# Woodenonez/TrajTrack-MPCnDQN-RLBoost

Hardware: NVIDIA B200
Metric: batched NMPC solves/sec (higher is better)
Workload: dtype f64

## Files before the change

### trajtrack_mpcndqn_rlboost_b200/csrc/ttmpc_api.cu

```cuda
#include <cuda_runtime.h>

#include <cstdio>
#include <cstdlib>
#include <cstring>
#include <algorithm>
#include <atomic>
#include <condition_variable>
#include <mutex>
#include <thread>
#include <string>
#include <vector>

#include "ttmpc_device.cuh"
#include "ttmpc_launch.cuh"

using namespace ttmpc;

static thread_local std::string g_err;
static int fail(int code, const std::string &msg) { g_err = msg; return code; }
namespace ttmpc { void set_last_error(const std::string &msg) { g_err = msg; } }
#define CUDA_TRY(x)                                                                     \
  do {                                                                                  \
    cudaError_t e__ = (x);                                                              \
    if (e__ != cudaSuccess)                                                             \
      return fail(TTMPC_ERR_CUDA, std::string(#x) + ": " + cudaGetErrorString(e__));    \
  } while (0)

extern "C" const char *ttmpc_last_error(void) { return g_err.c_str(); }
extern "C" int ttmpc_version(void) { return TTMPC_VERSION; }
extern "C" int ttmpc_set_device(int device) { CUDA_TRY(cudaSetDevice(device)); return TTMPC_OK; }
extern "C" int ttmpc_get_device(int *device) {
  if (!device) return fail(TTMPC_ERR_BAD_ARG, "null output");
  CUDA_TRY(cudaGetDevice(device));
  return TTMPC_OK;
}
extern "C" const char *ttmpc_exit_status_name(int code) {
  switch (code) {
    case TTMPC_CONVERGED: return "Converged";
    case TTMPC_NOT_CONVERGED_ITERATIONS: return "NotConvergedIterations";
    case TTMPC_NOT_CONVERGED_OUT_OF_TIME: return "NotConvergedOutOfTime";
    case TTMPC_NOT_FINITE: return "NotFiniteComputation";
    default: return "Unknown";
  }
}

extern "C" void ttmpc_default_config(ttmpc_config *c) {
  std::memset(c, 0, sizeof(*c));
  c->N_hor = 20; c->nu = 2; c->ns = 3; c->nq = 10;
  c->Nother = 10; c->Nstcobs = 10; c->nstcobs = 12; c->Ndynobs = 15; c->ndynobs = 6;
  c->ts = 0.2; c->vehicle_width = 0.5; c->social_margin = 0.2;
  c->lin_vel_min = -0.5; c->lin_vel_max = 1.5; c->ang_vel_max = 0.5;
  c->lin_acc_min = -1.0; c->lin_acc_max = 1.0; c->ang_acc_max = 3.0;
  c->tolerance = 1e-4; c->initial_tolerance = 1e-4; c->delta_tolerance = 1e-4;
  c->initial_penalty = 10.0; c->penalty_update_factor = 5.0;
  c->inner_tolerance_update_factor = 0.1; c->sufficient_decrease_coeff = 0.1;
  c->lbfgs_memory = 10; c->max_inner_iterations = 500; c->max_outer_iterations = 10;
  c->max_duration_ms = 5000;
}
extern "C" int ttmpc_num_params(const ttmpc_config *c) {
  const int N = c->N_hor;
  return 2 * c->ns + c->nu + c->nq + c->ns * N + N + c->ns * N * c->Nother +
         c->Nstcobs * c->nstcobs + c->Ndynobs * c->ndynobs * N + 2 * N;
}
extern "C" int ttmpc_num_decision(const ttmpc_config *c) { return c->nu * c->N_hor; }
extern "C" int ttmpc_num_alm(const ttmpc_config *c) { return 2 * c->N_hor; }
extern "C" int ttmpc_num_penalty(const ttmpc_config *c) { return c->Ndynobs; }

static int make_devcfg(const ttmpc_config *c, DevCfg *g) {
  if (!c) return fail(TTMPC_ERR_BAD_CONFIG, "null config");
  if (c->nu != 2 || c->ns != 3 || c->nq != 10 || c->ndynobs != 6)
    return fail(TTMPC_ERR_BAD_CONFIG, "nu/ns/nq/ndynobs must be 2/3/10/6 (unicycle, mpc_generator.py layout)");
  if (c->N_hor < 1 || c->N_hor > 32) return fail(TTMPC_ERR_BAD_CONFIG, "N_hor must be in 1..32");
  if (c->nstcobs % 3 != 0 || c->nstcobs / 3 > MAX_EDGE || (c->Nstcobs > 0 && c->nstcobs < 3))
    return fail(TTMPC_ERR_BAD_CONFIG, "nstcobs must be 3*edges with edges <= 8");
  if (c->Nother < 0 || c->Nstcobs < 0 || c->Ndynobs < 0 || c->Ndynobs > 64 || c->Nother > 32 ||
      c->Nstcobs > 32)
    return fail(TTMPC_ERR_BAD_CONFIG, "obstacle counts out of range (Nother, Nstcobs <= 32, Ndynobs <= 64)");
  if (c->lbfgs_memory < 1 || c->lbfgs_memory > MAX_MEM)
    return fail(TTMPC_ERR_BAD_CONFIG, "lbfgs_memory must be in 1..16");
  if (c->max_inner_iterations < 1 || c->max_outer_iterations < 1 || !(c->ts > 0.0))
    return fail(TTMPC_ERR_BAD_CONFIG, "iteration limits and ts must be positive");
  const int N = c->N_hor;
  g->N = N; g->Nother = c->Nother; g->Nstc = c->Nstcobs; g->nstcobs = c->nstcobs;
  g->ne = c->nstcobs / 3; g->Ndyn = c->Ndynobs; g->mem = c->lbfgs_memory;
  g->max_inner = c->max_inner_iterations; g->max_outer = c->max_outer_iterations;
  g->max_ns = c->max_duration_ms > 0 ? (unsigned long long)c->max_duration_ms * 1000000ull : 0ull;
  g->off_s = 0; g->off_q = 2 * c->ns + c->nu; g->off_r = g->off_q + c->nq;
  g->off_vref = g->off_r + c->ns * N; g->off_c = g->off_vref + N;
  g->off_os = g->off_c + c->ns * N * c->Nother;
  g->off_od = g->off_os + c->Nstcobs * c->nstcobs;
  g->off_qdyn = g->off_od + c->Ndynobs * c->ndynobs * N + N;
  g->np = g->off_qdyn + N;
  g->smem_per_warp = smem_bytes_per_warp(N, g->Nother, g->Nstc, g->nstcobs, g->Ndyn, g->mem);
  {
    const size_t cap = 232448 - 256;
    if ((size_t)g->smem_per_warp > cap)
      return fail(TTMPC_ERR_UNSUPPORTED, "configuration does not fit in shared memory: " +
                  std::to_string(g->smem_per_warp) + " bytes of tables per scene, 227 KB per SM");
    int wpb = 1, best = 0;
    for (int cand : {2, 3, 4, 1}) {
      const size_t per_cta = (size_t)g->smem_per_warp * cand + 96 + 1024;
      if ((size_t)g->smem_per_warp * cand > cap) continue;
      const int ctas = (int)std::min<size_t>(233472 / per_cta, (size_t)(8 / cand));
      if (ctas * cand > best) { best = ctas * cand; wpb = cand; }
    }
    g->warps_per_block = wpb;
  }
  g->ts = c->ts; g->inv_ts = 1.0 / c->ts; g->h6 = c->ts / 6.0; g->veh_d2 = c->vehicle_width * c->vehicle_width; g->margin = c->social_margin;
  g->vmin = c->lin_vel_min; g->vmax = c->lin_vel_max; g->wmax = c->ang_vel_max;
  g->amin = c->lin_acc_min; g->amax = c->lin_acc_max; g->awmax = c->ang_acc_max;
  g->tol = c->tolerance; g->init_tol = c->initial_tolerance; g->delta_tol = c->delta_tolerance;
  g->c0 = c->initial_penalty; g->pen_factor = c->penalty_update_factor;
  g->tol_factor = c->inner_tolerance_update_factor; g->suff_dec = c->sufficient_decrease_coeff;
  return TTMPC_OK;
}

struct Slot {
  bool keyed = false;
  cudaStream_t key = nullptr;
  bool host = false, host_busy = false;
  double *dyn_scratch = nullptr; size_t dyn_bytes = 0;
  int *work_counter = nullptr;
  unsigned long long *run_stats = nullptr;
  int *ready = nullptr;
  int *h_ready = nullptr;
  cudaStream_t copy_stream = nullptr, exec_stream = nullptr;
  cudaEvent_t ev_inputs = nullptr;
  cudaEvent_t ev_done = nullptr;
  int *order = nullptr; size_t order_ints = 0;
  void *dbuf = nullptr; size_t dbytes = 0;
  void *hbuf = nullptr; size_t hbytes = 0;
};
constexpr int MAX_STREAM_SLOTS = 16, MAX_HOST_SLOTS = 8;
struct Workspace {
  int device = -1;
  int sm_count = 0;
  unsigned long long *stats = nullptr;
  std::vector<Slot *> slots;
};
static std::mutex g_mu;
static std::condition_variable g_cv;
static std::vector<Workspace> g_ws;

static int get_ws(Workspace **out) {
  int dev = 0;
  CUDA_TRY(cudaGetDevice(&dev));
  for (auto &w : g_ws)
    if (w.device == dev) { *out = &w; return TTMPC_OK; }
  Workspace w;
  w.device = dev;
  CUDA_TRY(cudaDeviceGetAttribute(&w.sm_count, cudaDevAttrMultiProcessorCount, dev));
  CUDA_TRY(cudaMalloc(&w.stats, 192));
  CUDA_TRY(cudaMemset(w.stats, 0, 192));
  g_ws.reserve(16);
  g_ws.push_back(w);
  *out = &g_ws.back();
  return TTMPC_OK;
}
static int new_slot(Workspace *w, Slot **out) {
  Slot *s = new Slot();
  CUDA_TRY(cudaMalloc(&s->work_counter, 64));
  CUDA_TRY(cudaMalloc(&s->run_stats, 64));
  CUDA_TRY(cudaMemset(s->run_stats, 0, 64));
  CUDA_TRY(cudaMalloc(&s->ready, 64));
  w->slots.push_back(s);
  *out = s;
  return TTMPC_OK;
}
static int slot_for_stream(Workspace *w, cudaStream_t st, Slot **out) {
  for (int pass = 0; pass < 2; pass++) {
    int device_slots = 0;
    Slot *free_slot = nullptr;
    for (Slot *s : w->slots) {
      if (s->host) continue;
      device_slots++;
      if (s->keyed && s->key == st) { *out = s; return TTMPC_OK; }
      if (!s->keyed && !free_slot) free_slot = s;
    }
    if (!free_slot && device_slots < MAX_STREAM_SLOTS) {
      int rc = new_slot(w, &free_slot);
      if (rc) return rc;
    }
    if (free_slot) {
      free_slot->keyed = true; free_slot->key = st;
      *out = free_slot;
      return TTMPC_OK;
    }
    CUDA_TRY(cudaDeviceSynchronize());
    for (Slot *s : w->slots)
      if (!s->host) s->keyed = false;
  }
  return fail(TTMPC_ERR_CUDA, "no scene-queue slot for this stream");
}
static int acquire_host_slot(Workspace **wout, Slot **out, int *busy_calls) {
  std::unique_lock<std::mutex> lk(g_mu);
  Workspace *w;
  int rc = get_ws(&w);
  if (rc) return rc;
  *wout = w;
  while (true) {
    int hosts = 0, busy = 1;
    for (Slot *s : w->slots) busy += (s->host && s->host_busy) ? 1 : 0;
    *busy_calls = busy;
    for (Slot *s : w->slots) {
      if (!s->host) continue;
      hosts++;
      if (!s->host_busy) { s->host_busy = true; *out = s; return TTMPC_OK; }
    }
    if (hosts < MAX_HOST_SLOTS) break;
    g_cv.wait(lk);
  }
  Slot *s;
  rc = new_slot(w, &s);
  if (rc) return rc;
  cudaError_t e = cudaHostAlloc(&s->h_ready, sizeof(int) * 4096, cudaHostAllocDefault);
  if (e == cudaSuccess) e = cudaStreamCreateWithFlags(&s->copy_stream, cudaStreamNonBlocking);
  if (e == cudaSuccess) e = cudaStreamCreateWithFlags(&s->exec_stream, cudaStreamNonBlocking);
  if (e == cudaSuccess) e = cudaEventCreateWithFlags(&s->ev_inputs, cudaEventDisableTiming);
  if (e == cudaSuccess) e = cudaEventCreateWithFlags(&s->ev_done, cudaEventDisableTiming | cudaEventBlockingSync);
  if (e != cudaSuccess)
    return fail(TTMPC_ERR_CUDA, std::string("host path: streams / pinned memory of a new slot: ") + cudaGetErrorString(e));
  s->host = true; s->host_busy = true;
  *out = s;
  return TTMPC_OK;
}
namespace {
struct HostSlotLease {
  Slot *s = nullptr;
  bool clean = false;
  ~HostSlotLease() {
    if (!s) return;
    if (!clean) {
      if (s->copy_stream) cudaStreamSynchronize(s->copy_stream);
      if (s->exec_stream) cudaStreamSynchronize(s->exec_stream);
      cudaGetLastError();
    }
    { std::lock_guard<std::mutex> lk(g_mu); s->host_busy = false; }
    g_cv.notify_one();
  }
};
}
static int wait_stream(Slot *s, cudaStream_t st, int n_scenes) {
  if (n_scenes < 512) { CUDA_TRY(cudaStreamSynchronize(st)); return TTMPC_OK; }
  CUDA_TRY(cudaEventRecord(s->ev_done, st));
  CUDA_TRY(cudaEventSynchronize(s->ev_done));
  return TTMPC_OK;
}
static int ensure_dyn(Slot *w, size_t bytes) {
  if (bytes <= w->dyn_bytes) return TTMPC_OK;
  if (w->dyn_scratch) CUDA_TRY(cudaFree(w->dyn_scratch));
  w->dyn_scratch = nullptr; w->dyn_bytes = 0;
  CUDA_TRY(cudaMalloc(&w->dyn_scratch, bytes));
  w->dyn_bytes = bytes;
  return TTMPC_OK;
}
static int ensure_order(Slot *w, size_t ints) {
  if (ints <= w->order_ints) return TTMPC_OK;
  if (w->order) CUDA_TRY(cudaFree(w->order));
  w->order = nullptr; w->order_ints = 0;
  CUDA_TRY(cudaMalloc(&w->order, ints * sizeof(int)));
  w->order_ints = ints;
  return TTMPC_OK;
}
static int ensure_staging(Slot *w, size_t bytes) {
  if (bytes > w->dbytes) {
    if (w->dbuf) CUDA_TRY(cudaFree(w->dbuf));
    w->dbuf = nullptr; w->dbytes = 0;
    CUDA_TRY(cudaMalloc(&w->dbuf, bytes));
    if (w->copy_stream) CUDA_TRY(cudaMemsetAsync(w->dbuf, 0, bytes, w->copy_stream));
    else { CUDA_TRY(cudaMemset(w->dbuf, 0, bytes)); CUDA_TRY(cudaDeviceSynchronize()); }
    w->dbytes = bytes;
  }
  if (bytes > w->hbytes) {
    if (w->hbuf) CUDA_TRY(cudaFreeHost(w->hbuf));
    w->hbuf = nullptr; w->hbytes = 0;
    CUDA_TRY(cudaHostAlloc(&w->hbuf, bytes, cudaHostAllocDefault));
    w->hbytes = bytes;
  }
  return TTMPC_OK;
}

static int grid_for(Workspace *w, const DevCfg &g, int n_scenes, int *grid) {
  int bps = 0;
  CUDA_TRY(solve_occupancy(g, &bps));
  if (bps < 1) return fail(TTMPC_ERR_UNSUPPORTED, "configuration does not fit in shared memory");
  long long want = ((long long)n_scenes + g.warps_per_block - 1) / g.warps_per_block;
  long long cap = (long long)w->sm_count * bps;
  *grid = (int)(want < cap ? (want < 1 ? 1 : want) : cap);
  return TTMPC_OK;
}

static int solve_device_impl(const ttmpc_config *cfg, int n_scenes, const double *d_p, int use_u0,
                             int use_y0, const double *d_c0, const ttmpc_result *res,
                             cudaStream_t st, Slot *host_slot, bool gated);

extern "C" int ttmpc_solve_batch_device(const ttmpc_config *cfg, int n_scenes, const double *d_p,
                                        int use_u0, int use_y0, const double *d_c0,
                                        const ttmpc_result *res, void *stream) {
  return solve_device_impl(cfg, n_scenes, d_p, use_u0, use_y0, d_c0, res, (cudaStream_t)stream, nullptr, false);
}

static int solve_device_impl(const ttmpc_config *cfg, int n_scenes, const double *d_p, int use_u0,
                             int use_y0, const double *d_c0, const ttmpc_result *res,
                             cudaStream_t st, Slot *host_slot, bool gated) {
  DevCfg g;
  int rc = make_devcfg(cfg, &g);
  if (rc) return rc;
  if (n_scenes < 0 || !res || !res->u || (n_scenes > 0 && !d_p))
    return fail(TTMPC_ERR_BAD_ARG, "n_scenes >= 0, d_p and res->u are required");
  if (n_scenes == 0) return TTMPC_OK;
  Workspace *w;
  Slot *sl = host_slot;
  const int *d_ready = (host_slot && gated) ? host_slot->ready : nullptr;
  int grid;
  bool want_order = false;
  {
    std::lock_guard<std::mutex> lk(g_mu);
    rc = get_ws(&w);
    if (rc) return rc;
    if (!sl) { rc = slot_for_stream(w, st, &sl); if (rc) return rc; }
    rc = grid_for(w, g, n_scenes, &grid);
    if (rc) return rc;
    const size_t table = (size_t)DYN_FIELDS * g.Ndyn * g.N * sizeof(double);
    rc = ensure_dyn(sl, (table ? table : 8) * (size_t)grid * g.warps_per_block);
    if (rc) return rc;
    want_order = !d_ready && n_scenes > (long long)grid * g.warps_per_block;
    if (want_order) {
      rc = ensure_order(sl, 2 * (size_t)n_scenes + 64);
      if (rc) return rc;
    }
  }
  CUDA_TRY(cudaMemsetAsync(sl->work_counter, 0, sizeof(int), st));
  const char *nh = std::getenv("TTMPC_NO_HELPERS");
  SolveArgs A;
  A.eprof = w->stats + 8;
  A.helpers = (nh && nh[0] == '1') ? 0 : 1;
  A.ready = d_ready; A.timeout_flag = d_ready ? sl->ready + 1 : nullptr;
  A.p = d_p; A.c0 = d_c0; A.u = res->u; A.y = res->y; A.cost = res->cost;
  A.last_fpr = res->last_fpr; A.f1_infeas = res->f1_infeas; A.f2_norm = res->f2_norm;
  A.penalty = res->penalty; A.exit_status = res->exit_status; A.outer_iters = res->outer_iters;
  A.inner_iters = res->inner_iters; A.pred_states = res->pred_states; A.evals = res->evals;
  A.dyn_scratch = sl->dyn_scratch; A.work_counter = sl->work_counter; A.stats = w->stats;
  A.run_stats = sl->run_stats;
  CUDA_TRY(cudaMemsetAsync(A.run_stats, 0, 2 * sizeof(unsigned long long), st));
  A.n_scenes = n_scenes; A.use_u0 = use_u0; A.use_y0 = use_y0;
  A.order = nullptr;
  if (want_order) {
    CUDA_TRY(launch_rank_scenes(g, d_p, n_scenes, sl->order + n_scenes, sl->order, st));
    A.order = sl->order;
  }
  bool small_code = n_scenes > (long long)grid * g.warps_per_block;
  if (const char *e = std::getenv("TTMPC_CODE")) {
    if (e[0] == 's') small_code = true;
    else if (e[0] == 'u') small_code = false;
  }
  if (small_code) CUDA_TRY(launch_solve_small(g, A, grid, st));
  else CUDA_TRY(launch_solve(g, A, grid, st));
  return TTMPC_OK;
}

static int fleet_dims(const ttmpc_config *cfg, const ttmpc_fleet *f, FleetDims *d) {
  DevCfg g;
  int rc = make_devcfg(cfg, &g);
  if (rc) return rc;
  if (!f || f->n < 0) return fail(TTMPC_ERR_BAD_ARG, "fleet: null or n < 0");
  if (f->n > 0 && (!f->state || !f->goal || !f->last_u || !f->idx_ref || !f->status || !f->ref_traj ||
                   !f->ref_len || !f->stc))
    return fail(TTMPC_ERR_BAD_ARG, "fleet: state, goal, last_u, idx_ref, status, ref_traj, ref_len, stc are required");
  if (f->action_steps != 1) return fail(TTMPC_ERR_UNSUPPORTED, "fleet: only action_steps = 1 is supported");
  if (f->ref_stride < 1) return fail(TTMPC_ERR_BAD_ARG, "fleet: ref_stride must be >= 1");
  if (f->dyn_cur && (!f->dyn_last || !f->dyn_disp || f->n_dyn_live < 0 || f->n_dyn_live > cfg->Ndynobs))
    return fail(TTMPC_ERR_BAD_ARG, "fleet: dyn_cur needs dyn_last, dyn_disp and 0 <= n_dyn_live <= Ndynobs");
  d->N = cfg->N_hor; d->np = g.np; d->ts = cfg->ts;
  d->n_other = cfg->ns * cfg->N_hor * cfg->Nother;
  d->n_stc = cfg->Nstcobs * cfg->nstcobs;
  d->n_dyn = cfg->Ndynobs * cfg->ndynobs * cfg->N_hor;
  return TTMPC_OK;
}
extern "C" int ttmpc_fleet_pack_device(const ttmpc_config *cfg, const ttmpc_fleet *fleet, double *d_p,
                                       void *stream) {
  FleetDims d;
  int rc = fleet_dims(cfg, fleet, &d);
  if (rc) return rc;
  if (fleet->n == 0) return TTMPC_OK;
  if (!d_p) return fail(TTMPC_ERR_BAD_ARG, "fleet: d_p is required");
  CUDA_TRY(launch_fleet_pack(*fleet, d, d_p, (cudaStream_t)stream));
  return TTMPC_OK;
}
extern "C" int ttmpc_fleet_advance_device(const ttmpc_config *cfg, const ttmpc_fleet *fleet,
                                          const double *d_u, const int *d_exit_status, void *stream) {
  FleetDims d;
  int rc = fleet_dims(cfg, fleet, &d);
  if (rc) return rc;
  if (fleet->n == 0) return TTMPC_OK;
  if (!d_u) return fail(TTMPC_ERR_BAD_ARG, "fleet: d_u is required");
  CUDA_TRY(launch_fleet_advance(*fleet, d, d_u, d_exit_status, (cudaStream_t)stream));
  return TTMPC_OK;
}
extern "C" int ttmpc_fleet_step_device(const ttmpc_config *cfg, const ttmpc_fleet *fleet, double *d_p,
                                       int use_y0, const ttmpc_result *res, void *stream) {
  if (!res || !res->u || !res->exit_status)
    return fail(TTMPC_ERR_BAD_ARG, "fleet: res->u and res->exit_status are required");
  int rc = ttmpc_fleet_pack_device(cfg, fleet, d_p, stream);
  if (rc) return rc;
  rc = ttmpc_solve_batch_device(cfg, fleet->n, d_p, 0, use_y0, nullptr, res, stream);
  if (rc) return rc;
  return ttmpc_fleet_advance_device(cfg, fleet, res->u, res->exit_status, stream);
}

static int read_stats(unsigned long long *out, int count, int reset) {
  std::lock_guard<std::mutex> lk(g_mu);
  Workspace *w;
  int rc = get_ws(&w);
  if (rc) return rc;
  CUDA_TRY(cudaDeviceSynchronize());
  CUDA_TRY(cudaMemcpy(out, w->stats, count * sizeof(unsigned long long), cudaMemcpyDeviceToHost));
  if (reset) CUDA_TRY(cudaMemset(w->stats, 0, 192));
  return TTMPC_OK;
}
extern "C" int ttmpc_read_stats(unsigned long long out[4], int reset) { return read_stats(out, 4, reset); }
extern "C" int ttmpc_read_stats8(unsigned long long out[8], int reset) { return read_stats(out, 8, reset); }
extern "C" int ttmpc_read_stats24(unsigned long long out[24], int reset) { return read_stats(out, 24, reset); }

extern "C" int ttmpc_launch_info(const ttmpc_config *cfg, int n_scenes, int *grid, int *block,
                                 int *smem_bytes, int *blocks_per_sm, int *sm_count) {
  DevCfg g;
  int rc = make_devcfg(cfg, &g);
  if (rc) return rc;
  std::lock_guard<std::mutex> lk(g_mu);
  Workspace *w;
  rc = get_ws(&w);
  if (rc) return rc;
  int gr;
  rc = grid_for(w, g, n_scenes, &gr);
  if (rc) return rc;
  int bps = 0;
  CUDA_TRY(solve_occupancy(g, &bps));
  if (grid) *grid = gr;
  if (block) *block = g.warps_per_block * 32;
  if (smem_bytes) *smem_bytes = g.smem_per_warp * g.warps_per_block;
  if (blocks_per_sm) *blocks_per_sm = bps;
  if (sm_count) *sm_count = w->sm_count;
  return TTMPC_OK;
}

namespace {
struct Carver {
  char *d, *h; size_t off = 0;
  template <class T> void take(size_t n, T **dp, T **hp) {
    off = (off + 255) / 256 * 256;
    *dp = reinterpret_cast<T *>(d + off);
    *hp = reinterpret_cast<T *>(h + off);
    off += n * sizeof(T);
  }
};
}

extern "C" int ttmpc_solve_batch_host(const ttmpc_config *cfg, int n, const double *h_p,
                                      int use_u0, int use_y0, const double *h_c0,
                                      const ttmpc_result *res) {
  DevCfg g;
  int rc = make_devcfg(cfg, &g);
  if (rc) return rc;
  if (n < 0 || !res || !res->u || (n > 0 && !h_p))
    return fail(TTMPC_ERR_BAD_ARG, "n >= 0, h_p and res->u are required");
  if (n == 0) return TTMPC_OK;
  const size_t nn = (size_t)n, nu = 2 * (size_t)g.N;
  size_t total = 4096 + 256 * 16 + sizeof(double) * (nn * g.np + nn + 2 * nn * nu + 5 * nn + nn * g.N * 3) +
                 sizeof(int) * 3 * nn + sizeof(long long) * 4 * nn;
  Workspace *ws;
  Slot *w = nullptr;
  int busy_calls = 1;
  rc = acquire_host_slot(&ws, &w, &busy_calls);
  HostSlotLease lease{w};
  if (rc) return rc;
  rc = ensure_staging(w, total);
  if (rc) return rc;
  Carver cv{(char *)w->dbuf, (char *)w->hbuf};
  double *dp, *hp, *dc0, *hc0, *du, *hu, *dy, *hy, *dcost, *hcost, *dfpr, *hfpr, *df1, *hf1, *df2,
      *hf2, *dpen, *hpen, *dps, *hps;
  int *dex, *hex, *dout, *hout, *din, *hin;
  long long *dev, *hev;
  cv.take(nn * g.np, &dp, &hp);
  cv.take(nn, &dc0, &hc0);
  cv.take(nn * nu, &du, &hu);
  cv.take(nn * nu, &dy, &hy);
  cv.take(nn, &dcost, &hcost);
  cv.take(nn, &dfpr, &hfpr);
  cv.take(nn, &df1, &hf1);
  cv.take(nn, &df2, &hf2);
  cv.take(nn, &dpen, &hpen);
  cv.take(nn * g.N * 3, &dps, &hps);
  cv.take(nn, &dex, &hex);
  cv.take(nn, &dout, &hout);
  cv.take(nn, &din, &hin);
  cv.take(4 * nn, &dev, &hev);
  cudaStream_t cs = w->copy_stream, st = w->exec_stream;
  CUDA_TRY(cudaMemsetAsync(w->ready, 0, 2 * sizeof(int), cs));
  if (h_c0) {
    std::memcpy(hc0, h_c0, sizeof(double) * nn);
    CUDA_TRY(cudaMemcpyAsync(dc0, hc0, sizeof(double) * nn, cudaMemcpyHostToDevice, cs));
  }
  if (use_u0) {
    std::memcpy(hu, res->u, sizeof(double) * nn * nu);
    CUDA_TRY(cudaMemcpyAsync(du, hu, sizeof(double) * nn * nu, cudaMemcpyHostToDevice, cs));
  }
  if (use_y0 && res->y) {
    std::memcpy(hy, res->y, sizeof(double) * nn * nu);
    CUDA_TRY(cudaMemcpyAsync(dy, hy, sizeof(double) * nn * nu, cudaMemcpyHostToDevice, cs));
  }
  CUDA_TRY(cudaEventRecord(w->ev_inputs, cs));
  CUDA_TRY(cudaStreamWaitEvent(st, w->ev_inputs, 0));
  ttmpc_result dres;
  std::memset(&dres, 0, sizeof(dres));
  dres.u = du; dres.y = res->y ? dy : nullptr; dres.cost = dcost; dres.exit_status = dex;
  dres.outer_iters = dout; dres.inner_iters = din; dres.last_fpr = dfpr; dres.f1_infeas = df1;
  dres.f2_norm = df2; dres.penalty = dpen; dres.pred_states = res->pred_states ? dps : nullptr;
  dres.evals = dev;
  const char *lb = std::getenv("CUDA_LAUNCH_BLOCKING");
  const bool stream_in = busy_calls <= 1 && !(lb && lb[0] == '1');
  if (stream_in) {
    rc = solve_device_impl(cfg, n, dp, use_u0, use_y0 && res->y, h_c0 ? dc0 : nullptr, &dres, st, w, true);
    if (rc) return rc;
  }
  cudaPointerAttributes at;
  const bool pinned_in = cudaPointerGetAttributes(&at, h_p) == cudaSuccess ? at.type == cudaMemoryTypeHost
                                                                           : (cudaGetLastError(), false);
  {
    int chunk = 256;
    while ((n + chunk - 1) / chunk > 4096) chunk *= 2;
    const int n_chunks = (n + chunk - 1) / chunk;
    struct Chunk { int s1; size_t off, cnt; };
    auto chunk_at = [&](int ci) {
      const int s0 = ci * chunk, s1 = std::min(s0 + chunk, n);
      return Chunk{s1, (size_t)s0 * g.np, (size_t)(s1 - s0) * g.np};
    };
    const unsigned hw = std::thread::hardware_concurrency();
    int budget = (int)(hw ? hw / 2 : 1);
    if (const char *e = std::getenv("TTMPC_HOST_THREADS")) { const int v = std::atoi(e); if (v >= 1) budget = v; }
    const int T = pinned_in ? 1 : std::max(1, std::min({8, budget / std::max(1, busy_calls), n_chunks}));
    const double *src = pinned_in ? h_p : hp;
    std::vector<std::atomic<int>> staged(n_chunks);
    for (auto &f : staged) f.store(pinned_in ? 1 : 0, std::memory_order_relaxed);
    auto stage = [&](int ci) {
      const Chunk c = chunk_at(ci);
      std::memcpy(hp + c.off, h_p + c.off, sizeof(double) * c.cnt);
      staged[ci].store(1, std::memory_order_release);
    };
    std::vector<std::thread> workers;
    for (int t = 1; t < T; t++)
      workers.emplace_back([&, t] { for (int ci = t; ci < n_chunks; ci += T) stage(ci); });
    int rc_copy = TTMPC_OK;
    int mine = 0;
    for (int ci = 0; ci < n_chunks; ci++) {
      while (!staged[ci].load(std::memory_order_acquire)) {
        if (mine < n_chunks) { stage(mine); mine += T; }
        else std::this_thread::yield();
      }
      if (rc_copy != TTMPC_OK) continue;
      const Chunk c = chunk_at(ci);
      w->h_ready[ci] = c.s1;
      if (cudaMemcpyAsync(dp + c.off, src + c.off, sizeof(double) * c.cnt, cudaMemcpyHostToDevice, cs) != cudaSuccess ||
          cudaMemcpyAsync(w->ready, w->h_ready + ci, sizeof(int), cudaMemcpyHostToDevice, cs) != cudaSuccess)
        rc_copy = TTMPC_ERR_CUDA;
    }
    for (auto &th : workers) th.join();
    if (rc_copy != TTMPC_OK) return fail(TTMPC_ERR_CUDA, "host path: asynchronous copy of the parameter block failed");
  }
  int timed_out = 0;
  if (stream_in) {
    rc = wait_stream(w, st, n);
    if (rc) return rc;
    CUDA_TRY(cudaMemcpy(&timed_out, w->ready + 1, sizeof(int), cudaMemcpyDeviceToHost));
  }
  if (!stream_in || timed_out) {
    rc = wait_stream(w, cs, n);
    if (rc) return rc;
    if (use_u0) CUDA_TRY(cudaMemcpyAsync(du, hu, sizeof(double) * nn * nu, cudaMemcpyHostToDevice, st));
    if (use_y0 && res->y) CUDA_TRY(cudaMemcpyAsync(dy, hy, sizeof(double) * nn * nu, cudaMemcpyHostToDevice, st));
    rc = solve_device_impl(cfg, n, dp, use_u0, use_y0 && res->y, h_c0 ? dc0 : nullptr, &dres, st, w, false);
    if (rc) return rc;
  }
  const size_t out_begin = (size_t)((char *)du - (char *)w->dbuf);
  CUDA_TRY(cudaMemcpyAsync((char *)w->hbuf + out_begin, (char *)w->dbuf + out_begin, cv.off - out_begin,
                           cudaMemcpyDeviceToHost, st));
  rc = wait_stream(w, st, n);
  if (rc) return rc;
  std::memcpy(res->u, hu, sizeof(double) * nn * nu);
  if (res->y) std::memcpy(res->y, hy, sizeof(double) * nn * nu);
  if (res->cost) std::memcpy(res->cost, hcost, sizeof(double) * nn);
  if (res->last_fpr) std::memcpy(res->last_fpr, hfpr, sizeof(double) * nn);
  if (res->f1_infeas) std::memcpy(res->f1_infeas, hf1, sizeof(double) * nn);
  if (res->f2_norm) std::memcpy(res->f2_norm, hf2, sizeof(double) * nn);
  if (res->penalty) std::memcpy(res->penalty, hpen, sizeof(double) * nn);
  if (res->pred_states) std::memcpy(res->pred_states, hps, sizeof(double) * nn * g.N * 3);
  if (res->exit_status) std::memcpy(res->exit_status, hex, sizeof(int) * nn);
  if (res->outer_iters) std::memcpy(res->outer_iters, hout, sizeof(int) * nn);
  if (res->inner_iters) std::memcpy(res->inner_iters, hin, sizeof(int) * nn);
  if (res->evals) std::memcpy(res->evals, hev, sizeof(long long) * 4 * nn);
  lease.clean = true;
  return TTMPC_OK;
}

extern "C" int ttmpc_eval_batch_device(const ttmpc_config *cfg, int n, const double *d_p,
                                       const double *d_u, const double *d_c, const double *d_y,
                                       double *d_f, double *d_F1, double *d_F2, double *d_psi,
                                       double *d_grad, void *stream) {
  DevCfg g;
  int rc = make_devcfg(cfg, &g);
  if (rc) return rc;
  if (n < 0 || (n > 0 && (!d_p || !d_u))) return fail(TTMPC_ERR_BAD_ARG, "d_p and d_u are required");
  if (n == 0) return TTMPC_OK;
  std::lock_guard<std::mutex> lk(g_mu);
  Workspace *w;
  rc = get_ws(&w);
  if (rc) return rc;
  int grid;
  rc = grid_for(w, g, n, &grid);
  if (rc) return rc;
  const size_t table = (size_t)DYN_FIELDS * g.Ndyn * g.N * sizeof(double);
  Slot *sl;
  rc = slot_for_stream(w, (cudaStream_t)stream, &sl);
  if (rc) return rc;
  rc = ensure_dyn(sl, (table ? table : 8) * (size_t)grid * g.warps_per_block);
  if (rc) return rc;
  EvalArgs A;
  A.p = d_p; A.u = d_u; A.c = d_c; A.y = d_y; A.f = d_f; A.F1 = d_F1; A.F2 = d_F2; A.psi = d_psi;
  A.grad = d_grad; A.dyn_scratch = sl->dyn_scratch; A.n_scenes = n;
  CUDA_TRY(launch_eval(g, A, grid, (cudaStream_t)stream));
  return TTMPC_OK;
}

extern "C" int ttmpc_eval_batch_host(const ttmpc_config *cfg, int n, const double *h_p,
                                     const double *h_u, const double *h_c, const double *h_y,
                                     double *h_f, double *h_F1, double *h_F2, double *h_psi,
                                     double *h_grad) {
  DevCfg g;
  int rc = make_devcfg(cfg, &g);
  if (rc) return rc;
  if (n < 0 || (n > 0 && (!h_p || !h_u))) return fail(TTMPC_ERR_BAD_ARG, "h_p and h_u are required");
  if (n == 0) return TTMPC_OK;
  const size_t nn = (size_t)n, nu = 2 * (size_t)g.N;
  double *dp = nullptr, *du = nullptr, *dc = nullptr, *dy = nullptr, *df = nullptr, *dF1 = nullptr,
         *dF2 = nullptr, *dpsi = nullptr, *dgrad = nullptr;
  auto cleanup = [&]() {
    cudaFree(dp); cudaFree(du); cudaFree(dc); cudaFree(dy); cudaFree(df); cudaFree(dF1);
    cudaFree(dF2); cudaFree(dpsi); cudaFree(dgrad);
  };
#define TRY_OR_CLEAN(x) do { cudaError_t e__ = (x); if (e__ != cudaSuccess) { cleanup(); return fail(TTMPC_ERR_CUDA, std::string(#x) + ": " + cudaGetErrorString(e__)); } } while (0)
  TRY_OR_CLEAN(cudaMalloc(&dp, sizeof(double) * nn * g.np));
  TRY_OR_CLEAN(cudaMalloc(&du, sizeof(double) * nn * nu));
  TRY_OR_CLEAN(cudaMalloc(&dc, sizeof(double) * nn));
  TRY_OR_CLEAN(cudaMalloc(&dy, sizeof(double) * nn * nu));
  TRY_OR_CLEAN(cudaMalloc(&df, sizeof(double) * nn));
  TRY_OR_CLEAN(cudaMalloc(&dF1, sizeof(double) * nn * nu));
  TRY_OR_CLEAN(cudaMalloc(&dF2, sizeof(double) * nn * (g.Ndyn > 0 ? g.Ndyn : 1)));
  TRY_OR_CLEAN(cudaMalloc(&dpsi, sizeof(double) * nn));
  TRY_OR_CLEAN(cudaMalloc(&dgrad, sizeof(double) * nn * nu));
  TRY_OR_CLEAN(cudaMemcpy(dp, h_p, sizeof(double) * nn * g.np, cudaMemcpyHostToDevice));
  TRY_OR_CLEAN(cudaMemcpy(du, h_u, sizeof(double) * nn * nu, cudaMemcpyHostToDevice));
  if (h_c) TRY_OR_CLEAN(cudaMemcpy(dc, h_c, sizeof(double) * nn, cudaMemcpyHostToDevice));
  if (h_y) TRY_OR_CLEAN(cudaMemcpy(dy, h_y, sizeof(double) * nn * nu, cudaMemcpyHostToDevice));
  rc = ttmpc_eval_batch_device(cfg, n, dp, du, h_c ? dc : nullptr, h_y ? dy : nullptr, df, dF1, dF2,
                               dpsi, dgrad, 0);
  if (rc) { cleanup(); return rc; }
  TRY_OR_CLEAN(cudaDeviceSynchronize());
  if (h_f) TRY_OR_CLEAN(cudaMemcpy(h_f, df, sizeof(double) * nn, cudaMemcpyDeviceToHost));
  if (h_F1) TRY_OR_CLEAN(cudaMemcpy(h_F1, dF1, sizeof(double) * nn * nu, cudaMemcpyDeviceToHost));
  if (h_F2 && g.Ndyn) TRY_OR_CLEAN(cudaMemcpy(h_F2, dF2, sizeof(double) * nn * g.Ndyn, cudaMemcpyDeviceToHost));
  if (h_psi) TRY_OR_CLEAN(cudaMemcpy(h_psi, dpsi, sizeof(double) * nn, cudaMemcpyDeviceToHost));
  if (h_grad) TRY_OR_CLEAN(cudaMemcpy(h_grad, dgrad, sizeof(double) * nn * nu, cudaMemcpyDeviceToHost));
  cleanup();
  return TTMPC_OK;
}

extern "C" int ttmpc_probe_latency(const ttmpc_config *cfg, const double *h_p, long long out[8], int reps) {
  DevCfg g;
  int rc = make_devcfg(cfg, &g);
  if (rc) return rc;
  double *dp = nullptr, *dyn = nullptr; long long *dout = nullptr;
  CUDA_TRY(cudaMalloc(&dp, sizeof(double) * g.np));
  CUDA_TRY(cudaMalloc(&dyn, sizeof(double) * DYN_FIELDS * (g.Ndyn > 0 ? g.Ndyn : 1) * g.N));
  CUDA_TRY(cudaMalloc(&dout, 64));
  CUDA_TRY(cudaMemcpy(dp, h_p, sizeof(double) * g.np, cudaMemcpyHostToDevice));
  CUDA_TRY(launch_probe(g, dp, dyn, dout, reps, 0));
  CUDA_TRY(cudaDeviceSynchronize());
  CUDA_TRY(cudaMemcpy(out, dout, 64, cudaMemcpyDeviceToHost));
  cudaFree(dp); cudaFree(dyn); cudaFree(dout);
  return TTMPC_OK;
}

extern "C" int ttmpc_measure_fp64_peak(double *tflops, void *stream) {
  if (!tflops) return fail(TTMPC_ERR_BAD_ARG, "null output");
  int dev = 0, sms = 0;
  CUDA_TRY(cudaGetDevice(&dev));
  CUDA_TRY(cudaDeviceGetAttribute(&sms, cudaDevAttrMultiProcessorCount, dev));
  const int threads = 256, blocks = sms * 8, iters = 1 << 15;
  double *out = nullptr;
  CUDA_TRY(cudaMalloc(&out, sizeof(double) * threads * blocks));
  cudaStream_t st = (cudaStream_t)stream;
  cudaEvent_t e0, e1;
  CUDA_TRY(cudaEventCreate(&e0));
  CUDA_TRY(cudaEventCreate(&e1));
  double best = 0.0;
  for (int rep = 0; rep < 4; rep++) {
    CUDA_TRY(cudaEventRecord(e0, st));
    CUDA_TRY(launch_fp64_peak(out, blocks, threads, iters, st));
    CUDA_TRY(cudaEventRecord(e1, st));
    CUDA_TRY(cudaEventSynchronize(e1));
    float ms = 0;
    CUDA_TRY(cudaEventElapsedTime(&ms, e0, e1));
    double fl = 2.0 * 8.0 * (double)iters * threads * blocks;
    double tf = fl / (ms * 1e-3) / 1e12;
    if (rep > 0 && tf > best) best = tf;
  }
  cudaEventDestroy(e0); cudaEventDestroy(e1); cudaFree(out);
  *tflops = best;
  return TTMPC_OK;
}
```

### trajtrack_mpcndqn_rlboost_b200/csrc/ttmpc_device.cuh

```cuda
#pragma once
#include <cuda_runtime.h>
#include <math.h>
#include <stdint.h>

#include "../../include/ttmpc.h"

#ifdef TTMPC_SMALL_CODE
#define TT_UNROLL_4 _Pragma("unroll 1")
#else
#define TT_UNROLL_4 _Pragma("unroll 4")
#endif
namespace ttmpc {

constexpr unsigned FULL = 0xffffffffu;
constexpr int MAX_MEM = 16;
constexpr int MAX_EDGE = 8;
constexpr int DYN_FIELDS = 10;
#ifndef TT_DYN_SLOTS
#define TT_DYN_SLOTS 4
#endif
constexpr int DYN_SLOTS = TT_DYN_SLOTS;

struct DevCfg {
  int N, Nother, Nstc, ne, nstcobs, Ndyn, mem, max_inner, max_outer;
  int off_s, off_q, off_r, off_vref, off_c, off_os, off_od, off_qdyn, np;
  int smem_per_warp;
  int warps_per_block;
  double ts, inv_ts, h6, veh_d2, margin;
  double vmin, vmax, wmax, amin, amax, awmax;
  double tol, init_tol, delta_tol, c0, pen_factor, tol_factor, suff_dec;
  unsigned long long max_ns;
};

__host__ __device__ __forceinline__ void tt_sincos(double x, double *s, double *c) {
  const double kd = rint(x * 6.36619772367581382433e-01);
  double r = fma(-kd, 1.5707963267948966e+00, x);
  r = fma(-kd, 6.123233995736766e-17, r);
  r = fma(-kd, -1.4973849048591698e-33, r);
  const int q = (int)((long long)kd & 3);
  const double z = r * r;
  double ps = fma(z, 1.58969099521155010221e-10, -2.50507602534068634195e-08);
  ps = fma(z, ps, 2.75573137070700676789e-06);
  ps = fma(z, ps, -1.98412698298579493134e-04);
  ps = fma(z, ps, 8.33333333332248946124e-03);
  ps = fma(z, ps, -1.66666666666666324348e-01);
  const double sr = fma(r * z, ps, r);
  double pc = fma(z, -1.13596475577881948265e-11, 2.08757232129817482790e-09);
  pc = fma(z, pc, -2.75573143513906633035e-07);
  pc = fma(z, pc, 2.48015872894767294178e-05);
  pc = fma(z, pc, -1.38888888888741095749e-03);
  pc = fma(z, pc, 4.16666666666666019037e-02);
  const double cr = fma(z * z, pc, fma(-0.5, z, 1.0));
  const bool swap = (q & 1) != 0;
  const double sb = swap ? cr : sr, cb = swap ? sr : cr;
  double so = (q & 2) ? -sb : sb, co = ((q + 1) & 2) ? -cb : cb;
  if (!(fabs(x) < 1.0e9)) { so = x * 0.0 + NAN; co = so; }
  *s = so; *c = co;
}

static __constant__ double TT_SC[16] = {
    6.36619772367581382433e-01, 1.5707963267948966e+00, 6.123233995736766e-17, -1.4973849048591698e-33,
    1.58969099521155010221e-10, -2.50507602534068634195e-08, 2.75573137070700676789e-06,
    -1.98412698298579493134e-04, 8.33333333332248946124e-03, -1.66666666666666324348e-01,
    -1.13596475577881948265e-11, 2.08757232129817482790e-09, -2.75573143513906633035e-07,
    2.48015872894767294178e-05, -1.38888888888741095749e-03, 4.16666666666666019037e-02};
__device__ __forceinline__ void tt_sincos_c(double x, double *s, double *c) {
  const double kd = rint(x * TT_SC[0]);
  double r = fma(-kd, TT_SC[1], x);
  r = fma(-kd, TT_SC[2], r);
  r = fma(-kd, TT_SC[3], r);
  const int q = (int)((long long)kd & 3);
  const double z = r * r;
  double ps = fma(z, TT_SC[4], TT_SC[5]);
  ps = fma(z, ps, TT_SC[6]);
  ps = fma(z, ps, TT_SC[7]);
  ps = fma(z, ps, TT_SC[8]);
  ps = fma(z, ps, TT_SC[9]);
  const double sr = fma(r * z, ps, r);
  double pc = fma(z, TT_SC[10], TT_SC[11]);
  pc = fma(z, pc, TT_SC[12]);
  pc = fma(z, pc, TT_SC[13]);
  pc = fma(z, pc, TT_SC[14]);
  pc = fma(z, pc, TT_SC[15]);
  const double cr = fma(z * z, pc, fma(-0.5, z, 1.0));
  const bool swap = (q & 1) != 0;
  const double sb = swap ? cr : sr, cb = swap ? sr : cr;
  double so = (q & 2) ? -sb : sb, co = ((q + 1) & 2) ? -cb : cb;
  if (!(fabs(x) < 1.0e9)) { so = x * 0.0 + NAN; co = so; }
  *s = so; *c = co;
}

static __device__ __noinline__ double tt_div(double a, double b) { return a / b; }
static __device__ __noinline__ double tt_sqrt(double a) { return sqrt(a); }

template <int O>
__device__ __forceinline__ void up_add(double &v) {
  asm volatile("{\n\t.reg .pred p;\n\t.reg .b32 lo, hi, tl, th;\n\t.reg .f64 t;\n\t"
               "mov.b64 {lo, hi}, %0;\n\t"
               "shfl.sync.up.b32 tl|p, lo, %1, 0, 0xffffffff;\n\t"
               "shfl.sync.up.b32 th, hi, %1, 0, 0xffffffff;\n\t"
               "mov.b64 t, {tl, th};\n\t"
               "@p add.rn.f64 %0, %0, t;\n\t}"
               : "+d"(v) : "n"(O));
}
template <int O>
__device__ __forceinline__ void down_add(double &v) {
  asm volatile("{\n\t.reg .pred p;\n\t.reg .b32 lo, hi, tl, th;\n\t.reg .f64 t;\n\t"
               "mov.b64 {lo, hi}, %0;\n\t"
               "shfl.sync.down.b32 tl|p, lo, %1, 31, 0xffffffff;\n\t"
               "shfl.sync.down.b32 th, hi, %1, 31, 0xffffffff;\n\t"
               "mov.b64 t, {tl, th};\n\t"
               "@p add.rn.f64 %0, %0, t;\n\t}"
               : "+d"(v) : "n"(O));
}
__device__ __forceinline__ double wscan(double v, int) {
  up_add<1>(v); up_add<2>(v); up_add<4>(v); up_add<8>(v); up_add<16>(v);
  return v;
}
__device__ __forceinline__ void wscan2(double &a, double &b) {
  up_add<1>(a); up_add<1>(b); up_add<2>(a); up_add<2>(b); up_add<4>(a); up_add<4>(b);
  up_add<8>(a); up_add<8>(b); up_add<16>(a); up_add<16>(b);
}
__device__ __forceinline__ double wsuffix(double v, int) {
  down_add<1>(v); down_add<2>(v); down_add<4>(v); down_add<8>(v); down_add<16>(v);
  return v;
}
__device__ __forceinline__ void wsuffix2(double &a, double &b) {
  down_add<1>(a); down_add<1>(b); down_add<2>(a); down_add<2>(b); down_add<4>(a); down_add<4>(b);
  down_add<8>(a); down_add<8>(b); down_add<16>(a); down_add<16>(b);
}
template <int O>
__device__ __forceinline__ double xor_get(double v) {
  double t;
  asm volatile("{\n\t.reg .b32 lo, hi, tl, th;\n\t"
               "mov.b64 {lo, hi}, %1;\n\t"
               "shfl.sync.bfly.b32 tl, lo, %2, 31, 0xffffffff;\n\t"
               "shfl.sync.bfly.b32 th, hi, %2, 31, 0xffffffff;\n\t"
               "mov.b64 %0, {tl, th};\n\t}"
               : "=d"(t) : "d"(v), "n"(O));
  return t;
}
__device__ __forceinline__ double wsum_inl(double v) {
  v += xor_get<16>(v); v += xor_get<8>(v); v += xor_get<4>(v); v += xor_get<2>(v); v += xor_get<1>(v);
  return v;
}
static __device__ __noinline__ double wsum(double v) { return wsum_inl(v); }
__device__ __forceinline__ void wsum4_inl(double &a, double &b, double &c, double &d, int lane) {
  const bool b4 = (lane & 16) != 0, b3 = (lane & 8) != 0;
  double x = b4 ? c : a, y = b4 ? d : b;
  const double sx = b4 ? a : c, sy = b4 ? b : d;
  x += xor_get<16>(sx); y += xor_get<16>(sy);
  double z = b3 ? y : x;
  const double sz = b3 ? x : y;
  z += xor_get<8>(sz);
  z += xor_get<4>(z); z += xor_get<2>(z); z += xor_get<1>(z);
  a = __shfl_sync(FULL, z, 0); b = __shfl_sync(FULL, z, 8);
  c = __shfl_sync(FULL, z, 16); d = __shfl_sync(FULL, z, 24);
}
struct D4 { double a, b, c, d; };
static __device__ __noinline__ D4 wsum4v(double a, double b, double c, double d) {
  wsum4_inl(a, b, c, d, threadIdx.x & 31);
  D4 r; r.a = a; r.b = b; r.c = c; r.d = d;
  return r;
}
__device__ __forceinline__ void wsum4(double &a, double &b, double &c, double &d, int) {
  const D4 r = wsum4v(a, b, c, d);
  a = r.a; b = r.b; c = r.c; d = r.d;
}
__device__ __forceinline__ void wsum2(double &a, double &b) {
  const D4 r = wsum4v(a, b, 0.0, 0.0);
  a = r.a; b = r.b;
}
__device__ __forceinline__ void wsum3(double &a, double &b, double &c) {
  const D4 r = wsum4v(a, b, c, 0.0);
  a = r.a; b = r.b; c = r.c;
}
__device__ __forceinline__ double clipd_ref(double z, double lo, double hi) {
  return fmin(fmax(z, lo), hi);
}
__device__ __forceinline__ double sel_gt(double a, double b, double x, double y) {
  double r;
  asm("{\n\t.reg .pred p;\n\tsetp.gt.f64 p, %1, %2;\n\tselp.f64 %0, %3, %4, p;\n\t}"
      : "=d"(r) : "d"(a), "d"(b), "d"(x), "d"(y));
  return r;
}
__device__ __forceinline__ double sel_lt(double a, double b, double x, double y) {
  double r;
  asm("{\n\t.reg .pred p;\n\tsetp.lt.f64 p, %1, %2;\n\tselp.f64 %0, %3, %4, p;\n\t}"
      : "=d"(r) : "d"(a), "d"(b), "d"(x), "d"(y));
  return r;
}
__device__ __forceinline__ double clipd(double z, double lo, double hi) {
  const double t = sel_gt(z, lo, z, lo);
  return sel_lt(t, hi, t, hi);
}
__device__ __forceinline__ double relu(double x) { return sel_gt(x, 0.0, x, 0.0); }
__device__ __forceinline__ double clamp01(double x) {
  const double t = sel_gt(x, 0.0, x, 0.0);
  return sel_lt(t, 1.0, t, 1.0);
}
__device__ __forceinline__ double pdot(double a0, double a1, double b0, double b1) {
  return fma(a1, b1, a0 * b0);
}

struct WarpCtx {
  const double *p;
  double *dyn;
  double x0, y0, th0, xg, yg, thg, v_init, w_init;
  double qvel, rv, rw, qN, qthetaN, qrpd, acc_pen, wacc_pen;
  long long n_cost, n_grad, n_body;
  int nstc_active;
  float fleet_thr;
  double box_half;
  unsigned long long dyn_live;
  unsigned fleet_live;
  double lipc;
  double icm_c, icm;
#ifdef TTMPC_PROFILE
  long long prof[8];
  long long eprof[10];
#endif
};

struct HelpHdr;
struct WarpSmem {
  WarpCtx *ctx;
  double *seg;
  double *os;
  double *D;
  double *vref;
  float2 *fleet;
  float *dynb;
  double *dynt;
  double2 *lbs;
  double2 *lby;
  double *rho;
  double *alpha;
  double2 *hreq;
  double2 *hres;
  double2 *yrow;
  struct HelpHdr *hhdr;
};
struct HelpHdr {
  int state;
  int grad;
  double c, gamma_ls;
  double psi, f, f2sq, S, dd, g2;
};

__device__ __forceinline__ int first_bit(unsigned m) { return __ffs((int)m) - 1; }
__device__ __forceinline__ int first_bit(unsigned long long m) { return __ffsll((long long)m) - 1; }
__device__ __forceinline__ int pop_bits(unsigned m) { return __popc(m); }
__device__ __forceinline__ int pop_bits(unsigned long long m) { return __popcll(m); }
template <bool WIDE> struct DynMask { using type = unsigned long long; };
template <> struct DynMask<false> { using type = unsigned; };

template <int N_, int NO_, int NS_, int NE_, int ND_, int MEM_ = 0>
struct Dims {
  using dmask = typename DynMask<(N_ == 0 || ND_ > 32)>::type;
  static constexpr int kN = N_, kNstc = NS_;
  __device__ __forceinline__ static int mem(const DevCfg &g) { return N_ ? MEM_ : g.mem; }
  __device__ __forceinline__ static int N(const DevCfg &g) { return N_ ? N_ : g.N; }
  __device__ __forceinline__ static int Nother(const DevCfg &g) { return N_ ? NO_ : g.Nother; }
  __device__ __forceinline__ static int Nstc(const DevCfg &g) { return N_ ? NS_ : g.Nstc; }
  __device__ __forceinline__ static int ne(const DevCfg &g) { return N_ ? NE_ : g.ne; }
  __device__ __forceinline__ static int Ndyn(const DevCfg &g) { return N_ ? ND_ : g.Ndyn; }
};
using DimsRuntime = Dims<0, 0, 0, 0, 0>;
using DimsDefault = Dims<20, 10, 10, 4, 15, 10>;

__host__ __device__ inline int smem_bytes_per_warp(int N, int Nother, int Nstc, int nstcobs, int Ndyn,
                                                   int mem) {
  size_t b = 0;
  b += (sizeof(WarpCtx) + 15) / 16 * 16;
  b += sizeof(double) * 6 * N;
  b += sizeof(double) * ((Nstc * nstcobs + 1) / 2 * 2);
  b += sizeof(double) * ((Ndyn + 1) / 2 * 2);
  b += sizeof(double) * ((N + 1) / 2 * 2);
  b += (sizeof(float2) * (size_t)Nother * N + 15) / 16 * 16;
  b += (sizeof(float) * 3 * (size_t)Ndyn * N + 15) / 16 * 16;
  b += sizeof(double) * (size_t)(Ndyn ? DYN_SLOTS * DYN_FIELDS * N : 0);
  const int NP = N | 1;
  b += sizeof(double2) * (size_t)(mem + 1) * NP * 2;
  b += sizeof(double) * ((mem + 2) / 2 * 2);
  b += sizeof(double) * (2 * (mem + 1));
  b += sizeof(double2) * 3 * (size_t)N + (sizeof(HelpHdr) + 15) / 16 * 16;
  return (int)((b + 15) / 16 * 16);
}

template <class DM>
__device__ __forceinline__ WarpSmem carve(unsigned char *base, const DevCfg &g) {
  WarpSmem w;
  unsigned char *q = base;
  const int N = DM::N(g), MEM = DM::mem(g), Nother = DM::Nother(g), Nstc = DM::Nstc(g),
            nstcobs = 3 * DM::ne(g), Ndyn = DM::Ndyn(g);
  w.ctx = reinterpret_cast<WarpCtx *>(q); q += (sizeof(WarpCtx) + 15) / 16 * 16;
  const int NP = N | 1;
  w.lbs = reinterpret_cast<double2 *>(q); q += sizeof(double2) * (size_t)(MEM + 1) * NP;
  w.lby = reinterpret_cast<double2 *>(q); q += sizeof(double2) * (size_t)(MEM + 1) * NP;
  w.fleet = reinterpret_cast<float2 *>(q); q += (sizeof(float2) * (size_t)Nother * N + 15) / 16 * 16;
  w.dynb = reinterpret_cast<float *>(q); q += (sizeof(float) * 3 * (size_t)Ndyn * N + 15) / 16 * 16;
  w.dynt = reinterpret_cast<double *>(q); q += sizeof(double) * (size_t)(Ndyn ? DYN_SLOTS * DYN_FIELDS * N : 0);
  w.seg = reinterpret_cast<double *>(q); q += sizeof(double) * 6 * N;
  w.os = reinterpret_cast<double *>(q); q += sizeof(double) * ((Nstc * nstcobs + 1) / 2 * 2);
  w.D = reinterpret_cast<double *>(q); q += sizeof(double) * ((Ndyn + 1) / 2 * 2);
  w.vref = reinterpret_cast<double *>(q); q += sizeof(double) * ((N + 1) / 2 * 2);
  w.rho = reinterpret_cast<double *>(q); q += sizeof(double) * ((MEM + 2) / 2 * 2);
  w.alpha = reinterpret_cast<double *>(q); q += sizeof(double) * (2 * (MEM + 1));
  w.hreq = reinterpret_cast<double2 *>(q); q += sizeof(double2) * (size_t)N;
  w.hres = reinterpret_cast<double2 *>(q); q += sizeof(double2) * (size_t)N;
  w.yrow = reinterpret_cast<double2 *>(q); q += sizeof(double2) * (size_t)N;
  w.hhdr = reinterpret_cast<HelpHdr *>(q);
  return w;
}

__device__ __forceinline__ double &dynf(double *t, const DevCfg &g, int f, int j, int k) {
  return t[((size_t)f * g.Ndyn + j) * g.N + k];
}

struct DynRow { const double *p; int sf; };
template <class M>
__device__ __forceinline__ DynRow dyn_row(const WarpSmem &sm, const WarpCtx *cx, int j, int N, int Ndyn, int lk) {
  const M live = (M)cx->dyn_live;
  const int slot = pop_bits((M)(live & (((M)1 << j) - (M)1)));
  const bool in_s = (live >> j & (M)1) != (M)0 && slot < DYN_SLOTS;
  DynRow r;
  r.p = in_s ? sm.dynt + (size_t)slot * DYN_FIELDS * N + lk : cx->dyn + (size_t)j * N + lk;
  r.sf = in_s ? N : Ndyn * N;
  return r;
}

__device__ inline void stage_part1(const DevCfg &g, const WarpSmem &sm, const double *p, const double *p_global,
                                   double *dyn_scratch, int lane) {
  WarpCtx *c = sm.ctx;
  if (lane == 0) {
    const double *s = p + g.off_s, *q = p + g.off_q;
    c->p = p_global; c->dyn = dyn_scratch;
    c->x0 = s[0]; c->y0 = s[1]; c->th0 = s[2];
    c->xg = s[3]; c->yg = s[4]; c->thg = s[5];
    c->v_init = s[6]; c->w_init = s[7];
    c->qvel = q[1]; c->rv = q[3]; c->rw = q[4]; c->qN = q[5]; c->qthetaN = q[6];
    c->qrpd = q[7]; c->acc_pen = q[8]; c->wacc_pen = q[9];
    c->n_cost = 0; c->n_grad = 0; c->n_body = 0;
    c->lipc = 0.0; c->icm_c = NAN; c->icm = 0.0;
#ifdef TTMPC_PROFILE
    for (int i = 0; i < 8; i++) c->prof[i] = 0;
    for (int i = 0; i < 10; i++) c->eprof[i] = 0;
#endif
  }
  const double *r = p + g.off_r;
  for (int j = lane; j < g.N; j += 32) {
    int j2 = (j + 1 < g.N) ? j + 1 : g.N - 1;
    double s1x = r[3 * j], s1y = r[3 * j + 1];
    double sx = r[3 * j2] - s1x, sy = r[3 * j2 + 1] - s1y;
    double den = fma(sy, sy, sx * sx) + 1e-16;
    sm.seg[6 * j + 0] = s1x; sm.seg[6 * j + 1] = s1y;
    sm.seg[6 * j + 2] = sx;  sm.seg[6 * j + 3] = sy;
    sm.seg[6 * j + 4] = 1.0 / den; sm.seg[6 * j + 5] = 0.0;
  }
  const double *os = p + g.off_os;
  {
    int n_act = 0;
    for (int i0 = 0; i0 < g.Nstc; i0 += 32) {
      const int i = i0 + lane;
      bool live = false;
      if (i < g.Nstc) {
        live = true;
        const double *b = os + i * g.nstcobs, *a0 = b + g.ne, *a1 = b + 2 * g.ne;
        for (int e = 0; e < g.ne; e++)
          if (a0[e] == 0.0 && a1[e] == 0.0 && !(b[e] > 0.0)) live = false;
      }
      const unsigned m = __ballot_sync(FULL, live);
      if (live) {
        const int slot = n_act + __popc(m & ((1u << lane) - 1u));
        const double *src = os + i * g.nstcobs;
        double *dst = sm.os + slot * g.nstcobs;
        for (int e = 0; e < g.nstcobs; e++) dst[e] = (e < g.ne) ? src[e] : -src[e];
      }
      n_act += __popc(m);
    }
    if (lane == 0) c->nstc_active = n_act;
  }
  for (int k = lane; k < g.N; k += 32) sm.vref[k] = p[g.off_vref + k];
  const double *cpar = p + g.off_c;
  for (int t = lane; t < g.Nother * g.N; t += 32)
    sm.fleet[t] = make_float2((float)cpar[(size_t)t * 3], (float)cpar[(size_t)t * 3 + 1]);
  double cmax = 0.0;
  bool cnan = false;
  for (int t = lane; t < g.Nother * g.N; t += 32) {
    const double ax = fabs(cpar[(size_t)t * 3]), ay = fabs(cpar[(size_t)t * 3 + 1]);
    cnan = cnan || !(ax == ax) || !(ay == ay);
    cmax = fmax(cmax, fmax(ax, ay));
  }
  for (int o = 16; o > 0; o >>= 1) cmax = fmax(cmax, __shfl_xor_sync(FULL, cmax, o));
  cnan = __any_sync(FULL, cnan);
  if (lane == 0) {
    if (cnan) cmax = NAN;
    const double d = sqrt(g.veh_d2), pad = 4.8e-7 * (2.0 * cmax + 2.0 * d + 1.0) + 1e-6;
    float thr = __double2float_ru((d + pad) * (d + pad) * (1.0 + 1e-6));
    if (!(cmax == cmax)) thr = INFINITY;
    c->fleet_thr = thr;
  }
  {
    const double x0 = p[g.off_s], y0 = p[g.off_s + 1];
    const double vm = fmax(fabs(g.vmax), fabs(g.vmin));
    const double bh = 2.0 * g.N * g.ts * vm + 1.0;
    unsigned fl = 0;
    const double dveh = sqrt(g.veh_d2) * 1.001 + 1e-3;
    for (int t = lane; t < g.Nother * g.N; t += 32) {
      const int j = t / g.N;
      const bool outside = fabs(cpar[(size_t)t * 3] - x0) > bh + dveh || fabs(cpar[(size_t)t * 3 + 1] - y0) > bh + dveh;
      if (!outside) fl |= 1u << j;
    }
    fl = __reduce_or_sync(FULL, fl);
    if (lane == 0) { c->box_half = bh; c->fleet_live = fl; }
  }
  __syncwarp();
}

__device__ inline void stage_part2(const DevCfg &g, const WarpSmem &sm, const double *od, const double *qdyn,
                                   double *dyn_scratch, int lane) {
  WarpCtx *c = sm.ctx;
  const int npair = g.Ndyn * g.N;
  unsigned long long live;
  {
    const double x0 = c->x0, y0 = c->y0;
    const double bh = c->box_half;
    unsigned long long dl = 0;
    for (int t = lane; t < npair; t += 32) {
      const int j = t / g.N;
      const double *e = od + (size_t)t * 6;
      const double rmax = fmax(fmax(fabs(e[2] + 1e-6), fabs(e[3] + 1e-6)),
                               fmax(fabs(e[2] + g.margin + 1e-6), fabs(e[3] + g.margin + 1e-6))) * 1.001 + 1e-3;
      const bool outside = fabs(e[0] - x0) > bh + rmax || fabs(e[1] - y0) > bh + rmax;
      if (!outside) dl |= 1ull << j;
    }
    const unsigned dlo = __reduce_or_sync(FULL, (unsigned)dl), dhi = __reduce_or_sync(FULL, (unsigned)(dl >> 32));
    live = ((unsigned long long)dhi << 32) | dlo;
    if (lane == 0) c->dyn_live = live;
  }
  for (int t = lane; t < npair; t += 32) {
    int j = t / g.N, k = t - j * g.N;
    const double *e = od + (size_t)t * 6;
    double cx = e[0], cy = e[1], rx = e[2], ry = e[3], ang = e[4], alpha = e[5];
    double sa, ca;
    tt_sincos(ang, &sa, &ca);
    double Rx = rx + 1e-6, Ry = ry + 1e-6;
    double Rxm = rx + g.margin + 1e-6, Rym = ry + g.margin + 1e-6;
    double rmax = fmax(fmax(fabs(Rx), fabs(Ry)), fmax(fabs(Rxm), fabs(Rym)));
    double f[DYN_FIELDS];
    f[0] = cx; f[1] = cy; f[2] = rmax * rmax * (1.0 + 1e-9); f[3] = ca; f[4] = sa;
    f[5] = 1.0 / (Rx * Rx); f[6] = 1.0 / (Ry * Ry); f[7] = 1.0 / (Rxm * Rxm); f[8] = 1.0 / (Rym * Rym);
    f[9] = alpha * qdyn[k];
#pragma unroll
    for (int q = 0; q < DYN_FIELDS; q++) dynf(dyn_scratch, g, q, j, k) = f[q];
    {
      const int slot = __popcll(live & ((1ull << j) - 1ull));
      if ((live >> j & 1ull) && slot < DYN_SLOTS) {
#pragma unroll
        for (int q = 0; q < DYN_FIELDS; q++) sm.dynt[((size_t)slot * DYN_FIELDS + q) * g.N + k] = f[q];
      }
    }
    {
      const double pad = 4.8e-7 * (fabs(cx) + fabs(cy) + 2.0 * rmax + 1.0) + 1e-6;
      const double rp = rmax + pad;
      float r2f = __double2float_ru(rp * rp * (1.0 + 1e-6));
      if (!(rmax == rmax) || !(cx == cx) || !(cy == cy)) r2f = 0.0f;
      sm.dynb[3 * t] = (float)cx; sm.dynb[3 * t + 1] = (float)cy; sm.dynb[3 * t + 2] = r2f;
    }
  }
  __syncwarp();
}

__device__ inline void stage_scene(const DevCfg &g, const WarpSmem &sm, const double *p,
                                   double *dyn_scratch, int lane) {
#ifdef TTMPC_PROFILE_STAGE
  const long long td0 = clock64();
#endif
  stage_part1(g, sm, p, p, dyn_scratch, lane);
#ifdef TTMPC_PROFILE_STAGE
  const long long td1 = clock64();
#endif
  stage_part2(g, sm, p + g.off_od, p + g.off_qdyn, dyn_scratch, lane);
#ifdef TTMPC_PROFILE_STAGE
  if (lane == 0) { sm.ctx->prof[4] += td1 - td0; sm.ctx->prof[5] += clock64() - td1; }
#endif
}

#ifdef TTMPC_PROFILE
#define EPROF(slot) { const long long tt_ = clock64(); if (lane == 0 && !Dalt) sm.ctx->eprof[slot] += tt_ - ep_t; ep_t = tt_; }
#else
#define EPROF(slot)
#endif

struct EvalOut {
  double psi;
  double f;
  double f2sq;
  double S;
  double gv, gw;
  double h0, h1, dd, g2;
  bool any_hard;
};

static __device__ __noinline__ double icm_miss(double c, WarpCtx *ctx, bool store) {
  const double icm = 1.0 / fmax(c, 1.0);
  if (store) {
    __syncwarp();
    if ((threadIdx.x & 31) == 0) { ctx->icm = icm; ctx->icm_c = c; }
    __syncwarp();
  }
  return icm;
}

template <class DM>
__device__ __noinline__ EvalOut eval_psi(const DevCfg *gp, unsigned char *smem_base, double v_in,
                                         double w_in, double c, double ya, double yw,
                                         double *st_out, const bool GRAD, const double gamma_ls,
                                         double *Dalt = nullptr) {
  const DevCfg &g = *gp;
  const WarpSmem sm = carve<DM>(smem_base, g);
  double *const Dv = Dalt ? Dalt : sm.D;
  const int lane = threadIdx.x & 31;
  const double v = lane < DM::N(g) ? v_in : 0.0, w = lane < DM::N(g) ? w_in : 0.0;
  const WarpCtx *cx = sm.ctx;
  const int N = DM::N(g), Nother = DM::Nother(g), Nstc = cx->nstc_active, ne = DM::ne(g),
            Ndyn = DM::Ndyn(g);
  const int nstcobs = 3 * ne;
  const bool act = lane < N;
  const int lk = act ? lane : N - 1;
  const double ts = g.ts;

#ifdef TTMPC_PROFILE
  long long ep_t = clock64();
#endif
  const double icm = __builtin_expect(!Dalt && c == cx->icm_c, 1) ? cx->icm : icm_miss(c, sm.ctx, Dalt == nullptr);
  const double vr = sm.vref[lk];
  double t_vel, t_ctl, t_acc;
  double aa, aw, ea, ew, alm;
  {
    const double dv_ = v - vr;
    t_vel = cx->qvel * (dv_ * dv_);
    t_ctl = fma(cx->rw, w * w, cx->rv * (v * v));
    double vp = __shfl_up_sync(FULL, v, 1), wp = __shfl_up_sync(FULL, w, 1);
    if (lane == 0) { vp = cx->v_init; wp = cx->w_init; }
    aa = (v - vp) * g.inv_ts; aw = (w - wp) * g.inv_ts;
    t_acc = fma(aw * aw, cx->wacc_pen, (aa * aa) * cx->acc_pen);
    double z = fma(ya, icm, aa);
    ea = z - clipd(z, g.amin, g.amax);
    z = fma(yw, icm, aw);
    ew = z - clipd(z, -g.awmax, g.awmax);
    alm = fma(ew, ew, ea * ea);
  }
  const double tw = ts * w;
  const double th_in = wscan(tw, lane);
  double th_ex = __shfl_up_sync(FULL, th_in, 1);
  if (lane == 0) th_ex = 0.0;
  const double tha = cx->th0 + th_ex;
  const double thb = fma(0.5, tw, tha), thc = tha + tw;
  double sa, ca, sb, cb, sc, cc;
  tt_sincos_c(tha, &sa, &ca);
  tt_sincos_c(thb, &sb, &cb);
  if (N < 32) {
    sc = __shfl_down_sync(FULL, sa, 1); cc = __shfl_down_sync(FULL, ca, 1);
  } else {
    tt_sincos_c(thc, &sc, &cc);
  }
  const double Cs = fma(4.0, cb, ca) + cc, Ss = fma(4.0, sb, sa) + sc;
  const double hv = g.h6 * v;
  const double dx = hv * Cs, dy = hv * Ss;
  double X, Y;
  {
    double a = dx, b = dy;
    wscan2(a, b);
    X = cx->x0 + a; Y = cx->y0 + b;
  }
  const double TH = cx->th0 + th_in;
  if (st_out && act) { st_out[3 * lane] = X; st_out[3 * lane + 1] = Y; st_out[3 * lane + 2] = TH; }

  const bool in_box = __all_sync(FULL, fabs(X - cx->x0) < cx->box_half && fabs(Y - cx->y0) < cx->box_half);
  EPROF(0)
  double cost;
  double gx = 0.0, gy = 0.0;
  double S_loc = 0.0, gSx = 0.0, gSy = 0.0;

  auto static_obstacle = [&](int i) {
    const double *b = sm.os + i * nstcobs, *na0 = b + ne, *na1 = b + 2 * ne;
    double m[MAX_EDGE], sq[MAX_EDGE];
    double inside = 1.0;
#pragma unroll
    for (int e = 0; e < MAX_EDGE; e++) {
      if (e < ne) {
        m[e] = relu(fma(na1[e], Y, fma(na0[e], X, b[e])));
        sq[e] = m[e] * m[e];
        inside *= sq[e];
      }
    }
    if (__builtin_expect(__any_sync(FULL, inside > 0.0), 0)) {
      if (inside > 0.0) {
        S_loc += inside;
        if (GRAD) {
#pragma unroll
          for (int e = 0; e < MAX_EDGE; e++) {
            if (e < ne) {
              double rest = 1.0;
#pragma unroll
              for (int e2 = 0; e2 < MAX_EDGE; e2++)
                if (e2 < ne && e2 != e) rest *= sq[e2];
              const double coef = rest * (2.0 * m[e]);
              gSx = fma(coef, na0[e], gSx);
              gSy = fma(coef, na1[e], gSy);
            }
          }
        }
      }
    }
  };
  {
    const int nh = 32 - N;
    const bool is_helper = !act && (lane - N) < N;
    const int kq = is_helper ? lane - N : lk;
    const double Xq = __shfl_sync(FULL, X, kq), Yq = __shfl_sync(FULL, Y, kq);
    const bool split = kq < nh;
    const int mid = kq + (N - kq + 1) / 2;
    const int lo = is_helper ? mid : kq;
    const int hi = (act && split) ? mid : N;
    const int cnt = (act || is_helper) ? hi - lo : 0;
    const int trips = (nh >= N) ? (N + 1) / 2 : max((N + 1) / 2, N - nh);
    double dmin = INFINITY; int jmin = lo;
    const double2 *segv = reinterpret_cast<const double2 *>(sm.seg);
#pragma unroll 2
    for (int t = 0; t < trips; t++) {
      const int j = min(lo + t, N - 1);
      const double2 s1 = segv[3 * j], sd = segv[3 * j + 1];
      const double inv = sm.seg[6 * j + 4];
      const double px = Xq - s1.x, py = Yq - s1.y;
      const double t_hat = fma(py, sd.y, px * sd.x) * inv;
      const double tt = clamp01(t_hat);
      const double qx = fma(tt, sd.x, -px), qy = fma(tt, sd.y, -py);
      const double d2 = fma(qy, qy, qx * qx);
      const bool take = (t < cnt) && !(dmin <= d2);
      dmin = take ? d2 : dmin;
      jmin = take ? j : jmin;
    }
    {
      const int src = (act && split) ? N + lane : lane;
      const double dh = __shfl_sync(FULL, dmin, src);
      const int jh = __shfl_sync(FULL, jmin, src);
      if (act && split && !(dmin <= dh)) { dmin = dh; jmin = jh; }
    }
    cost = dmin * cx->qrpd;
    if (GRAD) {
      const int j = act ? jmin : N - 1;
      const double2 s1 = segv[3 * j], sd = segv[3 * j + 1];
      const double inv = sm.seg[6 * j + 4];
      const double px = X - s1.x, py = Y - s1.y;
      const double t_hat = fma(py, sd.y, px * sd.x) * inv;
      const double t = clamp01(t_hat);
      const double qx = fma(t, sd.x, -px), qy = fma(t, sd.y, -py);
      const double pass = (t_hat >= 0.0 && t_hat <= 1.0) ? 1.0 : 0.0;
      const double cs = fma(qy, sd.y, qx * sd.x) * pass * inv;
      gx = cx->qrpd * (2.0 * fma(cs, sd.x, -qx));
      gy = cx->qrpd * (2.0 * fma(cs, sd.y, -qy));
    }
  }
  EPROF(1)
  cost += t_vel;
  cost += t_ctl;
  const unsigned fleet_todo = in_box ? cx->fleet_live : (Nother >= 32 ? 0xffffffffu : ((1u << Nother) - 1u));
  using dmask = typename DM::dmask;
  const dmask dyn_todo = in_box ? (dmask)cx->dyn_live
                                : (Ndyn >= (int)(8 * sizeof(dmask)) ? ~(dmask)0 : (((dmask)1 << Ndyn) - (dmask)1));
  dmask hard_mask = 0;
  bool any_hard = false;
  if (fleet_todo != 0u || dyn_todo != 0ull) {
  const float Xf = (float)X, Yf = (float)Y;
  {
    unsigned hit = 0;
    const float thr = cx->fleet_thr;
    unsigned todo = fleet_todo;
    while (todo) {
      const int j = __ffs(todo) - 1;
      todo &= todo - 1;
      const float2 o = sm.fleet[j * N + lk];
      const float exf = Xf - o.x, eyf = Yf - o.y;
      hit |= (!((exf * exf + eyf * eyf) >= thr) ? 1u : 0u) << j;
    }
    if (__builtin_expect(__any_sync(FULL, hit != 0), 0)) {
      const double *cp = cx->p + g.off_c + 3 * lk;
      double acc = 0.0, fx = 0.0, fy = 0.0;
      while (hit) {
        const int j = __ffs(hit) - 1;
        hit &= hit - 1;
        const double ex = X - cp[(size_t)j * 3 * N], ey = Y - cp[(size_t)j * 3 * N + 1];
        const double e = g.veh_d2 - fma(ey, ey, ex * ex);
        if (e > 0.0) {
          acc += e;
          if (GRAD) { fx = fma(-2.0, ex, fx); fy = fma(-2.0, ey, fy); }
        }
      }
      cost += 1000.0 * acc;
      if (GRAD) { gx = fma(1000.0, fx, gx); gy = fma(1000.0, fy, gy); }
    }
  }
  EPROF(2)
  {
    dmask near_mask = 0;
    dmask todo = dyn_todo;
    while (todo) {
      const int j = first_bit(todo);
      todo &= todo - 1;
      const float *b = sm.dynb + 3 * (j * N + lk);
      const float exf = Xf - b[0], eyf = Yf - b[1];
      near_mask |= (dmask)((exf * exf + eyf * eyf) < b[2] ? 1u : 0u) << j;
    }
    if (__builtin_expect(__any_sync(FULL, near_mask != 0), 0)) {
      double soft = 0.0;
      int bodies = 0;
      while (near_mask) {
        const int j = first_bit(near_mask);
        near_mask &= near_mask - 1;
        const DynRow T = dyn_row<dmask>(sm, cx, j, N, Ndyn, lk);
        const double ex = X - T.p[0];
        const double ey = Y - T.p[T.sf];
        if (fma(ey, ey, ex * ex) < T.p[2 * T.sf]) {
          bodies++;
          const double ca_ = T.p[3 * T.sf];
          const double sa_ = T.p[4 * T.sf];
          const double A = fma(ey, sa_, ex * ca_), B = fma(-ey, ca_, ex * sa_);
          const double A2 = A * A, B2 = B * B;
          const double in1 = fma(-B2, T.p[6 * T.sf], fma(-A2, T.p[5 * T.sf], 1.0));
          if (in1 > 0.0) hard_mask |= (dmask)1 << j;
          const double iRxm = T.p[7 * T.sf];
          const double iRym = T.p[8 * T.sf];
          const double in2 = fma(-B2, iRym, fma(-A2, iRxm, 1.0));
          if (in2 > 0.0) {
            const double ws = T.p[9 * T.sf];
            soft = fma(in2 * in2, ws, soft);
            if (GRAD) {
              const double wg = ws * (2.0 * in2);
              const double tA = A * iRxm, tB = B * iRym;
              gx = fma(wg, -2.0 * fma(tB, sa_, tA * ca_), gx);
              gy = fma(wg, -2.0 * fma(-tB, ca_, tA * sa_), gy);
            }
          }
        }
      }
      cost += soft;
      if (!act) { bodies = 0; hard_mask = 0; }
      bodies = __reduce_add_sync(FULL, bodies);
      if (lane == 0 && !Dalt) sm.ctx->n_body += bodies;
    }
  }
  any_hard = __any_sync(FULL, hard_mask != 0);
  if (__builtin_expect(any_hard, 0)) {
    dmask warp_hard;
    if constexpr (sizeof(dmask) == 4) {
      warp_hard = __reduce_or_sync(FULL, (unsigned)hard_mask);
    } else {
      const unsigned lo = __reduce_or_sync(FULL, (unsigned)hard_mask);
      const unsigned hi = __reduce_or_sync(FULL, (unsigned)((unsigned long long)hard_mask >> 32));
      warp_hard = (dmask)(((unsigned long long)hi << 32) | lo);
    }
    for (int j = lane; j < Ndyn; j += 32) Dv[j] = 0.0;
    __syncwarp();
    while (warp_hard) {
      const int j = first_bit(warp_hard);
      warp_hard &= warp_hard - 1;
      double in1 = 0.0;
      if (hard_mask >> j & (dmask)1) {
        const DynRow T = dyn_row<dmask>(sm, cx, j, N, Ndyn, lk);
        const double ex = X - T.p[0];
        const double ey = Y - T.p[T.sf];
        const double ca_ = T.p[3 * T.sf];
        const double sa_ = T.p[4 * T.sf];
        const double A = fma(ey, sa_, ex * ca_), B = fma(-ey, ca_, ex * sa_);
        in1 = fma(-(B * B), T.p[6 * T.sf], fma(-(A * A), T.p[5 * T.sf], 1.0));
      }
      const double Dj = wsum(in1);
      if (lane == 0) Dv[j] = Dj;
    }
    __syncwarp();
  }
  }
  EPROF(3)
  double gt = 0.0;
  if (lane == N - 1 && (cx->qN != 0.0 || cx->qthetaN != 0.0)) {
    const double dxg = X - cx->xg, dyg = Y - cx->yg, dtg = TH - cx->thg;
    cost += fma(cx->qthetaN, dtg * dtg, cx->qN * fma(dyg, dyg, dxg * dxg));
    if (GRAD) {
      gx = fma(2.0 * cx->qN, dxg, gx);
      gy = fma(2.0 * cx->qN, dyg, gy);
      gt = 2.0 * cx->qthetaN * dtg;
    }
  }
  {
TT_UNROLL_4
    for (int i = 0; i < Nstc; i++) static_obstacle(i);
  }
  EPROF(4)
  cost += t_acc;
  if (!act) {
    cost = 0.0; gx = 0.0; gy = 0.0; S_loc = 0.0; gSx = 0.0; gSy = 0.0;
    aa = 0.0; aw = 0.0; ea = 0.0; ew = 0.0; alm = 0.0;
  }
  EPROF(5)
  double S = 0.0;
  if (__builtin_expect(__any_sync(FULL, S_loc != 0.0), 0)) S = wsum(S_loc);
  double f2sq = 0.0, sumF2 = 0.0;
  if (__builtin_expect(any_hard, 0)) {
#pragma unroll 1
    for (int j = 0; j < Ndyn; j++) {
      const double F2j = S + Dv[j];
      f2sq = fma(F2j, F2j, f2sq);
      sumF2 += F2j;
    }
  } else if (__builtin_expect(S != 0.0, 0)) {
#pragma unroll 5
    for (int j = 0; j < Ndyn; j++) {
      f2sq = fma(S, S, f2sq);
      sumF2 += S;
    }
  }
  EvalOut out;
  out.f2sq = f2sq; out.S = S; out.any_hard = any_hard;
  out.gv = 0.0; out.gw = 0.0;
  out.h0 = out.h1 = out.dd = out.g2 = 0.0;
  double ddp = 0.0, g2p = 0.0;

  EPROF(6)
  if (GRAD) {
    double gv = 0.0, gw = 0.0;
    if (c != 0.0) {
      const double cs_ = c * sumF2;
      gx = fma(cs_, gSx, gx);
      gy = fma(cs_, gSy, gy);
      if (__builtin_expect(any_hard, 0)) {
        dmask mk = hard_mask;
        while (mk) {
          const int j = first_bit(mk);
          mk &= mk - 1;
          const DynRow T = dyn_row<dmask>(sm, cx, j, N, Ndyn, lk);
          const double ex = X - T.p[0];
          const double ey = Y - T.p[T.sf];
          const double ca_ = T.p[3 * T.sf];
          const double sa_ = T.p[4 * T.sf];
          const double iRx = T.p[5 * T.sf];
          const double iRy = T.p[6 * T.sf];
          const double A = fma(ey, sa_, ex * ca_), B = fma(-ey, ca_, ex * sa_);
          const double wg = c * (S + Dv[j]);
          const double tA = A * iRx, tB = B * iRy;
          gx = fma(wg, -2.0 * fma(tB, sa_, tA * ca_), gx);
          gy = fma(wg, -2.0 * fma(-tB, ca_, tA * sa_), gy);
        }
      }
    }
    const double dxdv = g.h6 * Cs, dydv = g.h6 * Ss;
    const double hvt = hv * ts;
    const double dxdw = -(hvt * fma(2.0, sb, sc)), dydw = hvt * fma(2.0, cb, cc);
    double lx = gx, ly = gy;
    wsuffix2(lx, ly);
    const double m = fma(ly, dx, -(lx * dy));
    const double lt = wsuffix(gt + m, lane) - m;
    const double aa_n = __shfl_down_sync(FULL, aa, 1), aw_n = __shfl_down_sync(FULL, aw, 1);
    const double ea_n = __shfl_down_sync(FULL, ea, 1), ew_n = __shfl_down_sync(FULL, ew, 1);
    if (act) {
      const bool last = lane == N - 1;
      double dv = 2 * cx->qvel * (v - vr) + 2 * cx->rv * v;
      double dw = 2 * cx->rw * w;
      dv += (2 * cx->acc_pen * (aa - (last ? 0.0 : aa_n)) + c * (ea - (last ? 0.0 : ea_n))) * g.inv_ts;
      dw += (2 * cx->wacc_pen * (aw - (last ? 0.0 : aw_n)) + c * (ew - (last ? 0.0 : ew_n))) * g.inv_ts;
      gv = dv + lx * dxdv + ly * dydv;
      gw = dw + lx * dxdw + ly * dydw + lt * ts;
    }
    out.gv = gv; out.gw = gw;
    if (gamma_ls > 0.0 && act) {
      const double s0 = fma(-gamma_ls, gv, v), s1 = fma(-gamma_ls, gw, w);
      out.h0 = clipd(s0, g.vmin, g.vmax); out.h1 = clipd(s1, -g.wmax, g.wmax);
      const double q0 = out.h0 - s0, q1 = out.h1 - s1;
      ddp = pdot(q0, q1, q0, q1);
      g2p = pdot(gv, gw, gv, gw);
    }
  }
  EPROF(7)
  wsum4(cost, alm, ddp, g2p, lane);
  out.f = cost; out.dd = ddp; out.g2 = g2p;
  out.psi = cost + c * alm / 2 + c * f2sq / 2;
  EPROF(8)
  return out;
}

}
```

### trajtrack_mpcndqn_rlboost_b200/csrc/ttmpc_launch.cuh

```cuda
#pragma once
#include "ttmpc_device.cuh"

namespace ttmpc {

struct SolveArgs {
  const double *p;
  const double *c0;
  double *u;
  double *y;
  double *cost, *last_fpr, *f1_infeas, *f2_norm, *penalty;
  int *exit_status, *outer_iters, *inner_iters;
  double *pred_states;
  long long *evals;
  double *dyn_scratch;
  int *work_counter;
  const int *order;
  unsigned long long *eprof;
  int helpers;
  int *timeout_flag;
  const int *ready;
  unsigned long long *stats;
  unsigned long long *run_stats;
  int n_scenes;
  int use_u0, use_y0;
};

struct EvalArgs {
  const double *p, *u, *c, *y;
  double *f, *F1, *F2, *psi, *grad;
  double *dyn_scratch;
  int n_scenes;
};

cudaError_t launch_solve(const DevCfg &g, const SolveArgs &A, int grid, cudaStream_t st);
cudaError_t launch_solve_small(const DevCfg &g, const SolveArgs &A, int grid, cudaStream_t st);
cudaError_t launch_rank_scenes(const DevCfg &g, const double *p, int n, int *scratch, int *order,
                               cudaStream_t st);
cudaError_t launch_eval(const DevCfg &g, const EvalArgs &A, int grid, cudaStream_t st);
cudaError_t solve_occupancy(const DevCfg &g, int *blocks_per_sm);
cudaError_t launch_probe(const DevCfg &g, const double *p, double *dyn, long long *out, int reps,
                         cudaStream_t st);
struct FleetDims { int N, np, n_other, n_stc, n_dyn; double ts; };
cudaError_t launch_fleet_pack(const ttmpc_fleet &f, const FleetDims &d, double *p, cudaStream_t st);
cudaError_t launch_fleet_advance(const ttmpc_fleet &f, const FleetDims &d, const double *u,
                                 const int *exit_status, cudaStream_t st);
cudaError_t launch_fp64_peak(double *out, int blocks, int threads, int iters, cudaStream_t st);

}
```

### trajtrack_mpcndqn_rlboost_b200/csrc/ttmpc_solve.cu

```cuda
#include "ttmpc_device.cuh"
#include "ttmpc_launch.cuh"
#include <algorithm>
#include <cstdlib>
#include <map>
#include <mutex>
#include <tuple>

#ifndef TTMPC_MIN_BLOCKS
#define TTMPC_MIN_BLOCKS 2
#endif
#ifndef TTMPC_MAX_THREADS
#define TTMPC_MAX_THREADS 128
#endif
#ifdef TTMPC_SMALL_CODE
#define solve_kernel solve_kernel_small
#define launch_solve launch_solve_small
#define solve_occupancy_impl solve_occupancy_small_impl
#endif

namespace ttmpc {

constexpr double GAMMA_L_COEFF = 0.95;
constexpr double DELTA_LIPSCHITZ = 1e-12;
constexpr double EPSILON_LIPSCHITZ = 1e-6;
constexpr double LIPSCHITZ_UPDATE_EPSILON = 1e-6;
constexpr int MAX_LIPSCHITZ_UPDATE_ITERATIONS = 10;
constexpr double MAX_LIPSCHITZ_CONSTANT = 1e9;
constexpr int MAX_LINESEARCH_ITERATIONS = 10;
constexpr double MIN_L_ESTIMATE = 1e-10;
constexpr double CBFGS_EPSILON = 1e-8;
constexpr double SY_EPSILON = 1e-10;

struct Lane {
  double u0, u1;
  double g0, g1;
  double gp0, gp1;
  double h0, h1;
  double d0, d1;
  double f0, f1;
  double os0, os1, og0, og1;
};

struct Uni {
  double gamma, L, sigma, cost, norm_fpr, tau, akkt_tol, lb_gamma;
  double ip;
  double env_dd, env_g2;
  int iteration, lb_active, lb_head, lb_first;
};

__device__ __forceinline__ void project(const DevCfg &g, double a0, double a1, double &o0, double &o1) {
  o0 = clipd(a0, g.vmin, g.vmax);
  o1 = clipd(a1, -g.wmax, g.wmax);
}

__device__ __forceinline__ void set_lip_coeff(const Uni &U, const WarpSmem &sm) {
  const double lc = tt_div(GAMMA_L_COEFF, 2.0 * U.gamma);
  __syncwarp();
  if ((threadIdx.x & 31) == 0) sm.ctx->lipc = lc;
  __syncwarp();
}
__device__ __forceinline__ void set_gamma_terms(Uni &U, const WarpSmem &sm) {
  U.sigma = tt_div(1.0 - GAMMA_L_COEFF, 4.0 * U.gamma);
  set_lip_coeff(U, sm);
}
__device__ __forceinline__ double div_env(double x, double y) {
  if (x == 0.0 && y > 0.0) return x;
  return tt_div(x, y);
}

template <class DM>
__device__ __forceinline__ void lbfgs_update(const DevCfg &g, const WarpSmem &sm, Lane &z, Uni &U,
                                             int lane) {
  const int N = DM::N(g), NP = N | 1, MEM = DM::mem(g), M1 = MEM + 1;
  const double sv0 = z.u0 - z.os0, sv1 = z.u1 - z.os1;
  const double yv0 = z.f0 - z.og0, yv1 = z.f1 - z.og1;
  bool accept = true;
  double ys = 0.0, yy = 0.0;
  if (!U.lb_first) {
    double ss = pdot(sv0, sv1, sv0, sv1);
    ys = pdot(sv0, sv1, yv0, yv1); yy = pdot(yv0, yv1, yv0, yv1);
    wsum3(ys, ss, yy);
    const double lhs = tt_div(ys, ss);
    const double rhs = CBFGS_EPSILON * U.norm_fpr;
    accept = !(ss <= 2.2250738585072014e-308 || ys <= SY_EPSILON) &&
             (lhs > rhs && isfinite(lhs) && isfinite(rhs));
  }
  if (!accept) return;
  z.os0 = z.u0; z.os1 = z.u1; z.og0 = z.f0; z.og1 = z.f1;
  if (U.lb_first) { U.lb_first = 0; return; }
  U.lb_head = U.lb_head + MEM; if (U.lb_head >= M1) U.lb_head -= M1;
  const int k0 = U.lb_head;
  const double rho = tt_div(1.0, ys);
  if (lane < N) {
    sm.lbs[k0 * NP + lane] = make_double2(sv0, sv1);
    sm.lby[k0 * NP + lane] = make_double2(yv0, yv1);
  }
  if (lane == 0) sm.rho[k0] = rho;
  U.lb_gamma = tt_div(tt_div(1.0, rho), yy);
  U.lb_active = min(MEM, U.lb_active + 1);
  __syncwarp();
}

template <class DM>
__device__ __forceinline__ void lbfgs_apply(const DevCfg &g, const WarpSmem &sm, Lane &z,
                                            const Uni &U, int lane) {
  const int m = U.lb_active;
  if (m == 0) return;
  const int N = DM::N(g), NP = N | 1, M1 = DM::mem(g) + 1;
  const bool act = lane < N;
  const int lk = act ? lane : N - 1;
  double q0 = z.d0, q1 = z.d1, a_me = 0.0;
  int k = U.lb_head;
#pragma unroll 1
  for (int i = 0; i < m; i++) {
    const double2 s = sm.lbs[k * NP + lk], y = sm.lby[k * NP + lk];
    const double a = sm.rho[k] * wsum_inl(act ? pdot(s.x, s.y, q0, q1) : 0.0);
    if (lane == i) a_me = a;
    q0 = fma(-a, y.x, q0); q1 = fma(-a, y.y, q1);
    k = (k + 1 == M1) ? 0 : k + 1;
  }
  q0 = U.lb_gamma * q0; q1 = U.lb_gamma * q1;
#pragma unroll 1
  for (int i = m - 1; i >= 0; i--) {
    k = (k == 0) ? M1 - 1 : k - 1;
    const double2 s = sm.lbs[k * NP + lk], y = sm.lby[k * NP + lk];
    const double beta = sm.rho[k] * wsum_inl(act ? pdot(y.x, y.y, q0, q1) : 0.0);
    const double cf = __shfl_sync(FULL, a_me, i) - beta;
    q0 = fma(cf, s.x, q0); q1 = fma(cf, s.y, q1);
  }
  z.d0 = act ? q0 : 0.0; z.d1 = act ? q1 : 0.0;
}

__device__ __forceinline__ unsigned long long globaltimer_ns() {
  unsigned long long t;
  asm volatile("mov.u64 %0, %%globaltimer;" : "=l"(t));
  return t;
}

#ifdef TTMPC_PROFILE
#define PROF_BEGIN(v) const long long v = clock64();
#define PROF_END(v, slot) if (lane == 0) sm.ctx->prof[slot] += clock64() - v;
#else
#define PROF_BEGIN(v)
#define PROF_END(v, slot)
#endif

struct CtaHelp {
  int busy[8];
  int helper[8];
  int epoch[8];
};
struct HelpCtl {
  bool enabled;
  bool timed_out;
  volatile int *slot;
  bool pending;
};
template <bool HELP>
__device__ __forceinline__ bool help_available(const HelpCtl &hc) {
  if constexpr (!HELP) return false;
  else return hc.enabled && *hc.slot >= 0;
}
__device__ __forceinline__ bool help_wait(HelpCtl &hc, const WarpSmem &sm, int lane, int N, EvalOut &e) {
  int ok = 1;
  if (lane == 0) {
    const volatile int *st = reinterpret_cast<volatile int *>(&sm.hhdr->state);
    const unsigned long long t0 = globaltimer_ns();
    int spins = 0;
    while (*st != 2) {
      if (((++spins) & 1023) == 0 && globaltimer_ns() - t0 > 50000000ull) { ok = 0; break; }
    }
  }
  ok = __shfl_sync(FULL, ok, 0);
  hc.pending = false;
  if (!ok) {
    hc.enabled = false;
    hc.timed_out = true;
    return false;
  }
  __threadfence_block();
  const volatile HelpHdr *h = sm.hhdr;
  e.psi = h->psi; e.f = h->f; e.f2sq = h->f2sq; e.S = h->S; e.dd = h->dd; e.g2 = h->g2;
  {
    const volatile double *hr = reinterpret_cast<const volatile double *>(sm.hres);
    e.gv = lane < N ? hr[2 * lane] : 0.0;
    e.gw = lane < N ? hr[2 * lane + 1] : 0.0;
  }
  e.any_hard = false;
  e.h0 = e.h1 = 0.0;
  __syncwarp();
  if (lane == 0) *reinterpret_cast<volatile int *>(&sm.hhdr->state) = 0;
  return true;
}
__device__ __forceinline__ void help_post(HelpCtl &hc, const WarpSmem &sm, int lane, int N, double v,
                                          double w, double c, int grad, double gamma_ls) {
  if (hc.pending) {
    EvalOut tmp;
    if (!help_wait(hc, sm, lane, N, tmp)) return;
  }
  if (lane < N) sm.hreq[lane] = make_double2(v, w);
  if (lane == 0) { sm.hhdr->c = c; sm.hhdr->gamma_ls = gamma_ls; sm.hhdr->grad = grad; }
  __threadfence_block();
  __syncwarp();
  if (lane == 0) *reinterpret_cast<volatile int *>(&sm.hhdr->state) = 1;
  hc.pending = true;
}
__device__ __forceinline__ void help_drain(HelpCtl &hc, const WarpSmem &sm, int lane, int N) {
  if (hc.pending) { EvalOut tmp; help_wait(hc, sm, lane, N, tmp); }
}

struct Problem {
  double c, ya, yw;
};

template <class DM>
__device__ __forceinline__ double eval_cost(const DevCfg &g, const WarpSmem &sm, int lane,
                                            const Problem &pb, double a0, double a1, HelpCtl &hc) {
  PROF_BEGIN(t0)
  EvalOut e = eval_psi<DM>(&g, reinterpret_cast<unsigned char *>(sm.ctx), a0, a1, pb.c, pb.ya,
                           pb.yw, nullptr, false, 0.0);
  PROF_END(t0, 0)
  if (lane == 0) sm.ctx->n_cost++;
  return e.psi;
}
template <class DM>
__device__ __forceinline__ double eval_grad(const DevCfg &g, const WarpSmem &sm, int lane,
                                            const Problem &pb, double a0, double a1, double &o0,
                                            double &o1, HelpCtl &hc) {
  PROF_BEGIN(t0)
  EvalOut e = eval_psi<DM>(&g, reinterpret_cast<unsigned char *>(sm.ctx), a0, a1, pb.c, pb.ya, pb.yw,
                           nullptr, true, 0.0);
  PROF_END(t0, 1)
  if (lane == 0) sm.ctx->n_grad++;
  o0 = e.gv; o1 = e.gw;
  return e.psi;
}

__device__ __forceinline__ void compute_fpr(Lane &z, Uni &U) {
  z.f0 = z.u0 - z.h0; z.f1 = z.u1 - z.h1;
  double nf = pdot(z.f0, z.f1, z.f0, z.f1), ip = pdot(z.g0, z.g1, z.f0, z.f1);
  wsum2(nf, ip);
  U.norm_fpr = tt_sqrt(nf);
  U.ip = ip;
}
template <bool ENV>
__device__ __forceinline__ void gradient_and_half_step(const DevCfg &g, Lane &z, Uni &U,
                                                       double a0, double a1) {
  const double s0 = fma(-U.gamma, z.g0, a0), s1 = fma(-U.gamma, z.g1, a1);
  project(g, s0, s1, z.h0, z.h1);
  if constexpr (ENV) {
    const double e0 = s0 - z.h0, e1 = s1 - z.h1;
    double dist2 = pdot(e0, e1, e0, e1), gg = pdot(z.g0, z.g1, z.g0, z.g1);
    wsum2(dist2, gg);
    U.env_dd = dist2; U.env_g2 = gg;
  }
}

template <class DM>
__device__ bool serve_owner(const DevCfg &g, CtaHelp *cta, unsigned char *smem_raw, int m, int epoch_m,
                            const WarpSmem &mine, int lane) {
  unsigned char *base_m = smem_raw + (size_t)m * g.smem_per_warp;
  const WarpSmem own = carve<DM>(base_m, g);
  const int N = g.N;
  unsigned long long t_idle = globaltimer_ns();
  int idle_polls = 0;
  while (true) {
    int st = 0, alive = 1;
    if (lane == 0) {
      st = *reinterpret_cast<volatile int *>(&own.hhdr->state);
      alive = *reinterpret_cast<volatile int *>(&cta->busy[m]) &&
              *reinterpret_cast<volatile int *>(&cta->epoch[m]) == epoch_m;
    }
    st = __shfl_sync(FULL, st, 0);
    alive = __shfl_sync(FULL, alive, 0);
    if (st == 1 && alive) {
      __threadfence_block();
      const volatile HelpHdr *h = own.hhdr;
      double2 pt = make_double2(0.0, 0.0), yv = make_double2(0.0, 0.0);
      if (lane < N) {
        const volatile double *rq = reinterpret_cast<const volatile double *>(own.hreq);
        const volatile double *yr = reinterpret_cast<const volatile double *>(own.yrow);
        pt.x = rq[2 * lane]; pt.y = rq[2 * lane + 1];
        yv.x = yr[2 * lane]; yv.y = yr[2 * lane + 1];
      }
      const double c = h->c, gamma_ls = h->gamma_ls;
      const int grad = h->grad;
      const EvalOut e = eval_psi<DM>(&g, base_m, pt.x, pt.y, c, yv.x, yv.y, nullptr, grad != 0, gamma_ls, mine.D);
      if (lane < N) own.hres[lane] = make_double2(e.gv, e.gw);
      if (lane == 0) {
        own.hhdr->psi = e.psi; own.hhdr->f = e.f; own.hhdr->f2sq = e.f2sq; own.hhdr->S = e.S;
        own.hhdr->dd = e.dd; own.hhdr->g2 = e.g2;
      }
      __threadfence_block();
      __syncwarp();
      if (lane == 0) *reinterpret_cast<volatile int *>(&own.hhdr->state) = 2;
      t_idle = globaltimer_ns();
      idle_polls = 0;
    } else if (!alive) {
      if (lane == 0) atomicExch(&cta->helper[m], -1);
      return true;
    } else {
      if (++idle_polls > 96) {
        __nanosleep(32);
        if ((idle_polls & 255) == 0 && globaltimer_ns() - t_idle > 3000000000ull) {
          if (lane == 0) atomicExch(&cta->helper[m], -1);
          return false;
        }
      }
    }
  }
}

template <class DM>
__device__ void helper_loop(const DevCfg &g, const SolveArgs &A, CtaHelp *cta, unsigned char *smem_raw,
                            int warp, int lane) {
  const int W = g.warps_per_block;
  const WarpSmem mine = carve<DM>(smem_raw + (size_t)warp * g.smem_per_warp, g);
  const unsigned long long t_start = globaltimer_ns();
  while (true) {
    int m = -1, any_busy = 0, ep = 0;
    if (lane == 0) {
      for (int k = 1; k < W; k++) {
        const int cand = (warp + k) % W;
        if (*reinterpret_cast<volatile int *>(&cta->busy[cand])) {
          any_busy = 1;
          ep = *reinterpret_cast<volatile int *>(&cta->epoch[cand]);
          if (atomicCAS(&cta->helper[cand], -1, warp) == -1) { m = cand; break; }
        }
      }
    }
    m = __shfl_sync(FULL, m, 0);
    any_busy = __shfl_sync(FULL, any_busy, 0);
    ep = __shfl_sync(FULL, ep, 0);
    if (m < 0) {
      if (!any_busy || globaltimer_ns() - t_start > 20000000000ull) return;
      __nanosleep(2000);
      continue;
    }
    if (!serve_owner<DM>(g, cta, smem_raw, m, ep, mine, lane)) return;
  }
}

template <class DM>
__device__ bool help_long_running_mate(const DevCfg &g, const SolveArgs &A, CtaHelp *cta,
                                       unsigned char *smem_raw, int warp, int lane) {
  int m = -1, ep = 0;
  if (lane == 0) {
    const unsigned long long nd = *reinterpret_cast<volatile unsigned long long *>(A.run_stats + 1);
    if (nd >= 64) {
      const unsigned long long sum = *reinterpret_cast<volatile unsigned long long *>(A.run_stats);
      const long long thr = 4 * (long long)(sum / nd);
      const int W = g.warps_per_block;
      for (int k = 1; k < W; k++) {
        const int cand = (warp + k) % W;
        if (!*reinterpret_cast<volatile int *>(&cta->busy[cand]) ||
            *reinterpret_cast<volatile int *>(&cta->helper[cand]) != -1)
          continue;
        const volatile WarpCtx *cx = reinterpret_cast<const volatile WarpCtx *>(smem_raw + (size_t)cand * g.smem_per_warp);
        ep = *reinterpret_cast<volatile int *>(&cta->epoch[cand]);
        if (cx->n_cost + cx->n_grad > thr && atomicCAS(&cta->helper[cand], -1, warp) == -1) { m = cand; break; }
      }
    }
  }
  m = __shfl_sync(FULL, m, 0);
  ep = __shfl_sync(FULL, ep, 0);
  if (m < 0) return false;
  const WarpSmem mine = carve<DM>(smem_raw + (size_t)warp * g.smem_per_warp, g);
  serve_owner<DM>(g, cta, smem_raw, m, ep, mine, lane);
  return true;
}

template <class DM, bool HELP>
__device__ __forceinline__ bool panoc_step(const DevCfg &g, const WarpSmem &sm, int lane, const Problem &pb,
                           Lane &z, Uni &U, double tolerance, HelpCtl &hc) {
  PROF_BEGIN(t_step)
  if (U.iteration >= 1) { z.gp0 = z.g0; z.gp1 = z.g1; }
  compute_fpr(z, U);
  if (__builtin_expect(U.norm_fpr < tolerance, 0)) {
    const double r0 = fma(U.gamma, z.g0 - z.gp0, z.f0), r1 = fma(U.gamma, z.g1 - z.gp1, z.f1);
    if (sqrt(wsum(pdot(r0, r1, r0, r1))) < U.akkt_tol) return false;
  }
  bool lbfgs_done = false;
  {
    double cost_half = 0.0;
    const bool spec = __builtin_expect(help_available<HELP>(hc), 0);
    int s_first = 0, s_head = 0, s_active = 0;
    double s_gamma = 0.0, s_os0 = 0.0, s_os1 = 0.0, s_og0 = 0.0, s_og1 = 0.0;
    if (spec) {
      PROF_BEGIN(tp)
      help_post(hc, sm, lane, DM::N(g), z.h0, z.h1, pb.c, 0, 0.0);
      PROF_END(tp, 4)
      s_first = U.lb_first; s_head = U.lb_head; s_active = U.lb_active;
      s_gamma = U.lb_gamma; s_os0 = z.os0; s_os1 = z.os1; s_og0 = z.og0; s_og1 = z.og1;
    }
#pragma unroll 1
    for (int pass = 0; pass < 2; pass++) {
      if (pass == 0 ? spec : !lbfgs_done) {
        PROF_BEGIN(tl)
        {
          PROF_BEGIN(t0)
          lbfgs_update<DM>(g, sm, z, U, lane);
          PROF_END(t0, 2)
        }
        if (U.iteration > 0) {
          PROF_BEGIN(t0)
          z.d0 = z.f0; z.d1 = z.f1;
          lbfgs_apply<DM>(g, sm, z, U, lane);
          PROF_END(t0, 3)
        }
        if (pass == 0) { PROF_END(tl, 5) }
      }
      if (pass == 1) break;
      bool got = false;
      if (spec) {
        EvalOut r;
        PROF_BEGIN(tw)
        got = hc.pending && help_wait(hc, sm, lane, DM::N(g), r);
        PROF_END(tw, 6)
        if (got) {
          cost_half = r.psi;
          if (lane == 0) sm.ctx->n_cost++;
        }
      }
      if (!got) cost_half = eval_cost<DM>(g, sm, lane, pb, z.h0, z.h1, hc);
      if (spec) {
        const double rhs0 = U.cost + LIPSCHITZ_UPDATE_EPSILON * fabs(U.cost) - U.ip +
                            sm.ctx->lipc * (U.norm_fpr * U.norm_fpr);
        if (cost_half > rhs0 && U.L < MAX_LIPSCHITZ_CONSTANT) {
          U.lb_first = s_first; U.lb_head = s_head; U.lb_active = s_active; U.lb_gamma = s_gamma;
          z.os0 = s_os0; z.os1 = s_os1; z.og0 = s_og0; z.og1 = s_og1;
        } else {
          lbfgs_done = true;
        }
      }
      int it = 0;
      while (true) {
        const double rhs = U.cost + LIPSCHITZ_UPDATE_EPSILON * fabs(U.cost) - U.ip +
                           sm.ctx->lipc * (U.norm_fpr * U.norm_fpr);
        if (!(cost_half > rhs && it < MAX_LIPSCHITZ_UPDATE_ITERATIONS &&
              U.L < MAX_LIPSCHITZ_CONSTANT))
          break;
        U.lb_active = 0; U.lb_first = 1;
        U.L *= 2.0;
        U.gamma /= 2.0;
        set_lip_coeff(U, sm);
        gradient_and_half_step<false>(g, z, U, z.u0, z.u1);
        cost_half = eval_cost<DM>(g, sm, lane, pb, z.h0, z.h1, hc);
        compute_fpr(z, U);
        it++;
      }
      if (it > 0 && U.iteration > 0) gradient_and_half_step<true>(g, z, U, z.u0, z.u1);
      if (it > 0) U.sigma = tt_div(1.0 - GAMMA_L_COEFF, 4.0 * U.gamma);
    }
  }
  if (U.iteration == 0) {
    z.u0 = z.h0; z.u1 = z.h1;
    U.cost = eval_grad<DM>(g, sm, lane, pb, z.u0, z.u1, z.g0, z.g1, hc);
    gradient_and_half_step<true>(g, z, U, z.u0, z.u1);
  } else {
    const double dist2 = U.env_dd, gg = U.env_g2;
    const double fbe = U.cost - 0.5 * U.gamma * gg + div_env(0.5 * dist2, U.gamma);
    const double rhs_ls = fbe - U.sigma * (U.norm_fpr * U.norm_fpr);
    U.tau = 1.0;
    int nls = 0;
    double p0, p1;
    while (true) {
      const double one_m = 1.0 - U.tau;
      p0 = fma(-U.tau, z.d0, fma(-one_m, z.f0, z.u0));
      p1 = fma(-U.tau, z.d1, fma(-one_m, z.f1, z.u1));
      bool posted = false;
      double n0 = 0.0, n1 = 0.0;
      if (__builtin_expect(nls < MAX_LINESEARCH_ITERATIONS && help_available<HELP>(hc), 0)) {
        const double tau2 = U.tau / 2.0, one_m2 = 1.0 - tau2;
        n0 = fma(-tau2, z.d0, fma(-one_m2, z.f0, z.u0));
        n1 = fma(-tau2, z.d1, fma(-one_m2, z.f1, z.u1));
        help_post(hc, sm, lane, DM::N(g), n0, n1, pb.c, 1, U.gamma);
        posted = hc.pending;
      }
      PROF_BEGIN(t0)
      EvalOut e = eval_psi<DM>(&g, reinterpret_cast<unsigned char *>(sm.ctx), p0, p1, pb.c,
                               pb.ya, pb.yw, nullptr, true, U.gamma);
      PROF_END(t0, 1)
      if (lane == 0) sm.ctx->n_grad++;
      U.cost = e.psi;
      z.g0 = e.gv; z.g1 = e.gw; z.h0 = e.h0; z.h1 = e.h1;
      double lhs_ls = U.cost - 0.5 * U.gamma * e.g2 + div_env(0.5 * e.dd, U.gamma);
      U.env_dd = e.dd; U.env_g2 = e.g2;
      if (!(lhs_ls > rhs_ls && nls < MAX_LINESEARCH_ITERATIONS)) break;
      U.tau /= 2.0;
      nls++;
      if (posted && help_wait(hc, sm, lane, DM::N(g), e)) {
        if (lane == 0) sm.ctx->n_grad++;
        p0 = n0; p1 = n1;
        U.cost = e.psi;
        z.g0 = e.gv; z.g1 = e.gw;
        gradient_and_half_step<false>(g, z, U, p0, p1);
        lhs_ls = U.cost - 0.5 * U.gamma * e.g2 + div_env(0.5 * e.dd, U.gamma);
        U.env_dd = e.dd; U.env_g2 = e.g2;
        if (!(lhs_ls > rhs_ls && nls < MAX_LINESEARCH_ITERATIONS)) break;
        U.tau /= 2.0;
        nls++;
      }
    }
    z.u0 = p0; z.u1 = p1;
  }
  U.iteration++;
  PROF_END(t_step, 7)
  return true;
}

__device__ __forceinline__ void panoc_reset(Uni &U) {
  U.lb_active = 0; U.lb_first = 1; U.env_dd = 0.0; U.env_g2 = 0.0;
  U.tau = 1.0; U.L = 0.0; U.sigma = 0.0; U.cost = 0.0; U.iteration = 0; U.gamma = 0.0;
}

template <class DM>
__device__ void solve_scene(const DevCfg &g, const WarpSmem &sm, const SolveArgs &A, int scene,
                            int lane, unsigned long long *wstats, HelpCtl &hc) {
  const int N = g.N;
  const bool act = lane < N;
  const unsigned long long t_start = globaltimer_ns();
#ifdef TTMPC_PROFILE
  const long long t_clk0 = clock64();
#endif
  Lane z;
  Uni U;
  Problem pb;
  z.u0 = z.u1 = 0.0;
  pb.ya = pb.yw = 0.0;
  if (act) {
    if (A.use_u0) {
      z.u0 = A.u[(size_t)scene * 2 * N + 2 * lane];
      z.u1 = A.u[(size_t)scene * 2 * N + 2 * lane + 1];
    }
    if (A.use_y0 && A.y) {
      pb.ya = A.y[(size_t)scene * 2 * N + lane];
      pb.yw = A.y[(size_t)scene * 2 * N + N + lane];
    }
  }
  pb.c = A.c0 ? A.c0[scene] : g.c0;
  z.g0 = z.g1 = z.gp0 = z.gp1 = z.h0 = z.h1 = 0.0;
  z.d0 = z.d1 = z.f0 = z.f1 = z.os0 = z.os1 = z.og0 = z.og1 = 0.0;
  U.lb_head = 0; U.lb_gamma = 1.0; U.norm_fpr = 0.0;
  panoc_reset(U);
  U.akkt_tol = g.init_tol;

  double yp_a = 0.0, yp_w = 0.0;
  double delta_y_norm = 0.0, delta_y_norm_plus = 0.0, f2_norm = 0.0, f2_norm_plus = 0.0;
  double last_fpr = 0.0, f_final = 0.0;
  int alm_iter = 0, inner_count = 0, num_outer = 0, exit_status = TTMPC_CONVERGED;
  unsigned long long panoc_iters = 0;
  const double SMALL_EPSILON = 2.220446049250313e-16;

  bool in_time = true;
  for (int outer = 1; outer <= g.max_outer; outer++) {
    if (g.max_ns) {
      unsigned long long el = globaltimer_ns() - t_start;
      el = __shfl_sync(FULL, el, 0);
      if (el > g.max_ns) { exit_status = TTMPC_NOT_CONVERGED_OUT_OF_TIME; in_time = false; break; }
    }
    num_outer++;
    pb.ya = clipd(pb.ya, -1e12, 1e12);
    pb.yw = clipd(pb.yw, -1e12, 1e12);
    help_drain(hc, sm, lane, N);
    if (act) sm.yrow[lane] = make_double2(pb.ya, pb.yw);
    __syncwarp();
    int inner_status;
    {
      panoc_reset(U);
      U.cost = eval_grad<DM>(g, sm, lane, pb, z.u0, z.u1, z.g0, z.g1, hc);
      if (lane == 0) sm.ctx->n_cost++;
      {
        double h0 = 0.0, h1 = 0.0;
        if (act) {
          h0 = (EPSILON_LIPSCHITZ * z.u0 > DELTA_LIPSCHITZ) ? EPSILON_LIPSCHITZ * z.u0 : DELTA_LIPSCHITZ;
          h1 = (EPSILON_LIPSCHITZ * z.u1 > DELTA_LIPSCHITZ) ? EPSILON_LIPSCHITZ * z.u1 : DELTA_LIPSCHITZ;
        }
        double t0, t1;
        eval_grad<DM>(g, sm, lane, pb, z.u0 + h0, z.u1 + h1, t0, t1, hc);
        const double e0 = t0 - z.g0, e1 = t1 - z.g1;
        double nh = pdot(h0, h1, h0, h1);
        double nd = pdot(e0, e1, e0, e1);
        wsum2(nh, nd);
        U.L = sqrt(nd) / sqrt(nh);
      }
      U.gamma = GAMMA_L_COEFF / fmax(U.L, MIN_L_ESTIMATE);
      set_gamma_terms(U, sm);
      gradient_and_half_step<false>(g, z, U, z.u0, z.u1);

      int num_iter = 0;
      bool cont = true;
      while (true) {
        bool flag;
        if (__builtin_expect(hc.enabled && *hc.slot >= 0, 0))
          flag = panoc_step<DM, true>(g, sm, lane, pb, z, U, g.tol, hc);
        else
          flag = panoc_step<DM, false>(g, sm, lane, pb, z, U, g.tol, hc);
        if (!(flag && cont && in_time)) break;
        num_iter++;
        cont = num_iter < g.max_inner;
        if (g.max_ns) {
          unsigned long long el = globaltimer_ns() - t_start;
          el = __shfl_sync(FULL, el, 0);
          in_time = el <= g.max_ns;
        }
      }
      const bool finite = isfinite(z.u0) && isfinite(z.u1);
      if (!__all_sync(FULL, finite)) { exit_status = TTMPC_NOT_FINITE; inner_count += num_iter; break; }
      z.u0 = z.h0; z.u1 = z.h1;
      inner_status = !cont ? TTMPC_NOT_CONVERGED_ITERATIONS
                           : (!in_time ? TTMPC_NOT_CONVERGED_OUT_OF_TIME : TTMPC_CONVERGED);
      inner_count += num_iter;
      panoc_iters += num_iter;
      last_fpr = U.norm_fpr;
    }
    double F1a = 0.0, F1w = 0.0;
    {
      double vp = __shfl_up_sync(FULL, z.u0, 1), wp = __shfl_up_sync(FULL, z.u1, 1);
      if (lane == 0) { vp = sm.ctx->v_init; wp = sm.ctx->w_init; }
      if (act) { F1a = (z.u0 - vp) * g.inv_ts; F1w = (z.u1 - wp) * g.inv_ts; }
    }
    {
      const double icm = 1.0 / fmax(pb.c, 1.0);
      double t = clipd(fma(pb.ya, icm, F1a), g.amin, g.amax);
      yp_a = pb.ya + pb.c * (F1a - t);
      t = clipd(fma(pb.yw, icm, F1w), -g.awmax, g.awmax);
      yp_w = pb.yw + pb.c * (F1w - t);
      if (!act) { yp_a = 0.0; yp_w = 0.0; }
    }
    {
      const EvalOut e = eval_psi<DM>(&g, reinterpret_cast<unsigned char *>(sm.ctx), z.u0, z.u1, 0.0, 0.0,
                                     0.0, nullptr, false, 0.0);
      if (lane == 0) sm.ctx->n_cost++;
      f2_norm_plus = sqrt(e.f2sq);
      f_final = e.f;
    }
    {
      const double da = yp_a - pb.ya, dw = yp_w - pb.yw;
      delta_y_norm_plus = sqrt(wsum(pdot(da, dw, da, dw)));
    }
    const bool crit1 = alm_iter > 0 && delta_y_norm_plus <= pb.c * g.delta_tol + SMALL_EPSILON;
    const bool crit2 = f2_norm_plus <= g.delta_tol + SMALL_EPSILON;
    const bool crit3 = U.akkt_tol <= g.tol + SMALL_EPSILON;
    if (crit1 && crit2 && crit3) { exit_status = inner_status; break; }
    const bool crit_alm = delta_y_norm_plus <= g.suff_dec * delta_y_norm + SMALL_EPSILON;
    const bool crit_pm = g.Ndyn == 0 || f2_norm_plus <= g.suff_dec * f2_norm + SMALL_EPSILON;
    const bool stall = alm_iter == 0 || (crit_alm && crit_pm);
    if (!stall) pb.c *= g.pen_factor;
    U.akkt_tol = fmax(U.akkt_tol * g.tol_factor, g.tol);
    z.gp0 = 0.0; z.gp1 = 0.0;
    alm_iter++;
    delta_y_norm = delta_y_norm_plus;
    f2_norm = f2_norm_plus;
    pb.ya = yp_a; pb.yw = yp_w;
  }
  if (exit_status != TTMPC_NOT_FINITE && in_time && num_outer == g.max_outer)
    exit_status = TTMPC_NOT_CONVERGED_ITERATIONS;

  help_drain(hc, sm, lane, N);
  if (act) {
    A.u[(size_t)scene * 2 * N + 2 * lane] = z.u0;
    A.u[(size_t)scene * 2 * N + 2 * lane + 1] = z.u1;
    if (A.y) {
      A.y[(size_t)scene * 2 * N + lane] = pb.ya;
      A.y[(size_t)scene * 2 * N + N + lane] = pb.yw;
    }
  }
  if (A.pred_states)
    eval_psi<DM>(&g, reinterpret_cast<unsigned char *>(sm.ctx), z.u0, z.u1, 0.0, 0.0, 0.0,
                 A.pred_states + (size_t)scene * N * 3, false, 0.0);
  if (lane == 0) {
    if (A.cost) A.cost[scene] = f_final;
    if (A.exit_status) A.exit_status[scene] = exit_status;
    if (A.outer_iters) A.outer_iters[scene] = num_outer;
    if (A.inner_iters) A.inner_iters[scene] = inner_count;
    if (A.last_fpr) A.last_fpr[scene] = last_fpr;
    if (A.f1_infeas) A.f1_infeas[scene] = delta_y_norm_plus / pb.c;
    if (A.f2_norm) A.f2_norm[scene] = f2_norm_plus;
    if (A.penalty) A.penalty[scene] = pb.c;
    if (A.evals) {
      A.evals[4 * scene] = sm.ctx->n_cost; A.evals[4 * scene + 1] = sm.ctx->n_grad;
      A.evals[4 * scene + 2] = (long long)(globaltimer_ns() - t_start);
      A.evals[4 * scene + 3] = (long long)t_start;
    }
    wstats[0] += sm.ctx->n_cost;
    wstats[1] += sm.ctx->n_grad;
    wstats[2] += sm.ctx->n_body;
    wstats[3] += panoc_iters;
#ifdef TTMPC_PROFILE
    wstats[4] += sm.ctx->prof[0]; wstats[5] += sm.ctx->prof[1];
    wstats[6] += sm.ctx->prof[2] + sm.ctx->prof[3];
    wstats[7] += clock64() - t_clk0;
#ifndef TTMPC_PROFILE_STAGE
    sm.ctx->eprof[9] = sm.ctx->prof[3];
#else
    sm.ctx->eprof[9] = 0;
    sm.ctx->eprof[8] = sm.ctx->prof[4]; sm.ctx->eprof[7] = sm.ctx->prof[5];
#endif
#ifdef TTMPC_PROFILE_HELP
    for (int i = 0; i < 4; i++) sm.ctx->eprof[i] = sm.ctx->prof[4 + i];
#endif
    if (A.eprof) for (int i = 0; i < 10; i++) atomicAdd(A.eprof + i, (unsigned long long)sm.ctx->eprof[i]);
#endif
  }
}

template <class DM>
__global__ void __launch_bounds__(TTMPC_MAX_THREADS, TTMPC_MIN_BLOCKS) solve_kernel(const __grid_constant__ DevCfg g,
                                                    const __grid_constant__ SolveArgs A) {
  extern __shared__ __align__(16) unsigned char smem_raw[];
  const int warp = threadIdx.x >> 5, lane = threadIdx.x & 31;
  const WarpSmem sm = carve<DM>(smem_raw + (size_t)warp * g.smem_per_warp, g);
  const int gwarp = blockIdx.x * g.warps_per_block + warp;
  double *dyn = A.dyn_scratch + (size_t)gwarp * DYN_FIELDS * g.Ndyn * g.N;
  CtaHelp *cta = reinterpret_cast<CtaHelp *>(smem_raw + (size_t)g.warps_per_block * g.smem_per_warp);
  if (threadIdx.x < 8) { cta->busy[threadIdx.x] = 0; cta->helper[threadIdx.x] = -1; cta->epoch[threadIdx.x] = 0; }
  __syncthreads();
  HelpCtl hc;
  hc.enabled = A.helpers != 0;
  hc.timed_out = false;
  hc.slot = &cta->helper[warp];
  hc.pending = false;
  if (lane == 0) sm.hhdr->state = 0;
  unsigned long long wstats[8] = {0, 0, 0, 0, 0, 0, 0, 0};
  bool had_scene = false;
  while (true) {
    if (had_scene && A.helpers && A.run_stats && help_long_running_mate<DM>(g, A, cta, smem_raw, warp, lane))
      continue;
    int scene = 0;
    if (lane == 0) scene = atomicAdd(A.work_counter, 1);
    scene = __shfl_sync(FULL, scene, 0);
    if (scene >= A.n_scenes) break;
    had_scene = true;
    if (A.order) scene = A.order[scene];
    if (lane == 0) {
      *reinterpret_cast<volatile int *>(&cta->epoch[warp]) = cta->epoch[warp] + 1;
      *reinterpret_cast<volatile int *>(&cta->busy[warp]) = 1;
    }
    if (__builtin_expect(hc.timed_out, 0)) {
      if (lane == 0) {
        const unsigned long long t0 = globaltimer_ns();
        const volatile int *stp = reinterpret_cast<volatile int *>(&sm.hhdr->state);
        while (*reinterpret_cast<volatile int *>(&cta->helper[warp]) >= 0 && *stp == 1) {
          __nanosleep(1000);
          if (globaltimer_ns() - t0 > 5000000000ull) break;
        }
      }
      __syncwarp();
    }
    if (lane == 0) *reinterpret_cast<volatile int *>(&sm.hhdr->state) = 0;
    __syncwarp();
    if (A.ready) {
      int ok = 1;
      if (lane == 0) {
        const volatile int *rdy = A.ready;
        const unsigned long long t0 = globaltimer_ns();
        while (*rdy <= scene) {
          __nanosleep(200);
          if (globaltimer_ns() - t0 > 2000000000ull) {
            ok = 0; if (A.timeout_flag) atomicExch(A.timeout_flag, 1); break;
          }
        }
      }
      ok = __shfl_sync(FULL, ok, 0);
      if (!ok) {
        if (lane == 0) *reinterpret_cast<volatile int *>(&cta->busy[warp]) = 0;
        break;
      }
      __threadfence();
    }
#ifdef TTMPC_PROFILE_STAGE
    const long long t_stage0 = clock64();
#endif
    stage_scene(g, sm, A.p + (size_t)scene * g.np, dyn, lane);
#ifdef TTMPC_PROFILE_STAGE
    if (lane == 0 && A.eprof) atomicAdd(A.eprof + 9, (unsigned long long)(clock64() - t_stage0));
#endif
    hc.enabled = A.helpers != 0 && !hc.timed_out;
    solve_scene<DM>(g, sm, A, scene, lane, wstats, hc);
    if (lane == 0) {
      *reinterpret_cast<volatile int *>(&cta->busy[warp]) = 0;
      if (A.run_stats) {
        atomicAdd(A.run_stats, (unsigned long long)(sm.ctx->n_cost + sm.ctx->n_grad));
        atomicAdd(A.run_stats + 1, 1ull);
      }
    }
    __syncwarp();
  }
  if (A.helpers) helper_loop<DM>(g, A, cta, smem_raw, warp, lane);
  if (lane == 0 && A.stats) {
    for (int i = 0; i < 8; i++)
      if (wstats[i]) atomicAdd(A.stats + i, wstats[i]);
  }
}



#ifndef TTMPC_SMALL_CODE
constexpr int RANK_CLASSES = 16;
__global__ void __launch_bounds__(128) rank_scenes_kernel(const DevCfg g, const double *__restrict__ p_all,
                                                          int n, int *__restrict__ cls, int *__restrict__ hist) {
  const int scene = blockIdx.x * (blockDim.x >> 5) + (threadIdx.x >> 5), lane = threadIdx.x & 31;
  if (scene >= n) return;
  const double *p = p_all + (size_t)scene * g.np;
  int cnt = 0;
  if (lane < g.N) {
    const double x = p[g.off_r + 3 * lane], y = p[g.off_r + 3 * lane + 1];
    const double *os = p + g.off_os;
    for (int i = 0; i < g.Nstc; i++) {
      const double *b = os + i * g.nstcobs, *a0 = b + g.ne, *a1 = b + 2 * g.ne;
      bool inside = true, live = false;
      for (int e = 0; e < g.ne; e++) {
        inside = inside && (b[e] - a0[e] * x - a1[e] * y > 0.0);
        live = live || a0[e] != 0.0 || a1[e] != 0.0;
      }
      cnt += (inside && live) ? 1 : 0;
    }
    const double *od = p + g.off_od;
    for (int j = 0; j < g.Ndyn; j++) {
      const double *e = od + ((size_t)j * g.N + lane) * 6;
      const double dx = x - e[0], dy = y - e[1], r = fmax(e[2], e[3]) + g.margin;
      cnt += (e[5] > 0.0 && r > g.margin && dx * dx + dy * dy < r * r) ? 1 : 0;
    }
  }
  cnt = __reduce_add_sync(FULL, cnt);
  if (lane == 0) {
    const int c = cnt < RANK_CLASSES - 1 ? cnt : RANK_CLASSES - 1;
    cls[scene] = c;
    atomicAdd(hist + c, 1);
  }
}
__global__ void __launch_bounds__(256) order_scenes_kernel(int n, const int *__restrict__ cls,
                                                           const int *__restrict__ hist, int *__restrict__ cursor,
                                                           int *__restrict__ order) {
  const int scene = blockIdx.x * blockDim.x + threadIdx.x;
  if (scene >= n) return;
  const int c = cls[scene];
  int base = 0;
  for (int k = RANK_CLASSES - 1; k > c; k--) base += hist[k];
  order[base + atomicAdd(cursor + c, 1)] = scene;
}

template <class DM>
__global__ void __launch_bounds__(128) eval_kernel(const __grid_constant__ DevCfg g,
                                                   const __grid_constant__ EvalArgs A) {
  extern __shared__ __align__(16) unsigned char smem_raw[];
  const int warp = threadIdx.x >> 5, lane = threadIdx.x & 31;
  const WarpSmem sm = carve<DM>(smem_raw + (size_t)warp * g.smem_per_warp, g);
  const int gwarp = blockIdx.x * g.warps_per_block + warp;
  const int nwarps = gridDim.x * g.warps_per_block;
  double *dyn = A.dyn_scratch + (size_t)gwarp * DYN_FIELDS * g.Ndyn * g.N;
  const int N = g.N;
  for (int scene = gwarp; scene < A.n_scenes; scene += nwarps) {
    stage_scene(g, sm, A.p + (size_t)scene * g.np, dyn, lane);
    const bool act = lane < N;
    double v = 0.0, w = 0.0, ya = 0.0, yw = 0.0;
    if (act) {
      v = A.u[(size_t)scene * 2 * N + 2 * lane];
      w = A.u[(size_t)scene * 2 * N + 2 * lane + 1];
      if (A.y) { ya = A.y[(size_t)scene * 2 * N + lane]; yw = A.y[(size_t)scene * 2 * N + N + lane]; }
    }
    const double c = A.c ? A.c[scene] : 0.0;
    EvalOut e = eval_psi<DM>(&g, reinterpret_cast<unsigned char *>(sm.ctx), v, w, c, ya, yw, nullptr, true, 0.0);
    const double gv = e.gv, gw = e.gw;
    double vp = __shfl_up_sync(FULL, v, 1), wp = __shfl_up_sync(FULL, w, 1);
    if (lane == 0) { vp = sm.ctx->v_init; wp = sm.ctx->w_init; }
    if (act) {
      if (A.grad) { A.grad[(size_t)scene * 2 * N + 2 * lane] = gv; A.grad[(size_t)scene * 2 * N + 2 * lane + 1] = gw; }
      if (A.F1) {
        A.F1[(size_t)scene * 2 * N + lane] = (v - vp) * g.inv_ts;
        A.F1[(size_t)scene * 2 * N + N + lane] = (w - wp) * g.inv_ts;
      }
    }
    if (A.F2)
      for (int j = lane; j < g.Ndyn; j += 32)
        A.F2[(size_t)scene * g.Ndyn + j] = e.S + (e.any_hard ? sm.D[j] : 0.0);
    if (lane == 0) {
      if (A.f) A.f[scene] = e.f;
      if (A.psi) A.psi[scene] = e.psi;
    }
    __syncwarp();
  }
}

template <class DM>
__global__ void __launch_bounds__(128, 3) probe_kernel(const __grid_constant__ DevCfg g, const double *p,
                                                       double *dyn, long long *out, int reps,
                                                       int warps) {
  extern __shared__ __align__(16) unsigned char smem_all[];
  const int lane = threadIdx.x & 31, warp_id = threadIdx.x >> 5;
  if (warp_id >= warps) return;
  unsigned char *smem_raw = smem_all + (size_t)warp_id * g.smem_per_warp;
  const WarpSmem sm = carve<DM>(smem_raw, g);
  stage_scene(g, sm, p, dyn, lane);
  {
    const long long until = clock64() + ((blockIdx.x * 4 + warp_id) * 7919) % 9000;
    while (clock64() < until) {}
  }
  double v = lane < g.N ? 0.8 : 0.0, w = lane < g.N ? 0.05 : 0.0, acc = 0.0;
  long long t0 = clock64();
  for (int i = 0; i < reps; i++) {
    EvalOut e = eval_psi<DM>(&g, smem_raw, v, w, 10.0, 0.0, 0.0, nullptr, false, 0.0);
    v += 1e-9 * e.psi * 0.0 + 1e-12;
    acc += e.psi;
  }
  long long t1 = clock64();
  for (int i = 0; i < reps; i++) {
    EvalOut e = eval_psi<DM>(&g, smem_raw, v, w, 10.0, 0.0, 0.0, nullptr, true, 1e-3);
    v += e.gv * 1e-300; w += e.gw * 1e-300;
    acc += e.psi;
  }
  long long t2 = clock64();
  for (int i = 0; i < reps; i++) acc = wsum(acc * 1e-3 + v);
  long long t3 = clock64();
  Lane z; Uni U;
  z.d0 = v; z.d1 = w; U.lb_active = g.mem; U.lb_head = 0; U.lb_gamma = 0.7;
  if (lane < g.N)
    for (int k = 0; k <= g.mem; k++) {
      sm.lbs[k * (g.N | 1) + lane] = make_double2(0.01 * (k + 1), 0.02);
      sm.lby[k * (g.N | 1) + lane] = make_double2(0.03, 0.01 * (k + 2));
    }
  if (lane <= g.mem) sm.rho[lane] = 0.5;
  __syncwarp();
  for (int i = 0; i < reps; i++) { lbfgs_apply<DM>(g, sm, z, U, lane); z.d0 *= 1e-3; z.d1 *= 1e-3; }
  long long t4 = clock64();
  double d = 1.0 + acc * 1e-30;
  for (int i = 0; i < reps; i++) d = 1.0 / (d + 0.5);
  long long t5 = clock64();
  for (int i = 0; i < reps; i++) d = sqrt(d + 0.5);
  long long t6 = clock64();
  double f = d;
  for (int i = 0; i < reps; i++) f = fma(f, 0.999, 1e-3);
  long long t7 = clock64();
  if (lane == 0 && blockIdx.x == 0 && warp_id == 0) {
    out[0] = (t1 - t0) / reps; out[1] = (t2 - t1) / reps; out[2] = (t3 - t2) / reps;
    out[3] = (t4 - t3) / reps; out[4] = (t5 - t4) / reps; out[5] = (t6 - t5) / reps;
    out[6] = (t7 - t6) / reps; out[7] = (long long)(acc + z.d0 + d + f);
  }
}

__global__ void fp64_peak_kernel(double *out, int iters) {
  double a0 = threadIdx.x * 1e-3, a1 = a0 + 1, a2 = a0 + 2, a3 = a0 + 3, a4 = a0 + 4, a5 = a0 + 5,
         a6 = a0 + 6, a7 = a0 + 7;
  const double b = 1.0000001, c = 1e-9;
  for (int i = 0; i < iters; i++) {
    a0 = fma(a0, b, c); a1 = fma(a1, b, c); a2 = fma(a2, b, c); a3 = fma(a3, b, c);
    a4 = fma(a4, b, c); a5 = fma(a5, b, c); a6 = fma(a6, b, c); a7 = fma(a7, b, c);
  }
  out[blockIdx.x * blockDim.x + threadIdx.x] = a0 + a1 + a2 + a3 + a4 + a5 + a6 + a7;
}

#endif
}

namespace ttmpc {

static bool is_default_dims(const DevCfg &g) {
  return g.N == 20 && g.Nother == 10 && g.Nstc == 10 && g.ne == 4 && g.Ndyn == 15 && g.mem == 10;
}

static std::mutex g_attr_mu;
static std::map<std::pair<const void *, int>, size_t> g_attr_smem;
static std::map<std::tuple<const void *, int, int, size_t>, int> g_attr_occ;
template <class K>
static cudaError_t set_smem(K kernel, size_t smem) {
  int dev = 0;
  cudaError_t e = cudaGetDevice(&dev);
  if (e != cudaSuccess) return e;
  const auto key = std::make_pair(reinterpret_cast<const void *>(kernel), dev);
  {
    std::lock_guard<std::mutex> lk(g_attr_mu);
    auto it = g_attr_smem.find(key);
    if (it != g_attr_smem.end() && it->second >= smem) return cudaSuccess;
  }
  e = cudaFuncSetAttribute(kernel, cudaFuncAttributeMaxDynamicSharedMemorySize, (int)smem);
  if (e == cudaSuccess) {
    std::lock_guard<std::mutex> lk(g_attr_mu);
    size_t &v = g_attr_smem[key];
    if (v < smem) v = smem;
  }
  return e;
}
template <class K>
static cudaError_t cached_occupancy(K kernel, int block, size_t smem, int *blocks_per_sm) {
  int dev = 0;
  cudaError_t e = cudaGetDevice(&dev);
  if (e != cudaSuccess) return e;
  const auto key = std::make_tuple(reinterpret_cast<const void *>(kernel), dev, block, smem);
  {
    std::lock_guard<std::mutex> lk(g_attr_mu);
    auto it = g_attr_occ.find(key);
    if (it != g_attr_occ.end()) { *blocks_per_sm = it->second; return cudaSuccess; }
  }
  if ((e = set_smem(kernel, smem)) != cudaSuccess) return e;
  e = cudaOccupancyMaxActiveBlocksPerMultiprocessor(blocks_per_sm, kernel, block, smem);
  if (e == cudaSuccess) {
    std::lock_guard<std::mutex> lk(g_attr_mu);
    g_attr_occ[key] = *blocks_per_sm;
  }
  return e;
}

#define TTMPC_SOLVE_SHAPES(X) \
  X(20, 10, 10, 4, 15, 10)    \
  X(10, 10, 10, 4, 15, 10)    \
  X(32, 10, 10, 4, 15, 10)    \
  X(20, 10, 4, 4, 4, 10)      \
  X(20, 10, 20, 4, 30, 10)
template <class F>
static cudaError_t with_solve_dims(const DevCfg &g, F &&f) {
#define X(n, no, ns, e, nd, m) \
  if (g.N == n && g.Nother == no && g.Nstc == ns && g.ne == e && g.Ndyn == nd && g.mem == m) return f(Dims<n, no, ns, e, nd, m>{});
  TTMPC_SOLVE_SHAPES(X)
#undef X
  return f(DimsRuntime{});
}

cudaError_t launch_solve(const DevCfg &g, const SolveArgs &A, int grid, cudaStream_t st) {
  const size_t smem = (size_t)g.smem_per_warp * g.warps_per_block + sizeof(CtaHelp);
  return with_solve_dims(g, [&](auto dm) -> cudaError_t {
    using DM = decltype(dm);
    cudaError_t e;
    if ((e = set_smem(solve_kernel<DM>, smem)) != cudaSuccess) return e;
    solve_kernel<DM><<<grid, g.warps_per_block * 32, smem, st>>>(g, A);
    return cudaGetLastError();
  });
}
cudaError_t solve_occupancy_impl(const DevCfg &g, int *blocks_per_sm) {
  const size_t smem = (size_t)g.smem_per_warp * g.warps_per_block + sizeof(CtaHelp);
  return with_solve_dims(g, [&](auto dm) -> cudaError_t {
    using DM = decltype(dm);
    return cached_occupancy(solve_kernel<DM>, g.warps_per_block * 32, smem, blocks_per_sm);
  });
}
#ifndef TTMPC_SMALL_CODE
cudaError_t launch_rank_scenes(const DevCfg &g, const double *p, int n, int *scratch, int *order,
                               cudaStream_t st) {
  int *cls = scratch, *hist = scratch + n, *cursor = hist + RANK_CLASSES;
  cudaError_t e = cudaMemsetAsync(hist, 0, 2 * RANK_CLASSES * sizeof(int), st);
  if (e != cudaSuccess) return e;
  rank_scenes_kernel<<<(n + 3) / 4, 128, 0, st>>>(g, p, n, cls, hist);
  order_scenes_kernel<<<(n + 255) / 256, 256, 0, st>>>(n, cls, hist, cursor, order);
  return cudaGetLastError();
}
cudaError_t launch_eval(const DevCfg &g, const EvalArgs &A, int grid, cudaStream_t st) {
  const size_t smem = (size_t)g.smem_per_warp * g.warps_per_block;
  cudaError_t e;
  if (is_default_dims(g)) {
    if ((e = set_smem(eval_kernel<DimsDefault>, smem)) != cudaSuccess) return e;
    eval_kernel<DimsDefault><<<grid, g.warps_per_block * 32, smem, st>>>(g, A);
  } else {
    if ((e = set_smem(eval_kernel<DimsRuntime>, smem)) != cudaSuccess) return e;
    eval_kernel<DimsRuntime><<<grid, g.warps_per_block * 32, smem, st>>>(g, A);
  }
  return cudaGetLastError();
}
cudaError_t solve_occupancy(const DevCfg &g, int *blocks_per_sm) { return solve_occupancy_impl(g, blocks_per_sm); }
cudaError_t launch_probe(const DevCfg &g, const double *p, double *dyn, long long *out, int reps,
                         cudaStream_t st) {
  const size_t smem = (size_t)g.smem_per_warp * g.warps_per_block;
  cudaError_t e;
  int grid = 1, warps = 1;
  if (const char *s = std::getenv("TTMPC_PROBE_GRID")) grid = std::max(1, std::atoi(s));
  if (const char *s = std::getenv("TTMPC_PROBE_WARPS")) warps = std::min(std::max(1, std::atoi(s)), g.warps_per_block);
  if (is_default_dims(g)) {
    if ((e = set_smem(probe_kernel<DimsDefault>, smem)) != cudaSuccess) return e;
    probe_kernel<DimsDefault><<<grid, 128, smem, st>>>(g, p, dyn, out, reps, warps);
  } else {
    if ((e = set_smem(probe_kernel<DimsRuntime>, smem)) != cudaSuccess) return e;
    probe_kernel<DimsRuntime><<<grid, 128, smem, st>>>(g, p, dyn, out, reps, warps);
  }
  return cudaGetLastError();
}
cudaError_t launch_fp64_peak(double *out, int blocks, int threads, int iters, cudaStream_t st) {
  fp64_peak_kernel<<<blocks, threads, 0, st>>>(out, iters);
  return cudaGetLastError();
}

#endif
}
```

Before: 665,600.

## Move per-warp solver state from registers into shared memory to cut register pressure

Moves PANOC/L-BFGS scalar state and the old iterate/gradient vectors out of per-lane registers into a shared-memory context struct and per-warp buffers. It also shrinks the dyn table slots from 4 to 1, drops the odd-stride padding of the L-BFGS history, aliases hres onto hreq, and replaces per-warp stat accumulators with direct atomics. The grid is now sized from the occupancy of the small-code kernel when that kernel is chosen. The aim is lower register use and smaller shared memory per warp so more warps are resident. The cost is extra shared-memory traffic, more syncwarps, and possible bank conflicts from removing the padding.

```diff
diff --git a/trajtrack_mpcndqn_rlboost_b200/csrc/ttmpc_api.cu b/trajtrack_mpcndqn_rlboost_b200/csrc/ttmpc_api.cu
--- a/trajtrack_mpcndqn_rlboost_b200/csrc/ttmpc_api.cu
+++ b/trajtrack_mpcndqn_rlboost_b200/csrc/ttmpc_api.cu
@@ -280,13 +280,35 @@
   return TTMPC_OK;
 }
 
-static int grid_for(Workspace *w, const DevCfg &g, int n_scenes, int *grid) {
-  int bps = 0;
-  CUDA_TRY(solve_occupancy(g, &bps));
+static int grid_for_occupancy(Workspace *w, const DevCfg &g, int n_scenes, int bps, int *grid) {
   if (bps < 1) return fail(TTMPC_ERR_UNSUPPORTED, "configuration does not fit in shared memory");
   long long want = ((long long)n_scenes + g.warps_per_block - 1) / g.warps_per_block;
   long long cap = (long long)w->sm_count * bps;
   *grid = (int)(want < cap ? (want < 1 ? 1 : want) : cap);
+  return TTMPC_OK;
+}
+static int grid_for(Workspace *w, const DevCfg &g, int n_scenes, int *grid) {
+  int bps = 0;
+  CUDA_TRY(solve_occupancy(g, &bps));
+  return grid_for_occupancy(w, g, n_scenes, bps, grid);
+}
+struct SolvePlan { int grid, blocks_per_sm; bool small_code; };
+static int plan_solve(Workspace *w, const DevCfg &g, int n_scenes, SolvePlan *pl) {
+  int bps = 0, grid = 0;
+  CUDA_TRY(solve_occupancy(g, &bps));
+  int rc = grid_for_occupancy(w, g, n_scenes, bps, &grid);
+  if (rc) return rc;
+  bool small_code = n_scenes > (long long)grid * g.warps_per_block;
+  if (const char *e = std::getenv("TTMPC_CODE")) {
+    if (e[0] == 's') small_code = true;
+    else if (e[0] == 'u') small_code = false;
+  }
+  if (small_code) {
+    CUDA_TRY(solve_occupancy_small(g, &bps));
+    rc = grid_for_occupancy(w, g, n_scenes, bps, &grid);
+    if (rc) return rc;
+  }
+  pl->grid = grid; pl->blocks_per_sm = bps; pl->small_code = small_code;
   return TTMPC_OK;
 }
 
@@ -312,19 +334,19 @@
   Workspace *w;
   Slot *sl = host_slot;
   const int *d_ready = (host_slot && gated) ? host_slot->ready : nullptr;
-  int grid;
+  SolvePlan plan;
   bool want_order = false;
   {
     std::lock_guard<std::mutex> lk(g_mu);
     rc = get_ws(&w);
     if (rc) return rc;
     if (!sl) { rc = slot_for_stream(w, st, &sl); if (rc) return rc; }
-    rc = grid_for(w, g, n_scenes, &grid);
+    rc = plan_solve(w, g, n_scenes, &plan);
     if (rc) return rc;
     const size_t table = (size_t)DYN_FIELDS * g.Ndyn * g.N * sizeof(double);
-    rc = ensure_dyn(sl, (table ? table : 8) * (size_t)grid * g.warps_per_block);
+    rc = ensure_dyn(sl, (table ? table : 8) * (size_t)plan.grid * g.warps_per_block);
     if (rc) return rc;
-    want_order = !d_ready && n_scenes > (long long)grid * g.warps_per_block;
+    want_order = !d_ready && n_scenes > (long long)plan.grid * g.warps_per_block;
     if (want_order) {
       rc = ensure_order(sl, 2 * (size_t)n_scenes + 64);
       if (rc) return rc;
@@ -349,13 +371,8 @@
     CUDA_TRY(launch_rank_scenes(g, d_p, n_scenes, sl->order + n_scenes, sl->order, st));
     A.order = sl->order;
   }
-  bool small_code = n_scenes > (long long)grid * g.warps_per_block;
-  if (const char *e = std::getenv("TTMPC_CODE")) {
-    if (e[0] == 's') small_code = true;
-    else if (e[0] == 'u') small_code = false;
-  }
-  if (small_code) CUDA_TRY(launch_solve_small(g, A, grid, st));
-  else CUDA_TRY(launch_solve(g, A, grid, st));
+  if (plan.small_code) CUDA_TRY(launch_solve_small(g, A, plan.grid, st));
+  else CUDA_TRY(launch_solve(g, A, plan.grid, st));
   return TTMPC_OK;
 }
 
@@ -431,15 +448,13 @@
   Workspace *w;
   rc = get_ws(&w);
   if (rc) return rc;
-  int gr;
-  rc = grid_for(w, g, n_scenes, &gr);
-  if (rc) return rc;
-  int bps = 0;
-  CUDA_TRY(solve_occupancy(g, &bps));
-  if (grid) *grid = gr;
+  SolvePlan plan;
+  rc = plan_solve(w, g, n_scenes, &plan);
+  if (rc) return rc;
+  if (grid) *grid = plan.grid;
   if (block) *block = g.warps_per_block * 32;
   if (smem_bytes) *smem_bytes = g.smem_per_warp * g.warps_per_block;
-  if (blocks_per_sm) *blocks_per_sm = bps;
+  if (blocks_per_sm) *blocks_per_sm = plan.blocks_per_sm;
   if (sm_count) *sm_count = w->sm_count;
   return TTMPC_OK;
 }
diff --git a/trajtrack_mpcndqn_rlboost_b200/csrc/ttmpc_device.cuh b/trajtrack_mpcndqn_rlboost_b200/csrc/ttmpc_device.cuh
--- a/trajtrack_mpcndqn_rlboost_b200/csrc/ttmpc_device.cuh
+++ b/trajtrack_mpcndqn_rlboost_b200/csrc/ttmpc_device.cuh
@@ -17,7 +17,7 @@
 constexpr int MAX_EDGE = 8;
 constexpr int DYN_FIELDS = 10;
 #ifndef TT_DYN_SLOTS
-#define TT_DYN_SLOTS 4
+#define TT_DYN_SLOTS 1
 #endif
 constexpr int DYN_SLOTS = TT_DYN_SLOTS;
 
@@ -203,6 +203,19 @@
   return fma(a1, b1, a0 * b0);
 }
 
+struct PanocCold {
+  double L, sigma, lb_gamma;
+  double ip;
+  double env_dd, env_g2;
+  double tau;
+  double rhs_ls;
+  int iteration;
+  int lb_active, lb_head, lb_first;
+};
+struct SpecSave {
+  double lb_gamma;
+  int lb_first, lb_head, lb_active;
+};
 struct WarpCtx {
   const double *p;
   double *dyn;
@@ -216,6 +229,11 @@
   unsigned fleet_live;
   double lipc;
   double icm_c, icm;
+  PanocCold pc;
+  SpecSave spec;
+  double akkt_tol, f_final, last_fpr, dy_norm, dy_norm_plus, f2_norm, f2_norm_plus;
+  unsigned long long t_start, panoc_iters;
+  int inner_count, exit_status, num_outer, scene, in_time;
 #ifdef TTMPC_PROFILE
   long long prof[8];
   long long eprof[10];
@@ -235,7 +253,9 @@
   double2 *lbs;
   double2 *lby;
   double *rho;
-  double *alpha;
+  double2 *gprev;
+  double2 *olds;
+  double2 *oldg;
   double2 *hreq;
   double2 *hres;
   double2 *yrow;
@@ -280,11 +300,10 @@
   b += (sizeof(float2) * (size_t)Nother * N + 15) / 16 * 16;
   b += (sizeof(float) * 3 * (size_t)Ndyn * N + 15) / 16 * 16;
   b += sizeof(double) * (size_t)(Ndyn ? DYN_SLOTS * DYN_FIELDS * N : 0);
-  const int NP = N | 1;
-  b += sizeof(double2) * (size_t)(mem + 1) * NP * 2;
+  b += sizeof(double2) * (size_t)(mem + 1) * N * 2;
   b += sizeof(double) * ((mem + 2) / 2 * 2);
-  b += sizeof(double) * (2 * (mem + 1));
-  b += sizeof(double2) * 3 * (size_t)N + (sizeof(HelpHdr) + 15) / 16 * 16;
+  b += sizeof(double2) * ((size_t)N + 64);
+  b += sizeof(double2) * 2 * (size_t)N + (sizeof(HelpHdr) + 15) / 16 * 16;
   return (int)((b + 15) / 16 * 16);
 }
 
@@ -295,9 +314,8 @@
   const int N = DM::N(g), MEM = DM::mem(g), Nother = DM::Nother(g), Nstc = DM::Nstc(g),
             nstcobs = 3 * DM::ne(g), Ndyn = DM::Ndyn(g);
   w.ctx = reinterpret_cast<WarpCtx *>(q); q += (sizeof(WarpCtx) + 15) / 16 * 16;
-  const int NP = N | 1;
-  w.lbs = reinterpret_cast<double2 *>(q); q += sizeof(double2) * (size_t)(MEM + 1) * NP;
-  w.lby = reinterpret_cast<double2 *>(q); q += sizeof(double2) * (size_t)(MEM + 1) * NP;
+  w.lbs = reinterpret_cast<double2 *>(q); q += sizeof(double2) * (size_t)(MEM + 1) * N;
+  w.lby = reinterpret_cast<double2 *>(q); q += sizeof(double2) * (size_t)(MEM + 1) * N;
   w.fleet = reinterpret_cast<float2 *>(q); q += (sizeof(float2) * (size_t)Nother * N + 15) / 16 * 16;
   w.dynb = reinterpret_cast<float *>(q); q += (sizeof(float) * 3 * (size_t)Ndyn * N + 15) / 16 * 16;
   w.dynt = reinterpret_cast<double *>(q); q += sizeof(double) * (size_t)(Ndyn ? DYN_SLOTS * DYN_FIELDS * N : 0);
@@ -306,9 +324,11 @@
   w.D = reinterpret_cast<double *>(q); q += sizeof(double) * ((Ndyn + 1) / 2 * 2);
   w.vref = reinterpret_cast<double *>(q); q += sizeof(double) * ((N + 1) / 2 * 2);
   w.rho = reinterpret_cast<double *>(q); q += sizeof(double) * ((MEM + 2) / 2 * 2);
-  w.alpha = reinterpret_cast<double *>(q); q += sizeof(double) * (2 * (MEM + 1));
+  w.gprev = reinterpret_cast<double2 *>(q); q += sizeof(double2) * (size_t)N;
+  w.olds = reinterpret_cast<double2 *>(q); q += sizeof(double2) * 32;
+  w.oldg = reinterpret_cast<double2 *>(q); q += sizeof(double2) * 32;
   w.hreq = reinterpret_cast<double2 *>(q); q += sizeof(double2) * (size_t)N;
-  w.hres = reinterpret_cast<double2 *>(q); q += sizeof(double2) * (size_t)N;
+  w.hres = w.hreq;
   w.yrow = reinterpret_cast<double2 *>(q); q += sizeof(double2) * (size_t)N;
   w.hhdr = reinterpret_cast<HelpHdr *>(q);
   return w;
diff --git a/trajtrack_mpcndqn_rlboost_b200/csrc/ttmpc_launch.cuh b/trajtrack_mpcndqn_rlboost_b200/csrc/ttmpc_launch.cuh
--- a/trajtrack_mpcndqn_rlboost_b200/csrc/ttmpc_launch.cuh
+++ b/trajtrack_mpcndqn_rlboost_b200/csrc/ttmpc_launch.cuh
@@ -38,6 +38,7 @@
                                cudaStream_t st);
 cudaError_t launch_eval(const DevCfg &g, const EvalArgs &A, int grid, cudaStream_t st);
 cudaError_t solve_occupancy(const DevCfg &g, int *blocks_per_sm);
+cudaError_t solve_occupancy_small(const DevCfg &g, int *blocks_per_sm);
 cudaError_t launch_probe(const DevCfg &g, const double *p, double *dyn, long long *out, int reps,
                          cudaStream_t st);
 struct FleetDims { int N, np, n_other, n_stc, n_dyn; double ts; };
diff --git a/trajtrack_mpcndqn_rlboost_b200/csrc/ttmpc_solve.cu b/trajtrack_mpcndqn_rlboost_b200/csrc/ttmpc_solve.cu
--- a/trajtrack_mpcndqn_rlboost_b200/csrc/ttmpc_solve.cu
+++ b/trajtrack_mpcndqn_rlboost_b200/csrc/ttmpc_solve.cu
@@ -9,13 +9,16 @@
 #ifndef TTMPC_MIN_BLOCKS
 #define TTMPC_MIN_BLOCKS 2
 #endif
+#ifndef TTMPC_MIN_BLOCKS_RUNTIME
+#define TTMPC_MIN_BLOCKS_RUNTIME TTMPC_MIN_BLOCKS
+#endif
 #ifndef TTMPC_MAX_THREADS
 #define TTMPC_MAX_THREADS 128
 #endif
 #ifdef TTMPC_SMALL_CODE
 #define solve_kernel solve_kernel_small
 #define launch_solve launch_solve_small
-#define solve_occupancy_impl solve_occupancy_small_impl
+#define solve_occupancy solve_occupancy_small
 #endif
 
 namespace ttmpc {
@@ -27,6 +30,7 @@
 constexpr int MAX_LIPSCHITZ_UPDATE_ITERATIONS = 10;
 constexpr double MAX_LIPSCHITZ_CONSTANT = 1e9;
 constexpr int MAX_LINESEARCH_ITERATIONS = 10;
+constexpr double MIN_LINESEARCH_TAU = 1.0 / (1 << MAX_LINESEARCH_ITERATIONS);
 constexpr double MIN_L_ESTIMATE = 1e-10;
 constexpr double CBFGS_EPSILON = 1e-8;
 constexpr double SY_EPSILON = 1e-10;
@@ -34,18 +38,14 @@
 struct Lane {
   double u0, u1;
   double g0, g1;
-  double gp0, gp1;
   double h0, h1;
   double d0, d1;
   double f0, f1;
-  double os0, os1, og0, og1;
 };
 
 struct Uni {
-  double gamma, L, sigma, cost, norm_fpr, tau, akkt_tol, lb_gamma;
-  double ip;
-  double env_dd, env_g2;
-  int iteration, lb_active, lb_head, lb_first;
+  double gamma, cost, norm_fpr;
+  PanocCold *pc;
 };
 
 __device__ __forceinline__ void project(const DevCfg &g, double a0, double a1, double &o0, double &o1) {
@@ -60,7 +60,7 @@
   __syncwarp();
 }
 __device__ __forceinline__ void set_gamma_terms(Uni &U, const WarpSmem &sm) {
-  U.sigma = tt_div(1.0 - GAMMA_L_COEFF, 4.0 * U.gamma);
+  U.pc->sigma = tt_div(1.0 - GAMMA_L_COEFF, 4.0 * U.gamma);
   set_lip_coeff(U, sm);
 }
 __device__ __forceinline__ double div_env(double x, double y) {
@@ -68,15 +68,20 @@
   return tt_div(x, y);
 }
 
+__device__ __forceinline__ void set_old(const WarpSmem &sm, const Lane &z, int lane) {
+  sm.olds[lane] = make_double2(z.u0, z.u1);
+  sm.oldg[lane] = make_double2(z.f0, z.f1);
+}
 template <class DM>
-__device__ __forceinline__ void lbfgs_update(const DevCfg &g, const WarpSmem &sm, Lane &z, Uni &U,
-                                             int lane) {
-  const int N = DM::N(g), NP = N | 1, MEM = DM::mem(g), M1 = MEM + 1;
-  const double sv0 = z.u0 - z.os0, sv1 = z.u1 - z.os1;
-  const double yv0 = z.f0 - z.og0, yv1 = z.f1 - z.og1;
+__device__ __forceinline__ bool lbfgs_update(const DevCfg &g, const WarpSmem &sm, Lane &z, Uni &U,
+                                             int lane, bool keep_old = true) {
+  const int N = DM::N(g), MEM = DM::mem(g), M1 = MEM + 1;
+  const double2 os = sm.olds[lane], og = sm.oldg[lane];
+  const double sv0 = z.u0 - os.x, sv1 = z.u1 - os.y;
+  const double yv0 = z.f0 - og.x, yv1 = z.f1 - og.y;
   bool accept = true;
   double ys = 0.0, yy = 0.0;
-  if (!U.lb_first) {
+  if (!U.pc->lb_first) {
     double ss = pdot(sv0, sv1, sv0, sv1);
     ys = pdot(sv0, sv1, yv0, yv1); yy = pdot(yv0, yv1, yv0, yv1);
     wsum3(ys, ss, yy);
@@ -85,45 +90,50 @@
     accept = !(ss <= 2.2250738585072014e-308 || ys <= SY_EPSILON) &&
              (lhs > rhs && isfinite(lhs) && isfinite(rhs));
   }
-  if (!accept) return;
-  z.os0 = z.u0; z.os1 = z.u1; z.og0 = z.f0; z.og1 = z.f1;
-  if (U.lb_first) { U.lb_first = 0; return; }
-  U.lb_head = U.lb_head + MEM; if (U.lb_head >= M1) U.lb_head -= M1;
-  const int k0 = U.lb_head;
+  if (!accept) return false;
+  if (keep_old) set_old(sm, z, lane);
+  if (U.pc->lb_first) {
+    __syncwarp();
+    U.pc->lb_first = 0;
+    return true;
+  }
+  int k0 = U.pc->lb_head + MEM; if (k0 >= M1) k0 -= M1;
+  const int active = min(MEM, U.pc->lb_active + 1);
   const double rho = tt_div(1.0, ys);
   if (lane < N) {
-    sm.lbs[k0 * NP + lane] = make_double2(sv0, sv1);
-    sm.lby[k0 * NP + lane] = make_double2(yv0, yv1);
+    sm.lbs[k0 * N + lane] = make_double2(sv0, sv1);
+    sm.lby[k0 * N + lane] = make_double2(yv0, yv1);
   }
   if (lane == 0) sm.rho[k0] = rho;
-  U.lb_gamma = tt_div(tt_div(1.0, rho), yy);
-  U.lb_active = min(MEM, U.lb_active + 1);
+  U.pc->lb_gamma = tt_div(tt_div(1.0, rho), yy);
   __syncwarp();
+  U.pc->lb_head = k0; U.pc->lb_active = active;
+  return true;
 }
 
 template <class DM>
 __device__ __forceinline__ void lbfgs_apply(const DevCfg &g, const WarpSmem &sm, Lane &z,
                                             const Uni &U, int lane) {
-  const int m = U.lb_active;
+  const int m = U.pc->lb_active;
   if (m == 0) return;
-  const int N = DM::N(g), NP = N | 1, M1 = DM::mem(g) + 1;
+  const int N = DM::N(g), M1 = DM::mem(g) + 1;
   const bool act = lane < N;
   const int lk = act ? lane : N - 1;
   double q0 = z.d0, q1 = z.d1, a_me = 0.0;
-  int k = U.lb_head;
+  int k = U.pc->lb_head;
 #pragma unroll 1
   for (int i = 0; i < m; i++) {
-    const double2 s = sm.lbs[k * NP + lk], y = sm.lby[k * NP + lk];
+    const double2 s = sm.lbs[k * N + lk], y = sm.lby[k * N + lk];
     const double a = sm.rho[k] * wsum_inl(act ? pdot(s.x, s.y, q0, q1) : 0.0);
     if (lane == i) a_me = a;
     q0 = fma(-a, y.x, q0); q1 = fma(-a, y.y, q1);
     k = (k + 1 == M1) ? 0 : k + 1;
   }
-  q0 = U.lb_gamma * q0; q1 = U.lb_gamma * q1;
+  q0 = U.pc->lb_gamma * q0; q1 = U.pc->lb_gamma * q1;
 #pragma unroll 1
   for (int i = m - 1; i >= 0; i--) {
     k = (k == 0) ? M1 - 1 : k - 1;
-    const double2 s = sm.lbs[k * NP + lk], y = sm.lby[k * NP + lk];
+    const double2 s = sm.lbs[k * N + lk], y = sm.lby[k * N + lk];
     const double beta = sm.rho[k] * wsum_inl(act ? pdot(y.x, y.y, q0, q1) : 0.0);
     const double cf = __shfl_sync(FULL, a_me, i) - beta;
     q0 = fma(cf, s.x, q0); q1 = fma(cf, s.y, q1);
@@ -150,16 +160,25 @@
   int helper[8];
   int epoch[8];
 };
+extern __shared__ __align__(16) unsigned char smem_raw[];
+__device__ __forceinline__ CtaHelp *cta_help() { return reinterpret_cast<CtaHelp *>(smem_raw); }
+__device__ __forceinline__ unsigned char *warp_region(const DevCfg &g, int w) {
+  return smem_raw + sizeof(CtaHelp) + (size_t)w * g.smem_per_warp;
+}
 struct HelpCtl {
   bool enabled;
   bool timed_out;
-  volatile int *slot;
   bool pending;
 };
+__device__ __forceinline__ int ld_volatile_shared(unsigned addr) {
+  int v;
+  asm volatile("ld.volatile.shared.s32 %0, [%1];" : "=r"(v) : "r"(addr));
+  return v;
+}
 template <bool HELP>
 __device__ __forceinline__ bool help_available(const HelpCtl &hc) {
   if constexpr (!HELP) return false;
-  else return hc.enabled && *hc.slot >= 0;
+  else return hc.enabled && ld_volatile_shared((unsigned)__cvta_generic_to_shared(&cta_help()->helper[threadIdx.x >> 5])) >= 0;
 }
 __device__ __forceinline__ bool help_wait(HelpCtl &hc, const WarpSmem &sm, int lane, int N, EvalOut &e) {
   int ok = 1;
@@ -241,7 +260,7 @@
   double nf = pdot(z.f0, z.f1, z.f0, z.f1), ip = pdot(z.g0, z.g1, z.f0, z.f1);
   wsum2(nf, ip);
   U.norm_fpr = tt_sqrt(nf);
-  U.ip = ip;
+  U.pc->ip = ip;
 }
 template <bool ENV>
 __device__ __forceinline__ void gradient_and_half_step(const DevCfg &g, Lane &z, Uni &U,
@@ -252,14 +271,14 @@
     const double e0 = s0 - z.h0, e1 = s1 - z.h1;
     double dist2 = pdot(e0, e1, e0, e1), gg = pdot(z.g0, z.g1, z.g0, z.g1);
     wsum2(dist2, gg);
-    U.env_dd = dist2; U.env_g2 = gg;
+    U.pc->env_dd = dist2; U.pc->env_g2 = gg;
   }
 }
 
 template <class DM>
-__device__ bool serve_owner(const DevCfg &g, CtaHelp *cta, unsigned char *smem_raw, int m, int epoch_m,
+__device__ bool serve_owner(const DevCfg &g, CtaHelp *cta, int m, int epoch_m,
                             const WarpSmem &mine, int lane) {
-  unsigned char *base_m = smem_raw + (size_t)m * g.smem_per_warp;
+  unsigned char *base_m = warp_region(g, m);
   const WarpSmem own = carve<DM>(base_m, g);
   const int N = g.N;
   unsigned long long t_idle = globaltimer_ns();
@@ -312,10 +331,9 @@
 }
 
 template <class DM>
-__device__ void helper_loop(const DevCfg &g, const SolveArgs &A, CtaHelp *cta, unsigned char *smem_raw,
-                            int warp, int lane) {
+__device__ void helper_loop(const DevCfg &g, const SolveArgs &A, CtaHelp *cta, int warp, int lane) {
   const int W = g.warps_per_block;
-  const WarpSmem mine = carve<DM>(smem_raw + (size_t)warp * g.smem_per_warp, g);
+  const WarpSmem mine = carve<DM>(warp_region(g, warp), g);
   const unsigned long long t_start = globaltimer_ns();
   while (true) {
     int m = -1, any_busy = 0, ep = 0;
@@ -337,13 +355,13 @@
       __nanosleep(2000);
       continue;
     }
-    if (!serve_owner<DM>(g, cta, smem_raw, m, ep, mine, lane)) return;
+    if (!serve_owner<DM>(g, cta, m, ep, mine, lane)) return;
   }
 }
 
 template <class DM>
 __device__ bool help_long_running_mate(const DevCfg &g, const SolveArgs &A, CtaHelp *cta,
-                                       unsigned char *smem_raw, int warp, int lane) {
+                                       int warp, int lane) {
   int m = -1, ep = 0;
   if (lane == 0) {
     const unsigned long long nd = *reinterpret_cast<volatile unsigned long long *>(A.run_stats + 1);
@@ -356,7 +374,7 @@
         if (!*reinterpret_cast<volatile int *>(&cta->busy[cand]) ||
             *reinterpret_cast<volatile int *>(&cta->helper[cand]) != -1)
           continue;
-        const volatile WarpCtx *cx = reinterpret_cast<const volatile WarpCtx *>(smem_raw + (size_t)cand * g.smem_per_warp);
+        const volatile WarpCtx *cx = reinterpret_cast<const volatile WarpCtx *>(warp_region(g, cand));
         ep = *reinterpret_cast<volatile int *>(&cta->epoch[cand]);
         if (cx->n_cost + cx->n_grad > thr && atomicCAS(&cta->helper[cand], -1, warp) == -1) { m = cand; break; }
       }
@@ -365,33 +383,41 @@
   m = __shfl_sync(FULL, m, 0);
   ep = __shfl_sync(FULL, ep, 0);
   if (m < 0) return false;
-  const WarpSmem mine = carve<DM>(smem_raw + (size_t)warp * g.smem_per_warp, g);
-  serve_owner<DM>(g, cta, smem_raw, m, ep, mine, lane);
+  const WarpSmem mine = carve<DM>(warp_region(g, warp), g);
+  serve_owner<DM>(g, cta, m, ep, mine, lane);
   return true;
+}
+
+__device__ __forceinline__ void halve_tau(Uni &U) {
+  const double t = U.pc->tau / 2.0;
+  __syncwarp();
+  U.pc->tau = t;
 }
 
 template <class DM, bool HELP>
 __device__ __forceinline__ bool panoc_step(const DevCfg &g, const WarpSmem &sm, int lane, const Problem &pb,
                            Lane &z, Uni &U, double tolerance, HelpCtl &hc) {
   PROF_BEGIN(t_step)
-  if (U.iteration >= 1) { z.gp0 = z.g0; z.gp1 = z.g1; }
+  const bool act = lane < DM::N(g);
+  if (U.pc->iteration >= 1 && act) sm.gprev[lane] = make_double2(z.g0, z.g1);
   compute_fpr(z, U);
   if (__builtin_expect(U.norm_fpr < tolerance, 0)) {
-    const double r0 = fma(U.gamma, z.g0 - z.gp0, z.f0), r1 = fma(U.gamma, z.g1 - z.gp1, z.f1);
-    if (sqrt(wsum(pdot(r0, r1, r0, r1))) < U.akkt_tol) return false;
+    const double2 gp = act ? sm.gprev[lane] : make_double2(0.0, 0.0);
+    const double r0 = fma(U.gamma, z.g0 - gp.x, z.f0), r1 = fma(U.gamma, z.g1 - gp.y, z.f1);
+    if (sqrt(wsum(pdot(r0, r1, r0, r1))) < sm.ctx->akkt_tol) return false;
   }
   bool lbfgs_done = false;
   {
     double cost_half = 0.0;
     const bool spec = __builtin_expect(help_available<HELP>(hc), 0);
-    int s_first = 0, s_head = 0, s_active = 0;
-    double s_gamma = 0.0, s_os0 = 0.0, s_os1 = 0.0, s_og0 = 0.0, s_og1 = 0.0;
+    bool s_accept = false;
+    SpecSave &sv = sm.ctx->spec;
     if (spec) {
       PROF_BEGIN(tp)
       help_post(hc, sm, lane, DM::N(g), z.h0, z.h1, pb.c, 0, 0.0);
       PROF_END(tp, 4)
-      s_first = U.lb_first; s_head = U.lb_head; s_active = U.lb_active;
-      s_gamma = U.lb_gamma; s_os0 = z.os0; s_os1 = z.os1; s_og0 = z.og0; s_og1 = z.og1;
+      sv.lb_first = U.pc->lb_first; sv.lb_head = U.pc->lb_head; sv.lb_active = U.pc->lb_active;
+      sv.lb_gamma = U.pc->lb_gamma;
     }
 #pragma unroll 1
     for (int pass = 0; pass < 2; pass++) {
@@ -399,10 +425,11 @@
         PROF_BEGIN(tl)
         {
           PROF_BEGIN(t0)
-          lbfgs_update<DM>(g, sm, z, U, lane);
+          const bool acc = lbfgs_update<DM>(g, sm, z, U, lane, pass != 0);
+          if (pass == 0) s_accept = acc;
           PROF_END(t0, 2)
         }
-        if (U.iteration > 0) {
+        if (U.pc->iteration > 0) {
           PROF_BEGIN(t0)
           z.d0 = z.f0; z.d1 = z.f1;
           lbfgs_apply<DM>(g, sm, z, U, lane);
@@ -424,24 +451,27 @@
       }
       if (!got) cost_half = eval_cost<DM>(g, sm, lane, pb, z.h0, z.h1, hc);
       if (spec) {
-        const double rhs0 = U.cost + LIPSCHITZ_UPDATE_EPSILON * fabs(U.cost) - U.ip +
+        const double rhs0 = U.cost + LIPSCHITZ_UPDATE_EPSILON * fabs(U.cost) - U.pc->ip +
                             sm.ctx->lipc * (U.norm_fpr * U.norm_fpr);
-        if (cost_half > rhs0 && U.L < MAX_LIPSCHITZ_CONSTANT) {
-          U.lb_first = s_first; U.lb_head = s_head; U.lb_active = s_active; U.lb_gamma = s_gamma;
-          z.os0 = s_os0; z.os1 = s_os1; z.og0 = s_og0; z.og1 = s_og1;
+        if (cost_half > rhs0 && U.pc->L < MAX_LIPSCHITZ_CONSTANT) {
+          U.pc->lb_first = sv.lb_first; U.pc->lb_head = sv.lb_head; U.pc->lb_active = sv.lb_active;
+          U.pc->lb_gamma = sv.lb_gamma;
         } else {
           lbfgs_done = true;
+          if (s_accept) set_old(sm, z, lane);
         }
       }
       int it = 0;
       while (true) {
-        const double rhs = U.cost + LIPSCHITZ_UPDATE_EPSILON * fabs(U.cost) - U.ip +
+        const double rhs = U.cost + LIPSCHITZ_UPDATE_EPSILON * fabs(U.cost) - U.pc->ip +
                            sm.ctx->lipc * (U.norm_fpr * U.norm_fpr);
         if (!(cost_half > rhs && it < MAX_LIPSCHITZ_UPDATE_ITERATIONS &&
-              U.L < MAX_LIPSCHITZ_CONSTANT))
+              U.pc->L < MAX_LIPSCHITZ_CONSTANT))
           break;
-        U.lb_active = 0; U.lb_first = 1;
-        U.L *= 2.0;
+        U.pc->lb_active = 0; U.pc->lb_first = 1;
+        const double L2 = U.pc->L * 2.0;
+        __syncwarp();
+        U.pc->L = L2;
         U.gamma /= 2.0;
         set_lip_coeff(U, sm);
         gradient_and_half_step<false>(g, z, U, z.u0, z.u1);
@@ -449,29 +479,28 @@
         compute_fpr(z, U);
         it++;
       }
-      if (it > 0 && U.iteration > 0) gradient_and_half_step<true>(g, z, U, z.u0, z.u1);
-      if (it > 0) U.sigma = tt_div(1.0 - GAMMA_L_COEFF, 4.0 * U.gamma);
-    }
-  }
-  if (U.iteration == 0) {
+      if (it > 0 && U.pc->iteration > 0) gradient_and_half_step<true>(g, z, U, z.u0, z.u1);
+      if (it > 0) U.pc->sigma = tt_div(1.0 - GAMMA_L_COEFF, 4.0 * U.gamma);
+    }
+  }
+  if (U.pc->iteration == 0) {
     z.u0 = z.h0; z.u1 = z.h1;
     U.cost = eval_grad<DM>(g, sm, lane, pb, z.u0, z.u1, z.g0, z.g1, hc);
     gradient_and_half_step<true>(g, z, U, z.u0, z.u1);
   } else {
-    const double dist2 = U.env_dd, gg = U.env_g2;
+    const double dist2 = U.pc->env_dd, gg = U.pc->env_g2;
     const double fbe = U.cost - 0.5 * U.gamma * gg + div_env(0.5 * dist2, U.gamma);
-    const double rhs_ls = fbe - U.sigma * (U.norm_fpr * U.norm_fpr);
-    U.tau = 1.0;
-    int nls = 0;
+    U.pc->rhs_ls = fbe - U.pc->sigma * (U.norm_fpr * U.norm_fpr);
+    U.pc->tau = 1.0;
     double p0, p1;
     while (true) {
-      const double one_m = 1.0 - U.tau;
-      p0 = fma(-U.tau, z.d0, fma(-one_m, z.f0, z.u0));
-      p1 = fma(-U.tau, z.d1, fma(-one_m, z.f1, z.u1));
+      const double one_m = 1.0 - U.pc->tau;
+      p0 = fma(-U.pc->tau, z.d0, fma(-one_m, z.f0, z.u0));
+      p1 = fma(-U.pc->tau, z.d1, fma(-one_m, z.f1, z.u1));
       bool posted = false;
       double n0 = 0.0, n1 = 0.0;
-      if (__builtin_expect(nls < MAX_LINESEARCH_ITERATIONS && help_available<HELP>(hc), 0)) {
-        const double tau2 = U.tau / 2.0, one_m2 = 1.0 - tau2;
+      if (__builtin_expect(U.pc->tau > MIN_LINESEARCH_TAU && help_available<HELP>(hc), 0)) {
+        const double tau2 = U.pc->tau / 2.0, one_m2 = 1.0 - tau2;
         n0 = fma(-tau2, z.d0, fma(-one_m2, z.f0, z.u0));
         n1 = fma(-tau2, z.d1, fma(-one_m2, z.f1, z.u1));
         help_post(hc, sm, lane, DM::N(g), n0, n1, pb.c, 1, U.gamma);
@@ -485,10 +514,9 @@
       U.cost = e.psi;
       z.g0 = e.gv; z.g1 = e.gw; z.h0 = e.h0; z.h1 = e.h1;
       double lhs_ls = U.cost - 0.5 * U.gamma * e.g2 + div_env(0.5 * e.dd, U.gamma);
-      U.env_dd = e.dd; U.env_g2 = e.g2;
-      if (!(lhs_ls > rhs_ls && nls < MAX_LINESEARCH_ITERATIONS)) break;
-      U.tau /= 2.0;
-      nls++;
+      U.pc->env_dd = e.dd; U.pc->env_g2 = e.g2;
+      if (!(lhs_ls > U.pc->rhs_ls && U.pc->tau > MIN_LINESEARCH_TAU)) break;
+      halve_tau(U);
       if (posted && help_wait(hc, sm, lane, DM::N(g), e)) {
         if (lane == 0) sm.ctx->n_grad++;
         p0 = n0; p1 = n1;
@@ -496,35 +524,40 @@
         z.g0 = e.gv; z.g1 = e.gw;
         gradient_and_half_step<false>(g, z, U, p0, p1);
         lhs_ls = U.cost - 0.5 * U.gamma * e.g2 + div_env(0.5 * e.dd, U.gamma);
-        U.env_dd = e.dd; U.env_g2 = e.g2;
-        if (!(lhs_ls > rhs_ls && nls < MAX_LINESEARCH_ITERATIONS)) break;
-        U.tau /= 2.0;
-        nls++;
+        U.pc->env_dd = e.dd; U.pc->env_g2 = e.g2;
+        if (!(lhs_ls > U.pc->rhs_ls && U.pc->tau > MIN_LINESEARCH_TAU)) break;
+        halve_tau(U);
       }
     }
     z.u0 = p0; z.u1 = p1;
   }
-  U.iteration++;
+  {
+    const int it1 = U.pc->iteration + 1;
+    __syncwarp();
+    U.pc->iteration = it1;
+  }
   PROF_END(t_step, 7)
   return true;
 }
 
 __device__ __forceinline__ void panoc_reset(Uni &U) {
-  U.lb_active = 0; U.lb_first = 1; U.env_dd = 0.0; U.env_g2 = 0.0;
-  U.tau = 1.0; U.L = 0.0; U.sigma = 0.0; U.cost = 0.0; U.iteration = 0; U.gamma = 0.0;
+  U.pc->lb_active = 0; U.pc->lb_first = 1; U.pc->env_dd = 0.0; U.pc->env_g2 = 0.0;
+  U.pc->tau = 1.0; U.pc->L = 0.0; U.pc->sigma = 0.0; U.cost = 0.0; U.pc->iteration = 0; U.gamma = 0.0;
 }
 
 template <class DM>
 __device__ void solve_scene(const DevCfg &g, const WarpSmem &sm, const SolveArgs &A, int scene,
-                            int lane, unsigned long long *wstats, HelpCtl &hc) {
+                            int lane, HelpCtl &hc) {
   const int N = g.N;
   const bool act = lane < N;
-  const unsigned long long t_start = globaltimer_ns();
+  WarpCtx *const cx = sm.ctx;
+  cx->t_start = __shfl_sync(FULL, globaltimer_ns(), 0);
 #ifdef TTMPC_PROFILE
   const long long t_clk0 = clock64();
 #endif
   Lane z;
   Uni U;
+  U.pc = &cx->pc;
   Problem pb;
   z.u0 = z.u1 = 0.0;
   pb.ya = pb.yw = 0.0;
@@ -539,27 +572,31 @@
     }
   }
   pb.c = A.c0 ? A.c0[scene] : g.c0;
-  z.g0 = z.g1 = z.gp0 = z.gp1 = z.h0 = z.h1 = 0.0;
-  z.d0 = z.d1 = z.f0 = z.f1 = z.os0 = z.os1 = z.og0 = z.og1 = 0.0;
-  U.lb_head = 0; U.lb_gamma = 1.0; U.norm_fpr = 0.0;
+  z.g0 = z.g1 = z.h0 = z.h1 = 0.0;
+  if (act) sm.gprev[lane] = make_double2(0.0, 0.0);
+  z.d0 = z.d1 = z.f0 = z.f1 = 0.0;
+  sm.olds[lane] = make_double2(0.0, 0.0);
+  sm.oldg[lane] = make_double2(0.0, 0.0);
+  U.pc->lb_head = 0; U.pc->lb_gamma = 1.0; U.norm_fpr = 0.0;
   panoc_reset(U);
-  U.akkt_tol = g.init_tol;
+  cx->akkt_tol = g.init_tol;
 
   double yp_a = 0.0, yp_w = 0.0;
-  double delta_y_norm = 0.0, delta_y_norm_plus = 0.0, f2_norm = 0.0, f2_norm_plus = 0.0;
-  double last_fpr = 0.0, f_final = 0.0;
-  int alm_iter = 0, inner_count = 0, num_outer = 0, exit_status = TTMPC_CONVERGED;
-  unsigned long long panoc_iters = 0;
+  cx->dy_norm = 0.0; cx->dy_norm_plus = 0.0; cx->f2_norm = 0.0; cx->f2_norm_plus = 0.0;
+  cx->last_fpr = 0.0; cx->f_final = 0.0;
+  cx->inner_count = 0; cx->exit_status = TTMPC_CONVERGED; cx->panoc_iters = 0;
+  cx->num_outer = 0;
+  cx->scene = scene;
   const double SMALL_EPSILON = 2.220446049250313e-16;
 
-  bool in_time = true;
-  for (int outer = 1; outer <= g.max_outer; outer++) {
+  cx->in_time = 1;
+  for (int outer = 1; outer <= g.max_outer; outer = cx->num_outer + 1) {
     if (g.max_ns) {
-      unsigned long long el = globaltimer_ns() - t_start;
+      unsigned long long el = globaltimer_ns() - cx->t_start;
       el = __shfl_sync(FULL, el, 0);
-      if (el > g.max_ns) { exit_status = TTMPC_NOT_CONVERGED_OUT_OF_TIME; in_time = false; break; }
-    }
-    num_outer++;
+      if (el > g.max_ns) { cx->exit_status = TTMPC_NOT_CONVERGED_OUT_OF_TIME; cx->in_time = 0; break; }
+    }
+    cx->num_outer = outer;
     pb.ya = clipd(pb.ya, -1e12, 1e12);
     pb.yw = clipd(pb.yw, -1e12, 1e12);
     help_drain(hc, sm, lane, N);
@@ -582,37 +619,39 @@
         double nh = pdot(h0, h1, h0, h1);
         double nd = pdot(e0, e1, e0, e1);
         wsum2(nh, nd);
-        U.L = sqrt(nd) / sqrt(nh);
-      }
-      U.gamma = GAMMA_L_COEFF / fmax(U.L, MIN_L_ESTIMATE);
+        U.pc->L = sqrt(nd) / sqrt(nh);
+      }
+      U.gamma = GAMMA_L_COEFF / fmax(U.pc->L, MIN_L_ESTIMATE);
       set_gamma_terms(U, sm);
       gradient_and_half_step<false>(g, z, U, z.u0, z.u1);
 
-      int num_iter = 0;
-      bool cont = true;
+      bool flag;
       while (true) {
-        bool flag;
-        if (__builtin_expect(hc.enabled && *hc.slot >= 0, 0))
+        if (__builtin_expect(help_available<true>(hc), 0))
           flag = panoc_step<DM, true>(g, sm, lane, pb, z, U, g.tol, hc);
         else
           flag = panoc_step<DM, false>(g, sm, lane, pb, z, U, g.tol, hc);
-        if (!(flag && cont && in_time)) break;
-        num_iter++;
-        cont = num_iter < g.max_inner;
+        if (!(flag && U.pc->iteration - 1 < g.max_inner && cx->in_time)) break;
         if (g.max_ns) {
-          unsigned long long el = globaltimer_ns() - t_start;
+          unsigned long long el = globaltimer_ns() - cx->t_start;
           el = __shfl_sync(FULL, el, 0);
-          in_time = el <= g.max_ns;
+          cx->in_time = el <= g.max_ns;
         }
       }
+      const int num_iter = flag ? U.pc->iteration - 1 : U.pc->iteration;
+      const bool cont = num_iter < g.max_inner;
       const bool finite = isfinite(z.u0) && isfinite(z.u1);
-      if (!__all_sync(FULL, finite)) { exit_status = TTMPC_NOT_FINITE; inner_count += num_iter; break; }
+      const int ic = cx->inner_count + num_iter;
+      const unsigned long long pi = cx->panoc_iters + num_iter;
+      const bool all_finite = __all_sync(FULL, finite);
+      __syncwarp();
+      cx->inner_count = ic;
+      if (!all_finite) { cx->exit_status = TTMPC_NOT_FINITE; break; }
       z.u0 = z.h0; z.u1 = z.h1;
       inner_status = !cont ? TTMPC_NOT_CONVERGED_ITERATIONS
-                           : (!in_time ? TTMPC_NOT_CONVERGED_OUT_OF_TIME : TTMPC_CONVERGED);
-      inner_count += num_iter;
-      panoc_iters += num_iter;
-      last_fpr = U.norm_fpr;
+                           : (!cx->in_time ? TTMPC_NOT_CONVERGED_OUT_OF_TIME : TTMPC_CONVERGED);
+      cx->panoc_iters = pi;
+      cx->last_fpr = U.norm_fpr;
     }
     double F1a = 0.0, F1w = 0.0;
     {
@@ -628,36 +667,46 @@
       yp_w = pb.yw + pb.c * (F1w - t);
       if (!act) { yp_a = 0.0; yp_w = 0.0; }
     }
+    double f2_norm_plus;
     {
       const EvalOut e = eval_psi<DM>(&g, reinterpret_cast<unsigned char *>(sm.ctx), z.u0, z.u1, 0.0, 0.0,
                                      0.0, nullptr, false, 0.0);
       if (lane == 0) sm.ctx->n_cost++;
       f2_norm_plus = sqrt(e.f2sq);
-      f_final = e.f;
-    }
+      cx->f2_norm_plus = f2_norm_plus;
+      cx->f_final = e.f;
+    }
+    double delta_y_norm_plus;
     {
       const double da = yp_a - pb.ya, dw = yp_w - pb.yw;
       delta_y_norm_plus = sqrt(wsum(pdot(da, dw, da, dw)));
-    }
+      cx->dy_norm_plus = delta_y_norm_plus;
+    }
+    const double akkt_tol = cx->akkt_tol;
+    const int alm_iter = cx->num_outer - 1;
     const bool crit1 = alm_iter > 0 && delta_y_norm_plus <= pb.c * g.delta_tol + SMALL_EPSILON;
     const bool crit2 = f2_norm_plus <= g.delta_tol + SMALL_EPSILON;
-    const bool crit3 = U.akkt_tol <= g.tol + SMALL_EPSILON;
-    if (crit1 && crit2 && crit3) { exit_status = inner_status; break; }
-    const bool crit_alm = delta_y_norm_plus <= g.suff_dec * delta_y_norm + SMALL_EPSILON;
-    const bool crit_pm = g.Ndyn == 0 || f2_norm_plus <= g.suff_dec * f2_norm + SMALL_EPSILON;
+    const bool crit3 = akkt_tol <= g.tol + SMALL_EPSILON;
+    if (crit1 && crit2 && crit3) { cx->exit_status = inner_status; break; }
+    const bool crit_alm = delta_y_norm_plus <= g.suff_dec * cx->dy_norm + SMALL_EPSILON;
+    const bool crit_pm = g.Ndyn == 0 || f2_norm_plus <= g.suff_dec * cx->f2_norm + SMALL_EPSILON;
     const bool stall = alm_iter == 0 || (crit_alm && crit_pm);
     if (!stall) pb.c *= g.pen_factor;
-    U.akkt_tol = fmax(U.akkt_tol * g.tol_factor, g.tol);
-    z.gp0 = 0.0; z.gp1 = 0.0;
-    alm_iter++;
-    delta_y_norm = delta_y_norm_plus;
-    f2_norm = f2_norm_plus;
+    __syncwarp();
+    cx->akkt_tol = fmax(akkt_tol * g.tol_factor, g.tol);
+    if (act) sm.gprev[lane] = make_double2(0.0, 0.0);
+    cx->dy_norm = delta_y_norm_plus;
+    cx->f2_norm = f2_norm_plus;
     pb.ya = yp_a; pb.yw = yp_w;
   }
-  if (exit_status != TTMPC_NOT_FINITE && in_time && num_outer == g.max_outer)
+  help_drain(hc, sm, lane, N);
+  __syncwarp();
+  int exit_status = cx->exit_status;
+  const int num_outer = cx->num_outer;
+  if (exit_status != TTMPC_NOT_FINITE && cx->in_time && num_outer == g.max_outer)
     exit_status = TTMPC_NOT_CONVERGED_ITERATIONS;
 
-  help_drain(hc, sm, lane, N);
+  scene = cx->scene;
   if (act) {
     A.u[(size_t)scene * 2 * N + 2 * lane] = z.u0;
     A.u[(size_t)scene * 2 * N + 2 * lane + 1] = z.u1;
@@ -670,27 +719,32 @@
     eval_psi<DM>(&g, reinterpret_cast<unsigned char *>(sm.ctx), z.u0, z.u1, 0.0, 0.0, 0.0,
                  A.pred_states + (size_t)scene * N * 3, false, 0.0);
   if (lane == 0) {
-    if (A.cost) A.cost[scene] = f_final;
+    if (A.cost) A.cost[scene] = cx->f_final;
     if (A.exit_status) A.exit_status[scene] = exit_status;
     if (A.outer_iters) A.outer_iters[scene] = num_outer;
-    if (A.inner_iters) A.inner_iters[scene] = inner_count;
-    if (A.last_fpr) A.last_fpr[scene] = last_fpr;
-    if (A.f1_infeas) A.f1_infeas[scene] = delta_y_norm_plus / pb.c;
-    if (A.f2_norm) A.f2_norm[scene] = f2_norm_plus;
+    if (A.inner_iters) A.inner_iters[scene] = cx->inner_count;
+    if (A.last_fpr) A.last_fpr[scene] = cx->last_fpr;
+    if (A.f1_infeas) A.f1_infeas[scene] = cx->dy_norm_plus / pb.c;
+    if (A.f2_norm) A.f2_norm[scene] = cx->f2_norm_plus;
     if (A.penalty) A.penalty[scene] = pb.c;
     if (A.evals) {
       A.evals[4 * scene] = sm.ctx->n_cost; A.evals[4 * scene + 1] = sm.ctx->n_grad;
-      A.evals[4 * scene + 2] = (long long)(globaltimer_ns() - t_start);
-      A.evals[4 * scene + 3] = (long long)t_start;
-    }
-    wstats[0] += sm.ctx->n_cost;
-    wstats[1] += sm.ctx->n_grad;
-    wstats[2] += sm.ctx->n_body;
-    wstats[3] += panoc_iters;
+      A.evals[4 * scene + 2] = (long long)(globaltimer_ns() - cx->t_start);
+      A.evals[4 * scene + 3] = (long long)cx->t_start;
+    }
+    if (A.stats) {
+      atomicAdd(A.stats + 0, (unsigned long long)sm.ctx->n_cost);
+      atomicAdd(A.stats + 1, (unsigned long long)sm.ctx->n_grad);
+      atomicAdd(A.stats + 2, (unsigned long long)sm.ctx->n_body);
+      atomicAdd(A.stats + 3, cx->panoc_iters);
 #ifdef TTMPC_PROFILE
-    wstats[4] += sm.ctx->prof[0]; wstats[5] += sm.ctx->prof[1];
-    wstats[6] += sm.ctx->prof[2] + sm.ctx->prof[3];
-    wstats[7] += clock64() - t_clk0;
+      atomicAdd(A.stats + 4, (unsigned long long)sm.ctx->prof[0]);
+      atomicAdd(A.stats + 5, (unsigned long long)sm.ctx->prof[1]);
+      atomicAdd(A.stats + 6, (unsigned long long)(sm.ctx->prof[2] + sm.ctx->prof[3]));
+      atomicAdd(A.stats + 7, (unsigned long long)(clock64() - t_clk0));
+#endif
+    }
+#ifdef TTMPC_PROFILE
 #ifndef TTMPC_PROFILE_STAGE
     sm.ctx->eprof[9] = sm.ctx->prof[3];
 #else
@@ -706,26 +760,21 @@
 }
 
 template <class DM>
-__global__ void __launch_bounds__(TTMPC_MAX_THREADS, TTMPC_MIN_BLOCKS) solve_kernel(const __grid_constant__ DevCfg g,
+__global__ void __launch_bounds__(TTMPC_MAX_THREADS, DM::kN ? TTMPC_MIN_BLOCKS : TTMPC_MIN_BLOCKS_RUNTIME) solve_kernel(const __grid_constant__ DevCfg g,
                                                     const __grid_constant__ SolveArgs A) {
-  extern __shared__ __align__(16) unsigned char smem_raw[];
   const int warp = threadIdx.x >> 5, lane = threadIdx.x & 31;
-  const WarpSmem sm = carve<DM>(smem_raw + (size_t)warp * g.smem_per_warp, g);
-  const int gwarp = blockIdx.x * g.warps_per_block + warp;
-  double *dyn = A.dyn_scratch + (size_t)gwarp * DYN_FIELDS * g.Ndyn * g.N;
-  CtaHelp *cta = reinterpret_cast<CtaHelp *>(smem_raw + (size_t)g.warps_per_block * g.smem_per_warp);
+  const WarpSmem sm = carve<DM>(warp_region(g, warp), g);
+  CtaHelp *cta = cta_help();
   if (threadIdx.x < 8) { cta->busy[threadIdx.x] = 0; cta->helper[threadIdx.x] = -1; cta->epoch[threadIdx.x] = 0; }
   __syncthreads();
   HelpCtl hc;
   hc.enabled = A.helpers != 0;
   hc.timed_out = false;
-  hc.slot = &cta->helper[warp];
   hc.pending = false;
   if (lane == 0) sm.hhdr->state = 0;
-  unsigned long long wstats[8] = {0, 0, 0, 0, 0, 0, 0, 0};
   bool had_scene = false;
   while (true) {
-    if (had_scene && A.helpers && A.run_stats && help_long_running_mate<DM>(g, A, cta, smem_raw, warp, lane))
+    if (had_scene && A.helpers && A.run_stats && help_long_running_mate<DM>(g, A, cta, warp, lane))
       continue;
     int scene = 0;
     if (lane == 0) scene = atomicAdd(A.work_counter, 1);
@@ -772,12 +821,15 @@
 #ifdef TTMPC_PROFILE_STAGE
     const long long t_stage0 = clock64();
 #endif
-    stage_scene(g, sm, A.p + (size_t)scene * g.np, dyn, lane);
+    {
+      const int gwarp = blockIdx.x * g.warps_per_block + warp;
+      stage_scene(g, sm, A.p + (size_t)scene * g.np, A.dyn_scratch + (size_t)gwarp * DYN_FIELDS * g.Ndyn * g.N, lane);
+    }
 #ifdef TTMPC_PROFILE_STAGE
     if (lane == 0 && A.eprof) atomicAdd(A.eprof + 9, (unsigned long long)(clock64() - t_stage0));
 #endif
     hc.enabled = A.helpers != 0 && !hc.timed_out;
-    solve_scene<DM>(g, sm, A, scene, lane, wstats, hc);
+    solve_scene<DM>(g, sm, A, scene, lane, hc);
     if (lane == 0) {
       *reinterpret_cast<volatile int *>(&cta->busy[warp]) = 0;
       if (A.run_stats) {
@@ -787,11 +839,7 @@
     }
     __syncwarp();
   }
-  if (A.helpers) helper_loop<DM>(g, A, cta, smem_raw, warp, lane);
-  if (lane == 0 && A.stats) {
-    for (int i = 0; i < 8; i++)
-      if (wstats[i]) atomicAdd(A.stats + i, wstats[i]);
-  }
+  if (A.helpers) helper_loop<DM>(g, A, cta, warp, lane);
 }
 
 
@@ -844,7 +892,6 @@
 template <class DM>
 __global__ void __launch_bounds__(128) eval_kernel(const __grid_constant__ DevCfg g,
                                                    const __grid_constant__ EvalArgs A) {
-  extern __shared__ __align__(16) unsigned char smem_raw[];
   const int warp = threadIdx.x >> 5, lane = threadIdx.x & 31;
   const WarpSmem sm = carve<DM>(smem_raw + (size_t)warp * g.smem_per_warp, g);
   const int gwarp = blockIdx.x * g.warps_per_block + warp;
@@ -914,11 +961,12 @@
   for (int i = 0; i < reps; i++) acc = wsum(acc * 1e-3 + v);
   long long t3 = clock64();
   Lane z; Uni U;
-  z.d0 = v; z.d1 = w; U.lb_active = g.mem; U.lb_head = 0; U.lb_gamma = 0.7;
+  U.pc = &sm.ctx->pc;
+  z.d0 = v; z.d1 = w; U.pc->lb_active = g.mem; U.pc->lb_head = 0; U.pc->lb_gamma = 0.7;
   if (lane < g.N)
     for (int k = 0; k <= g.mem; k++) {
-      sm.lbs[k * (g.N | 1) + lane] = make_double2(0.01 * (k + 1), 0.02);
-      sm.lby[k * (g.N | 1) + lane] = make_double2(0.03, 0.01 * (k + 2));
+      sm.lbs[k * g.N + lane] = make_double2(0.01 * (k + 1), 0.02);
+      sm.lby[k * g.N + lane] = make_double2(0.03, 0.01 * (k + 2));
     }
   if (lane <= g.mem) sm.rho[lane] = 0.5;
   __syncwarp();
@@ -1026,7 +1074,7 @@
     return cudaGetLastError();
   });
 }
-cudaError_t solve_occupancy_impl(const DevCfg &g, int *blocks_per_sm) {
+cudaError_t solve_occupancy(const DevCfg &g, int *blocks_per_sm) {
   const size_t smem = (size_t)g.smem_per_warp * g.warps_per_block + sizeof(CtaHelp);
   return with_solve_dims(g, [&](auto dm) -> cudaError_t {
     using DM = decltype(dm);
@@ -1055,7 +1103,6 @@
   }
   return cudaGetLastError();
 }
-cudaError_t solve_occupancy(const DevCfg &g, int *blocks_per_sm) { return solve_occupancy_impl(g, blocks_per_sm); }
 cudaError_t launch_probe(const DevCfg &g, const double *p, double *dyn, long long *out, int reps,
                          cudaStream_t st) {
   const size_t smem = (size_t)g.smem_per_warp * g.warps_per_block;
```

New measurement: 753,600, median of 6. +13.2%, better.
